# xiongzhenhai-zh/emqx

Measured on AMD Instinct MI355X. Metric: published topics matched/sec (and match evals/sec) at 10M subs; % of HBM BW, higher is better.
Workload: dtype u32; 1 GPU; B: 10M mixed exact/'+'/'#' subscriptions, 1xMI355X, batched topics of depth 4-8; n_filters=10000000, batch_topics_per_gpu=1000000, mode=routes, parallelism=replicated table, topic stream split x1, walk_order=batch order

## Files before the change

### emqx_amd/csrc/engine.cpp

```cpp
#include <hip/hip_runtime.h>

#include <algorithm>
#include <atomic>
#include <chrono>
#include <cstdlib>
#include <cstring>
#include <memory>
#include <mutex>
#include <string>
#include <thread>
#include <vector>

#include "../../include/emqx_match.h"
#include "kernels.h"
#include "streams.h"
#include "tables.h"

using namespace emqx;

namespace {

#define HIP_TRY(expr)                    \
  do {                                   \
    hipError_t _e = (expr);              \
    if (_e != hipSuccess) {              \
      set_last_error(hipGetErrorString(_e)); \
      return EMQX_EDEVICE;               \
    }                                    \
  } while (0)

thread_local std::string g_last_error;
void set_last_error(const char* s) { g_last_error = s ? s : ""; }

template <class T>
void dfree(T*& p) {
  if (p) (void)hipFree(p);
  p = nullptr;
}

template <class T>
hipError_t dalloc(T*& p, uint64_t count) {
  dfree(p);
  return hipMalloc(reinterpret_cast<void**>(&p), std::max<uint64_t>(count, 1) * sizeof(T));
}

struct DeviceTables {
  int device = 0;
  EdgeSlot* edges = nullptr;
  uint32_t* fids = nullptr;
  VocabSlot* vocab = nullptr;
  uint8_t* arena = nullptr;
  uint64_t cap_slots = 0, n_vocab = 0, cap_arena = 0;
  uint64_t bytes() const {
    return cap_slots * (sizeof(EdgeSlot) + 2 * sizeof(uint32_t)) + n_vocab * sizeof(VocabSlot) + cap_arena;
  }
  ~DeviceTables() {
    int cur = 0;
    (void)hipGetDevice(&cur);
    (void)hipSetDevice(device);
    (void)hipDeviceSynchronize();
    dfree(edges);
    dfree(fids);
    dfree(vocab);
    dfree(arena);
    (void)hipSetDevice(cur);
  }
};

struct Snapshot {
  std::shared_ptr<DeviceTables> dt;
  TableView tv{};
  uint64_t n_nodes = 0, n_slots = 0, n_words = 0, bytes = 0;
  uint32_t max_depth = 0;
};

struct LiveState {
  bool valid = false;
  std::shared_ptr<DeviceTables> dt;
  std::unique_ptr<VocabState> vocab;
  std::unique_ptr<LiveTrie> lt;
  uint64_t inserted = 0;
  uint64_t base_live = 0;
  hipStream_t stream = nullptr;
  SlotPatch* d_patch = nullptr;
  uint64_t cap_patch = 0;
  std::vector<SlotPatch> patches;
  int device = 0;
  ~LiveState() {
    (void)hipSetDevice(device);
    if (d_patch) (void)hipFree(d_patch);
    if (stream) (void)hipStreamDestroy(stream);
  }
};

struct Workspace {
  int device = 0;
  hipStream_t stream = nullptr;
  hipStream_t last_stream = nullptr;
  hipEvent_t ev0 = nullptr, ev1 = nullptr, evk = nullptr;
  uint64_t cap_n = 0, cap_tiles = 0, cap_slab = 0;
  uint32_t slab_per_tile = 256;
  uint32_t* counts = nullptr;
  uint32_t* deferred = nullptr;
  uint32_t* deep_rank = nullptr;
  uint64_t* slab = nullptr;
  uint32_t* tile_fill = nullptr;
  uint64_t* tile_defer = nullptr;
  uint2* spill = nullptr;
  uint64_t* diag = nullptr;
  uint32_t spill_cap = 2048;
  uint32_t* ctrl = nullptr;
  uint64_t* tile_sum = nullptr;
  uint2* tile_stats = nullptr;
  uint64_t* group_sum = nullptr;
  uint2* group_stats = nullptr;
  hipEvent_t done = nullptr;
  std::shared_ptr<Snapshot> inflight;
  uint32_t* deep_wids = nullptr;
  uint4* deep_stack = nullptr;
  uint32_t deep_stack_cap = 1u << 14;
  uint64_t* deep_slab = nullptr;
  uint32_t deep_slab_cap = 1u << 20;
  uint64_t* h_rb = nullptr;
  bool deep_ready = false;
  bool ordered = false;
  hipEvent_t evo = nullptr;
  uint64_t ord_cap_n = 0, ord_cap_bytes = 0, ord_temp_bytes = 0;
  uint64_t* ord_keys = nullptr;
  uint64_t* ord_keys_out = nullptr;
  uint32_t* ord_idx = nullptr;
  uint32_t* ord_perm = nullptr;
  uint32_t* ord_lens = nullptr;
  uint32_t* ord_corig = nullptr;
  uint64_t* ord_noffs = nullptr;
  uint64_t* ord_partials = nullptr;
  uint8_t* ord_bytes = nullptr;
  uint8_t* ord_temp = nullptr;

  ~Workspace() {
    (void)hipSetDevice(device);
    dfree(counts); dfree(deferred); dfree(deep_rank); dfree(slab); dfree(tile_fill);
    dfree(tile_defer); dfree(spill); dfree(diag); dfree(ctrl); dfree(tile_sum); dfree(tile_stats);
    dfree(group_sum); dfree(group_stats);
    dfree(deep_wids); dfree(deep_stack); dfree(deep_slab);
    dfree(ord_keys); dfree(ord_keys_out); dfree(ord_idx); dfree(ord_perm); dfree(ord_lens); dfree(ord_corig);
    dfree(ord_noffs); dfree(ord_partials); dfree(ord_bytes); dfree(ord_temp);
    if (h_rb) (void)hipHostFree(h_rb);
    if (ev0) (void)hipEventDestroy(ev0);
    if (ev1) (void)hipEventDestroy(ev1);
    if (evk) (void)hipEventDestroy(evk);
    if (evo) (void)hipEventDestroy(evo);
    if (done) (void)hipEventDestroy(done);
    if (stream) (void)hipStreamDestroy(stream);
  }
};

uint64_t round_pow2(uint64_t x) {
  uint64_t p = 1;
  while (p < x) p <<= 1;
  return p;
}

}

struct emqx_engine {
  int device = 0;
  std::mutex writer;
  FilterStore store;
  uint64_t epoch = 0;
  double last_build_ms = 0;
  std::mutex snap_mu;
  std::shared_ptr<Snapshot> snap;
  std::mutex ws_mu;
  std::vector<std::unique_ptr<Workspace>> all_ws;
  std::vector<Workspace*> free_ws;
  std::atomic<uint64_t> last_evals{0}, last_deferred{0}, last_max_stack{0};
  std::atomic<double> last_match_ms{0};
  std::atomic<double> last_kernel_ms{0};
  std::atomic<int> forced_variant{-1};
  std::atomic<bool> diag_on{false};
  std::atomic<uint32_t> diag_stop{0};
  uint4* timeline = nullptr;
  uint64_t timeline_cap = 0;
  std::atomic<uint32_t> slab_hint{256};
  LiveState ls;
  std::vector<uint32_t> dirty;
  bool incremental = true;
  int64_t delta_max = -1;
  uint64_t last_commit_kind = 0;
  uint64_t last_relocations = 0, last_in_place = 0, last_patches = 0, last_new_slots = 0;
  double last_host_ms = 0;
  uint64_t last_extents = 0, last_vocab_slots = 0;
  double last_upload_ms = 0;
  std::mutex hb_mu;
  std::vector<emqx_host_batch*> hb_free;
  int commit_threads = std::max(1u, std::min(8u, std::thread::hardware_concurrency()));
  std::atomic<int> order{-1};
  std::atomic<int> order_level_bits{0};
  std::atomic<int> order_sort_bits{64};
  std::atomic<int> order_deal{1};
  std::atomic<uint64_t> last_ordered{0};
  std::atomic<uint64_t> order_bpt{48};
  std::atomic<double> last_order_ms{0};
  std::atomic<bool> small_batch{true};
};

namespace {

constexpr int EMQX_NEED_FULL = 1;

void publish(emqx_engine* e, std::shared_ptr<Snapshot> s) {
  std::lock_guard<std::mutex> g(e->snap_mu);
  e->snap = std::move(s);
}

int full_commit(emqx_engine* e) {
  auto vs = std::make_unique<VocabState>();
  std::vector<uint64_t> loc;
  std::vector<uint32_t> slot_ids;
  BuildOpts o;
  o.vocab = vs.get();
  o.fid_loc = &loc;
  o.slot_ids = &slot_ids;
  o.threads = e->commit_threads;
  HostTables ht;
  std::string err;
  if (!build_tables(e->store, o, ht, &err)) {
    set_last_error(err.c_str());
    return EMQX_ENOMEM;
  }
  const uint64_t n_slots = ht.edges.size();
  const uint64_t spare = std::min<uint64_t>(std::max<uint64_t>(1u << 20, n_slots / 2), MAX_SLOTS - n_slots);
  auto dt = std::make_shared<DeviceTables>();
  dt->device = e->device;
  dt->cap_slots = n_slots + spare;
  dt->n_vocab = ht.vocab.size();
  dt->cap_arena = ht.arena.size() + std::max<uint64_t>(1u << 20, ht.arena.size() / 4) + 16;
  HIP_TRY(dalloc(dt->edges, dt->cap_slots));
  HIP_TRY(dalloc(dt->fids, 2 * dt->cap_slots));
  HIP_TRY(dalloc(dt->vocab, dt->n_vocab));
  HIP_TRY(dalloc(dt->arena, dt->cap_arena));
  HIP_TRY(hipMemcpy(dt->edges, ht.edges.data(), n_slots * sizeof(EdgeSlot), hipMemcpyHostToDevice));
  HIP_TRY(hipMemcpy(dt->fids, ht.fids.data(), ht.fids.size() * sizeof(uint32_t), hipMemcpyHostToDevice));
  HIP_TRY(hipMemcpy(dt->vocab, ht.vocab.data(), ht.vocab.size() * sizeof(VocabSlot), hipMemcpyHostToDevice));
  HIP_TRY(hipMemcpy(dt->arena, ht.arena.data(), ht.arena.size(), hipMemcpyHostToDevice));
  HIP_TRY(hipStreamSynchronize(nullptr));

  auto s = std::make_shared<Snapshot>();
  s->dt = dt;
  s->tv.edges = dt->edges;
  s->tv.fids = dt->fids;
  s->tv.vocab = dt->vocab;
  s->tv.arena = dt->arena;
  s->tv.vocab_mask = ht.vocab_mask;
  s->tv.root_base = ht.root_base;
  s->tv.root_meta = ht.root_meta;
  s->tv.root_hash_fid = ht.root_hash_fid;
  s->tv.plus_mask = ht.plus_mask;
  s->n_nodes = ht.n_nodes;
  s->n_slots = n_slots;
  s->n_words = ht.n_words;
  s->max_depth = ht.max_depth;
  s->bytes = dt->bytes();

  LiveState& d = e->ls;
  d.device = e->device;
  d.dt = dt;
  d.vocab = std::move(vs);
  if (!d.lt) d.lt = std::make_unique<LiveTrie>();
  d.lt->adopt(ht, loc, slot_ids, spare, d.vocab.get());
  d.valid = true;
  d.inserted = 0;
  d.base_live = e->store.n_live;
  e->dirty.clear();
  publish(e, std::move(s));
  e->last_commit_kind = 0;
  return EMQX_OK;
}

int live_commit(emqx_engine* e) {
  LiveState& d = e->ls;
  LiveTrie& lt = *d.lt;
  const FilterStore& fs = e->store;
  std::vector<uint32_t> ids(e->dirty);
  sort_unique_u32(ids);
  uint64_t creates = 0;
  for (uint32_t id : ids)
    if (fs.live[id] && (id >= lt.loc.size() || lt.loc[id] == FIDLOC_NONE)) ++creates;
  if (e->delta_max >= 0) {
    if (d.inserted + creates > static_cast<uint64_t>(e->delta_max)) return EMQX_NEED_FULL;
  } else if (creates && 2 * (d.inserted + creates) > d.base_live) {
    return EMQX_NEED_FULL;
  }

  const uint64_t nw0 = d.vocab->n_words(), arena0 = d.vocab->arena.size();
  auto th0 = std::chrono::steady_clock::now();
  if (!lt.commit(fs, ids, e->commit_threads)) return EMQX_NEED_FULL;
  e->last_host_ms = std::chrono::duration<double, std::milli>(std::chrono::steady_clock::now() - th0).count();
  std::vector<uint32_t> vdirty;
  if (!d.vocab->insert_table(nw0, &vdirty) || d.vocab->arena.size() + 16 > d.dt->cap_arena) return EMQX_NEED_FULL;
  lt.patches(d.patches);
  e->last_extents = lt.ranges.size();
  e->last_vocab_slots = vdirty.size();
  const auto tu0 = std::chrono::steady_clock::now();

  HIP_TRY(hipSetDevice(e->device));
  if (!d.stream) HIP_TRY(hipStreamCreateWithFlags(&d.stream, hipStreamNonBlocking));
  hipStream_t st = d.stream;
  for (const auto& r : lt.ranges) {
    const uint64_t a0 = r.first, a1 = r.second;
    HIP_TRY(hipMemcpyAsync(d.dt->edges + a0, lt.edges.data() + a0, (a1 - a0) * sizeof(EdgeSlot),
                           hipMemcpyHostToDevice, st));
    HIP_TRY(hipMemcpyAsync(d.dt->fids + 2 * a0, lt.fids.data() + 2 * a0, 2 * (a1 - a0) * sizeof(uint32_t),
                           hipMemcpyHostToDevice, st));
  }
  if (d.vocab->arena.size() > arena0)
    HIP_TRY(hipMemcpyAsync(d.dt->arena + arena0, d.vocab->arena.data() + arena0, d.vocab->arena.size() - arena0,
                           hipMemcpyHostToDevice, st));
  for (uint32_t v : vdirty)
    HIP_TRY(hipMemcpyAsync(d.dt->vocab + v, &d.vocab->table[v], sizeof(VocabSlot), hipMemcpyHostToDevice, st));
  const uint64_t np = d.patches.size();
  if (np) {
    if (np > d.cap_patch) {
      HIP_TRY(hipStreamSynchronize(st));
      d.cap_patch = round_pow2(np);
      HIP_TRY(dalloc(d.d_patch, d.cap_patch));
    }
    HIP_TRY(hipMemcpyAsync(d.d_patch, d.patches.data(), np * sizeof(SlotPatch), hipMemcpyHostToDevice, st));
    HIP_TRY(launch_slot_patches(d.dt->edges, d.dt->fids, d.d_patch, static_cast<uint32_t>(np), st));
  }
  HIP_TRY(hipStreamSynchronize(st));
  e->last_upload_ms = std::chrono::duration<double, std::milli>(std::chrono::steady_clock::now() - tu0).count();

  std::shared_ptr<Snapshot> cur;
  {
    std::lock_guard<std::mutex> g(e->snap_mu);
    cur = e->snap;
  }
  auto s = std::make_shared<Snapshot>(*cur);
  s->tv.root_base = lt.root_base;
  s->tv.root_meta = lt.root_meta;
  s->tv.root_hash_fid = lt.root_hash_fid;
  s->n_nodes = lt.n_nodes;
  s->n_slots = lt.used;
  s->n_words = d.vocab->n_words();
  s->max_depth = lt.max_depth;
  d.inserted += creates;
  e->last_relocations = lt.relocations;
  e->last_in_place = lt.in_place;
  e->last_patches = np;
  e->last_new_slots = lt.new_slots();
  e->dirty.clear();
  publish(e, std::move(s));
  e->last_commit_kind = 1;
  return EMQX_OK;
}

int commit_locked(emqx_engine* e) {
  auto t0 = std::chrono::steady_clock::now();
  int rc = EMQX_NEED_FULL;
  if (e->incremental && e->ls.valid && e->snap) rc = live_commit(e);
  if (rc == EMQX_NEED_FULL) rc = full_commit(e);
  if (rc != EMQX_OK) return rc;
  e->epoch += 1;
  e->last_build_ms = std::chrono::duration<double, std::milli>(std::chrono::steady_clock::now() - t0).count();
  return EMQX_OK;
}

Workspace* acquire_ws(emqx_engine* e, hipStream_t want = nullptr) {
  std::lock_guard<std::mutex> g(e->ws_mu);
  auto& f = e->free_ws;
  auto take = [&](size_t i) {
    Workspace* w = f[i];
    f.erase(f.begin() + static_cast<std::ptrdiff_t>(i));
    w->slab_per_tile = std::max(w->slab_per_tile, e->slab_hint.load());
    return w;
  };
  if (!f.empty() && !want) return take(f.size() - 1);
  for (size_t i = f.size(); i-- > 0;)
    if (f[i]->last_stream == want || !f[i]->last_stream) return take(i);
  if (f.size() >= 8)
    for (size_t i = f.size(); i-- > 0;)
      if (!f[i]->done || hipEventQuery(f[i]->done) == hipSuccess) return take(i);
  auto w = std::make_unique<Workspace>();
  w->device = e->device;
  w->slab_per_tile = std::max(w->slab_per_tile, e->slab_hint.load());
  Workspace* p = w.get();
  e->all_ws.push_back(std::move(w));
  return p;
}

void release_ws(emqx_engine* e, Workspace* w) {
  std::lock_guard<std::mutex> g(e->ws_mu);
  e->free_ws.push_back(w);
}

int ensure_ws(Workspace* w, uint64_t n) {
  if (!w->stream) {
    HIP_TRY(hipStreamCreateWithFlags(&w->stream, hipStreamNonBlocking));
    HIP_TRY(hipEventCreate(&w->ev0));
    HIP_TRY(hipEventCreate(&w->ev1));
    HIP_TRY(hipEventCreate(&w->evk));
    HIP_TRY(hipEventCreate(&w->evo));
    HIP_TRY(hipEventCreateWithFlags(&w->done, hipEventDisableTiming));
    HIP_TRY(hipHostMalloc(reinterpret_cast<void**>(&w->h_rb), SUM_WORDS * sizeof(uint64_t), hipHostMallocDefault));
    HIP_TRY(dalloc(w->ctrl, CTRL_WORDS));
    HIP_TRY(dalloc(w->diag, DIAG_WORDS));
    HIP_TRY(hipMemset(w->diag, 0, DIAG_WORDS * sizeof(uint64_t)));
  }
  if (!w->deep_ready) {
    HIP_TRY(dalloc(w->deep_wids, uint64_t(DEEP_WAVES) * DEEP_MAX_LEVELS));
    HIP_TRY(dalloc(w->deep_stack, uint64_t(DEEP_WAVES) * w->deep_stack_cap));
    HIP_TRY(dalloc(w->deep_slab, w->deep_slab_cap));
    w->deep_ready = true;
  }
  if (n > w->cap_n) {
    const uint64_t cap = round_pow2(std::max<uint64_t>(n, 1024));
    HIP_TRY(dalloc(w->counts, cap));
    HIP_TRY(dalloc(w->deferred, cap));
    HIP_TRY(dalloc(w->deep_rank, cap));
    w->cap_n = cap;
  }
  const uint64_t ntiles = (n + TILE_TOPICS - 1) / TILE_TOPICS;
  if (ntiles > w->cap_tiles || w->cap_tiles == 0) {
    const uint64_t cap = round_pow2(std::max<uint64_t>(ntiles, 64));
    HIP_TRY(dalloc(w->tile_fill, cap));
    HIP_TRY(dalloc(w->tile_defer, cap));
    HIP_TRY(dalloc(w->tile_sum, cap));
    HIP_TRY(dalloc(w->tile_stats, cap));
    HIP_TRY(dalloc(w->group_sum, cap / GROUP_TILES + 1));
    HIP_TRY(dalloc(w->group_stats, cap / GROUP_TILES + 1));
    HIP_TRY(dalloc(w->spill, cap * w->spill_cap));
    w->cap_tiles = cap;
  }
  const uint64_t need_slab = std::max<uint64_t>(ntiles, 1) * w->slab_per_tile;
  if (need_slab > w->cap_slab) {
    const uint64_t cap = need_slab;
    HIP_TRY(dalloc(w->slab, cap));
    w->cap_slab = cap;
  }
  return EMQX_OK;
}

constexpr uint64_t ORDER_MIN_N = 65536;

bool use_order(const emqx_engine* e, const Snapshot& snap, uint64_t n) {
  if (n > 0xFFFFFFFFull) return false;
  const int o = e->order.load();
  if (o >= 0) return o > 0 && n > 0;
  return snap.max_depth > 12 && n >= ORDER_MIN_N;
}

int ensure_order(emqx_engine* e, Workspace* w, uint64_t n, uint32_t sort_bits) {
  if (n > w->ord_cap_n) {
    const uint64_t cap = round_pow2(std::max<uint64_t>(n, 1024));
    HIP_TRY(dalloc(w->ord_keys, cap));
    HIP_TRY(dalloc(w->ord_keys_out, cap));
    HIP_TRY(dalloc(w->ord_idx, cap));
    HIP_TRY(dalloc(w->ord_perm, cap));
    HIP_TRY(dalloc(w->ord_lens, cap));
    HIP_TRY(dalloc(w->ord_corig, cap));
    HIP_TRY(dalloc(w->ord_noffs, cap + 1));
    HIP_TRY(dalloc(w->ord_partials, scan_partials(cap)));
    w->ord_cap_n = cap;
  }
  const uint64_t tb = order_sort_temp_bytes(n, sort_bits);
  if (!w->ord_temp || tb > w->ord_temp_bytes) {
    HIP_TRY(dalloc(w->ord_temp, tb));
    w->ord_temp_bytes = tb;
  }
  const uint64_t want = e->order_bpt.load() * n + 4096;
  if (!w->ord_bytes || w->ord_cap_bytes < want) {
    const uint64_t cap = std::max<uint64_t>(w->ord_cap_bytes, want);
    HIP_TRY(dalloc(w->ord_bytes, cap + 16));
    w->ord_cap_bytes = cap;
  }
  return EMQX_OK;
}

FastVariant pick_variant(const emqx_engine* e, const Snapshot& snap) {
  static const int env_forced = [] {
    const char* v = getenv("EMQX_FAST_VARIANT");
    return v ? atoi(v) : -1;
  }();
  const int fv = e->forced_variant.load();
  const int forced = fv >= 0 ? fv : env_forced;
  if (forced >= 0 && forced < FAST_NVARIANTS) return static_cast<FastVariant>(forced);
  return snap.max_depth > 12 ? FAST_K1_S512W : FAST_K1_S384B1;
}

MatchArgs match_args(emqx_engine* e, const Snapshot& snap, Workspace* w, uint32_t mode, const uint8_t* d_tbytes,
                     const uint64_t* d_toffs, uint64_t n, uint64_t* d_out_off, uint32_t* d_out_ids, uint64_t cap,
                     uint64_t* summary) {
  MatchArgs a{};
  a.tv = snap.tv;
  a.tbytes = d_tbytes;
  a.toffs = d_toffs;
  a.n = n;
  a.mode = mode;
  a.slab_cap = w->slab_per_tile;
  a.counts = w->counts;
  a.slab = w->slab;
  a.tile_fill = w->tile_fill;
  a.tile_defer = w->tile_defer;
  a.spill = w->spill;
  a.diag = e->diag_on.load() ? w->diag : nullptr;
  a.diag_stop = a.diag ? e->diag_stop.load() : 0u;
  a.timeline = a.diag && e->timeline && (n + TILE_TOPICS - 1) / TILE_TOPICS <= e->timeline_cap ? e->timeline : nullptr;
  a.spill_cap = w->spill_cap;
  a.ctrl = w->ctrl;
  a.deferred = w->deferred;
  a.deep_wids = w->deep_wids;
  a.deep_stack = w->deep_stack;
  a.deep_stack_cap = w->deep_stack_cap;
  a.deep_waves = DEEP_WAVES;
  a.deep_slab = w->deep_slab;
  a.deep_slab_cap = w->deep_slab_cap;
  a.tile_sum = w->tile_sum;
  a.tile_stats = w->tile_stats;
  a.group_sum = w->group_sum;
  a.group_stats = w->group_stats;
  a.ngroups = static_cast<uint32_t>((n + TILE_TOPICS * GROUP_TILES - 1) / (TILE_TOPICS * GROUP_TILES));
  a.deep_rank = w->deep_rank;
  a.out_off = d_out_off;
  a.out_ids = d_out_ids;
  a.out_cap = d_out_ids ? cap : 0;
  a.summary = summary;
  return a;
}

int enqueue_match(emqx_engine* e, const Snapshot& snap, Workspace* w, uint32_t mode, const uint8_t* d_tbytes,
                  const uint64_t* d_toffs, uint64_t n, uint64_t* d_out_off, uint32_t* d_out_ids, uint64_t cap,
                  uint64_t* summary, hipStream_t s) {
  int rc = ensure_ws(w, n);
  if (rc != EMQX_OK) return rc;
  MatchArgs a = match_args(e, snap, w, mode, d_tbytes, d_toffs, n, d_out_off, d_out_ids, cap, summary);
  const bool ordered = use_order(e, snap, n);
  const uint32_t sort_bits = static_cast<uint32_t>(std::min(64, std::max(1, e->order_sort_bits.load())));
  if (ordered) {
    rc = ensure_order(e, w, n, sort_bits);
    if (rc != EMQX_OK) return rc;
  }

  HIP_TRY(hipStreamWaitEvent(s, w->done, 0));
  w->last_stream = s;
  HIP_TRY(hipMemsetAsync(w->ctrl, 0, CTRL_WORDS * sizeof(uint32_t), s));
  w->ordered = ordered;
  if (ordered) {
    HIP_TRY(hipEventRecord(w->evo, s));
    OrderArgs o{};
    o.tbytes = d_tbytes;
    o.toffs = d_toffs;
    o.n = n;
    const int lb = e->order_level_bits.load();
    o.level_bits = static_cast<uint32_t>(lb > 0 ? std::min(lb, 32) : (snap.max_depth > 12 ? 4 : 8));
    o.sort_bits = sort_bits;
    o.keys = w->ord_keys;
    o.keys_out = w->ord_keys_out;
    o.idx = w->ord_idx;
    o.perm = w->ord_perm;
    o.lens = w->ord_lens;
    o.noffs = w->ord_noffs;
    o.partials = w->ord_partials;
    o.obytes = w->ord_bytes;
    o.cap_bytes = w->ord_cap_bytes;
    o.temp = w->ord_temp;
    o.temp_bytes = w->ord_temp_bytes;
    o.ctrl = w->ctrl;
    HIP_TRY(launch_order(o, s));
    a.tbytes = w->ord_bytes;
    a.toffs = w->ord_noffs;
    a.perm = w->ord_perm;
    a.deal = e->order_deal.load() ? 1u : 0u;
    a.corig = w->ord_corig;
    a.partials = w->ord_partials;
  }
  HIP_TRY(hipEventRecord(w->ev0, s));
  HIP_TRY(launch_match_fast(a, pick_variant(e, snap), s));
  HIP_TRY(hipEventRecord(w->evk, s));
  HIP_TRY(launch_match_deep(a, s));
  HIP_TRY(launch_assemble(a, s));
  HIP_TRY(hipEventRecord(w->ev1, s));
  HIP_TRY(hipEventRecord(w->done, s));
  return EMQX_OK;
}

int run_match(emqx_engine* e, const Snapshot& snap, Workspace* w, uint32_t mode, const uint8_t* d_tbytes,
              const uint64_t* d_toffs, uint64_t n, uint64_t* d_out_off, uint32_t* d_out_ids, uint64_t cap,
              uint64_t* n_out, hipStream_t s) {
  uint64_t* sum_dev = nullptr;
  HIP_TRY(hipHostGetDevicePointer(reinterpret_cast<void**>(&sum_dev), w->h_rb, 0));
  for (int attempt = 0; attempt < 8; ++attempt) {
    int rc = enqueue_match(e, snap, w, mode, d_tbytes, d_toffs, n, d_out_off, d_out_ids, cap, sum_dev, s);
    if (rc != EMQX_OK) return rc;
    HIP_TRY(hipStreamSynchronize(s));
    const uint64_t* sm = w->h_rb;
    const uint64_t flags = sm[SUM_FLAGS];
    const uint32_t err = static_cast<uint32_t>(sm[SUM_ERROR]);
    if (flags & SUM_F_ERROR) {
      set_last_error("topic longer than 65535 bytes on the deep path");
      return EMQX_EINVAL;
    }
    if (flags & SUM_F_RETRY) {
      if (sm[SUM_NEED_SLAB] > w->slab_per_tile) {
        const uint64_t need = sm[SUM_NEED_SLAB];
        w->slab_per_tile = static_cast<uint32_t>(((need + need / 8) + 511) / 512 * 512);
        uint32_t h = e->slab_hint.load();
        while (h < w->slab_per_tile && !e->slab_hint.compare_exchange_weak(h, w->slab_per_tile)) {
        }
      }
      if (err & CTRL_ERR_DEEP_SLAB) {
        w->deep_slab_cap = static_cast<uint32_t>(std::min<uint64_t>(round_pow2(sm[SUM_DEEP_FILL] + uint64_t(DEEP_WAVES) * DEEP_CHUNK + 1), 1u << 30));
        HIP_TRY(dalloc(w->deep_slab, w->deep_slab_cap));
      }
      if (err & CTRL_ERR_ORDER_CAP) {
        uint64_t nb = 0;
        HIP_TRY(hipMemcpy(&nb, d_toffs + n, sizeof(uint64_t), hipMemcpyDeviceToHost));
        uint64_t nb0 = 0;
        HIP_TRY(hipMemcpy(&nb0, d_toffs, sizeof(uint64_t), hipMemcpyDeviceToHost));
        const uint64_t need = nb - nb0;
        w->ord_cap_bytes = need + need / 8 + 4096;
        HIP_TRY(dalloc(w->ord_bytes, w->ord_cap_bytes + 16));
        const uint64_t bpt = (need + need / 8) / std::max<uint64_t>(n, 1) + 1;
        uint64_t h = e->order_bpt.load();
        while (h < bpt && !e->order_bpt.compare_exchange_weak(h, bpt)) {
        }
      }
      if (err & CTRL_ERR_TOO_DEEP) {
        if (w->deep_stack_cap >= (1u << 22)) {
          set_last_error("topic frontier exceeds the deep path's stack");
          return EMQX_ETOODEEP;
        }
        w->deep_stack_cap <<= 2;
        HIP_TRY(dalloc(w->deep_stack, uint64_t(DEEP_WAVES) * w->deep_stack_cap));
      }
      continue;
    }
    float kms = 0, ms = 0;
    if (hipEventElapsedTime(&kms, w->ev0, w->evk) == hipSuccess) e->last_kernel_ms.store(kms);
    (void)hipEventElapsedTime(&ms, w->ev0, w->ev1);
    float oms = 0;
    if (w->ordered && hipEventElapsedTime(&oms, w->evo, w->ev0) == hipSuccess) ms += oms;
    e->last_match_ms.store(ms);
    e->last_order_ms.store(w->ordered ? oms : 0.0);
    e->last_ordered.store(w->ordered ? 1 : 0);
    e->last_deferred.store(sm[SUM_DEFERRED]);
    e->last_evals.store(sm[SUM_EVALS]);
    e->last_max_stack.store(sm[SUM_MAXSTACK]);
    *n_out = sm[SUM_TOTAL];
    return (flags & SUM_F_OVERFLOW) ? EMQX_EOVERFLOW : EMQX_OK;
  }
  set_last_error("match did not converge");
  return EMQX_EDEVICE;
}

std::shared_ptr<Snapshot> current(emqx_engine* e) {
  std::lock_guard<std::mutex> g(e->snap_mu);
  return e->snap;
}

bool small_ok(const emqx_engine* e, const Snapshot& snap, uint64_t n) {
  return e->small_batch.load() && n > 0 && n <= SMALL_MAX_N && snap.max_depth <= 12 && !e->diag_on.load() &&
         !use_order(e, snap, n);
}

int enqueue_small(emqx_engine* e, const Snapshot& snap, Workspace* w, uint32_t mode, const uint8_t* h_tbytes,
                  const uint64_t* h_toffs, uint64_t n, uint64_t nbytes, uint8_t* d_tbytes, uint64_t* d_toffs,
                  uint64_t* d_out_off, uint32_t* d_out_ids, uint64_t cap, uint64_t* summary, uint64_t* h_out_off,
                  uint32_t* h_out_ids, uint64_t h_cap, const SmallFanout* f, hipStream_t s) {
  int rc = ensure_ws(w, SMALL_MAX_N);
  if (rc != EMQX_OK) return rc;
  SmallArgs sa{};
  sa.m = match_args(e, snap, w, mode, d_tbytes, d_toffs, n, d_out_off, d_out_ids, cap, summary);
  sa.m.diag = nullptr;
  sa.h_tbytes = h_tbytes;
  sa.h_toffs = h_toffs;
  sa.nbytes = nbytes;
  sa.tt = static_cast<uint32_t>((n + SMALL_WAVES - 1) / SMALL_WAVES);
  sa.slab_tiles = static_cast<uint32_t>(std::min<uint64_t>(w->cap_slab / w->slab_per_tile, w->cap_tiles));
  sa.h_out_off = h_out_off;
  sa.h_out_ids = h_out_ids;
  sa.h_cap = h_cap;
  sa.clk = e->timeline && e->timeline_cap * 2 >= SMALL_CLK_WORDS ? reinterpret_cast<uint64_t*>(e->timeline) : nullptr;
  if (f) {
    sa.has_fanout = 1;
    sa.f = *f;
  }
  HIP_TRY(hipStreamWaitEvent(s, w->done, 0));
  w->last_stream = s;
  w->ordered = false;
  HIP_TRY(launch_small_batch(sa, s));
  HIP_TRY(hipEventRecord(w->done, s));
  return EMQX_OK;
}

struct HostBatchPriv {
  emqx_engine* e = nullptr;
  hipStream_t stream = nullptr;
  hipEvent_t done = nullptr;
  uint8_t* d_tbytes = nullptr;
  uint64_t* d_toffs = nullptr;
  uint64_t* d_out_off = nullptr;
  uint32_t* d_out_ids = nullptr;
  uint64_t* summary = nullptr;
  std::shared_ptr<Snapshot> snap;
  std::shared_ptr<Snapshot> pin;
  uint32_t mode = 0;
  bool pending = false;
  uint64_t evals = 0, deferred = 0, max_stack = 0;
};

template <class T>
hipError_t halloc(T*& p, uint64_t count) {
  if (p) (void)hipHostFree(p);
  p = nullptr;
  return hipHostMalloc(reinterpret_cast<void**>(&p), std::max<uint64_t>(count, 1) * sizeof(T), hipHostMallocDefault);
}

int hb_alloc(emqx_host_batch* b, uint64_t cap_topics, uint64_t cap_bytes, uint64_t cap_ids, bool keep_inputs) {
  auto* p = static_cast<HostBatchPriv*>(b->priv);
  HIP_TRY(hipSetDevice(p->e->device));
  if (cap_topics > b->cap_topics) {
    uint64_t* t = nullptr;
    HIP_TRY(halloc(t, cap_topics + 1));
    if (keep_inputs && b->topic_offsets) std::memcpy(t, b->topic_offsets, (b->cap_topics + 1) * sizeof(uint64_t));
    if (b->topic_offsets) (void)hipHostFree(b->topic_offsets);
    b->topic_offsets = t;
    HIP_TRY(halloc(b->out_offsets, cap_topics + 1));
    HIP_TRY(dalloc(p->d_toffs, cap_topics + 1));
    HIP_TRY(dalloc(p->d_out_off, cap_topics + 1));
    b->cap_topics = cap_topics;
  }
  if (cap_bytes > b->cap_bytes) {
    uint8_t* t = nullptr;
    HIP_TRY(halloc(t, cap_bytes + 16));
    if (keep_inputs && b->topic_bytes) std::memcpy(t, b->topic_bytes, b->cap_bytes);
    if (b->topic_bytes) (void)hipHostFree(b->topic_bytes);
    b->topic_bytes = t;
    HIP_TRY(dalloc(p->d_tbytes, cap_bytes + 16));
    b->cap_bytes = cap_bytes;
  }
  if (cap_ids > b->cap_ids) {
    HIP_TRY(halloc(b->out_ids, cap_ids));
    HIP_TRY(dalloc(p->d_out_ids, cap_ids));
    b->cap_ids = cap_ids;
  }
  return EMQX_OK;
}

int hb_enqueue(emqx_host_batch* b) {
  auto* p = static_cast<HostBatchPriv*>(b->priv);
  emqx_engine* e = p->e;
  const uint64_t n = b->n, nbytes = n ? b->topic_offsets[n] : 0;
  hipStream_t s = p->stream;
  uint64_t* sum_dev = nullptr;
  HIP_TRY(hipHostGetDevicePointer(reinterpret_cast<void**>(&sum_dev), p->summary, 0));
  p->snap = p->pin ? p->pin : current(e);
  if (small_ok(e, *p->snap, n)) {
    const uint8_t* h_tb = nullptr;
    const uint64_t* h_to = nullptr;
    uint64_t* h_off = nullptr;
    uint32_t* h_ids = nullptr;
    HIP_TRY(hipHostGetDevicePointer(reinterpret_cast<void**>(const_cast<uint8_t**>(&h_tb)), b->topic_bytes, 0));
    HIP_TRY(hipHostGetDevicePointer(reinterpret_cast<void**>(const_cast<uint64_t**>(&h_to)), b->topic_offsets, 0));
    HIP_TRY(hipHostGetDevicePointer(reinterpret_cast<void**>(&h_off), b->out_offsets, 0));
    HIP_TRY(hipHostGetDevicePointer(reinterpret_cast<void**>(&h_ids), b->out_ids, 0));
    Workspace* w = acquire_ws(e, s);
    int rc = enqueue_small(e, *p->snap, w, p->mode, h_tb, h_to, n, nbytes, p->d_tbytes, p->d_toffs, p->d_out_off,
                           p->d_out_ids, b->cap_ids, sum_dev, h_off, h_ids, b->cap_ids, nullptr, s);
    if (rc == EMQX_OK) w->inflight = p->snap;
    release_ws(e, w);
    if (rc != EMQX_OK) return rc;
    HIP_TRY(hipEventRecord(p->done, s));
    p->pending = true;
    return EMQX_OK;
  }
  if (nbytes) HIP_TRY(hipMemcpyAsync(p->d_tbytes, b->topic_bytes, nbytes, hipMemcpyHostToDevice, s));
  HIP_TRY(hipMemcpyAsync(p->d_toffs, b->topic_offsets, (n + 1) * sizeof(uint64_t), hipMemcpyHostToDevice, s));
  Workspace* w = acquire_ws(e, s);
  int rc = ensure_ws(w, n);
  if (rc == EMQX_OK)
    rc = enqueue_match(e, *p->snap, w, p->mode, p->d_tbytes, p->d_toffs, n, p->d_out_off, p->d_out_ids, b->cap_ids,
                       sum_dev, s);
  if (rc == EMQX_OK) w->inflight = p->snap;
  release_ws(e, w);
  if (rc != EMQX_OK) return rc;
  uint64_t *h_off = nullptr;
  uint32_t* h_ids = nullptr;
  HIP_TRY(hipHostGetDevicePointer(reinterpret_cast<void**>(&h_off), b->out_offsets, 0));
  HIP_TRY(hipHostGetDevicePointer(reinterpret_cast<void**>(&h_ids), b->out_ids, 0));
  HIP_TRY(launch_csr_to_host(p->d_out_off, n, p->d_out_ids, b->cap_ids, h_off, h_ids, s));
  HIP_TRY(hipEventRecord(p->done, s));
  p->pending = true;
  return EMQX_OK;
}

int hb_wait(emqx_host_batch* b) {
  auto* p = static_cast<HostBatchPriv*>(b->priv);
  if (!p->pending) return EMQX_EINVAL;
  HIP_TRY(hipSetDevice(p->e->device));
  p->pending = false;
  HIP_TRY(hipEventSynchronize(p->done));
  uint64_t flags = p->summary[SUM_FLAGS];
  uint64_t total = p->summary[SUM_TOTAL];
  if (flags & SUM_F_RETRY) {
    Workspace* w = acquire_ws(p->e, p->stream);
    int rc = ensure_ws(w, b->n);
    if (rc == EMQX_OK)
      rc = run_match(p->e, *p->snap, w, p->mode, p->d_tbytes, p->d_toffs, b->n, p->d_out_off, p->d_out_ids,
                     b->cap_ids, &total, p->stream);
    release_ws(p->e, w);
    if (rc != EMQX_OK && rc != EMQX_EOVERFLOW) return rc;
    uint64_t *h_off = nullptr;
    uint32_t* h_ids = nullptr;
    HIP_TRY(hipHostGetDevicePointer(reinterpret_cast<void**>(&h_off), b->out_offsets, 0));
    HIP_TRY(hipHostGetDevicePointer(reinterpret_cast<void**>(&h_ids), b->out_ids, 0));
    HIP_TRY(launch_csr_to_host(p->d_out_off, b->n, p->d_out_ids, b->cap_ids, h_off, h_ids, p->stream));
    HIP_TRY(hipStreamSynchronize(p->stream));
    flags = total > b->cap_ids ? SUM_F_OVERFLOW : 0;
  } else if (flags & SUM_F_ERROR) {
    set_last_error("topic longer than 65535 bytes on the deep path");
    return EMQX_EINVAL;
  }
  p->snap.reset();
  b->n_out = total;
  if (!(flags & SUM_F_RETRY)) {
    p->evals = p->summary[SUM_EVALS];
    p->deferred = p->summary[SUM_DEFERRED];
    p->max_stack = p->summary[SUM_MAXSTACK];
    p->e->last_evals.store(p->evals);
    p->e->last_deferred.store(p->deferred);
    p->e->last_max_stack.store(p->max_stack);
  } else {
    p->evals = p->e->last_evals.load();
    p->deferred = p->e->last_deferred.load();
    p->max_stack = p->e->last_max_stack.load();
  }
  return (flags & SUM_F_OVERFLOW) ? EMQX_EOVERFLOW : EMQX_OK;
}

}

int emqx::engine_small_batch(emqx_engine* e, uint32_t mode, const uint8_t* h_tbytes, const uint64_t* h_toffs,
                             uint64_t n, uint64_t nbytes, uint8_t* d_tbytes, uint64_t* d_toffs, uint64_t* d_out_off,
                             uint32_t* d_out_ids, uint64_t cap, uint64_t* h_summary, const SmallFanout& f,
                             hipStream_t s) {
  auto snap = current(e);
  if (!small_ok(e, *snap, n)) return SMALL_NOT_TAKEN;
  HIP_TRY(hipSetDevice(e->device));
  Workspace* w = acquire_ws(e, s);
  int rc = enqueue_small(e, *snap, w, mode, h_tbytes, h_toffs, n, nbytes, d_tbytes, d_toffs, d_out_off, d_out_ids,
                         cap, h_summary, nullptr, nullptr, 0, &f, s);
  if (rc == EMQX_OK) w->inflight = snap;
  release_ws(e, w);
  return rc;
}

namespace {

bool offsets_ok(const uint64_t* offs, uint64_t n) {
  if (!offs) return n == 0;
  for (uint64_t i = 0; i < n; ++i)
    if (offs[i + 1] < offs[i]) return false;
  return true;
}

}

extern "C" {

int emqx_engine_create(const emqx_engine_opts* opts, emqx_engine** out) {
  if (!out) return EMQX_EINVAL;
  *out = nullptr;
  int ndev = 0;
  if (hipGetDeviceCount(&ndev) != hipSuccess || ndev <= 0) {
    set_last_error("no HIP device");
    return EMQX_EDEVICE;
  }
  int dev = 0;
  if (opts && opts->device >= 0) dev = opts->device;
  else (void)hipGetDevice(&dev);
  if (dev >= ndev) return EMQX_EINVAL;
  HIP_TRY(hipSetDevice(dev));
  auto* e = new (std::nothrow) emqx_engine();
  if (!e) return EMQX_ENOMEM;
  e->device = dev;
  int rc = commit_locked(e);
  if (rc != EMQX_OK) {
    delete e;
    return rc;
  }
  e->epoch = 0;
  *out = e;
  return EMQX_OK;
}

int emqx_engine_destroy(emqx_engine* e) {
  if (!e) return EMQX_EINVAL;
  (void)hipSetDevice(e->device);
  for (emqx_host_batch* b : e->hb_free) emqx_host_batch_destroy(b);
  e->hb_free.clear();
  dfree(e->timeline);
  delete e;
  return EMQX_OK;
}

int emqx_insert_filters(emqx_engine* e, const uint8_t* bytes, const uint64_t* offsets, uint64_t n,
                        uint32_t* ids_out) {
  if (!e || (n && (!offsets || (!bytes && offsets[n] != offsets[0])))) return EMQX_EINVAL;
  if (!offsets_ok(offsets, n)) return EMQX_EINVAL;
  std::lock_guard<std::mutex> g(e->writer);
  for (uint64_t i = 0; i < n; ++i) {
    bool created = false;
    const uint32_t id = e->store.insert(bytes + offsets[i], offsets[i + 1] - offsets[i], &created);
    e->dirty.push_back(id);
    if (ids_out) ids_out[i] = id;
  }
  return EMQX_OK;
}

int emqx_insert_filters_ext(emqx_engine* e, const uint8_t* bytes, const uint64_t* offsets, uint64_t n,
                            const uint32_t* ext_ids, uint32_t* ids_out) {
  if (!e || !ext_ids || (n && (!offsets || (!bytes && offsets[n] != offsets[0])))) return EMQX_EINVAL;
  if (!offsets_ok(offsets, n)) return EMQX_EINVAL;
  std::lock_guard<std::mutex> g(e->writer);
  for (uint64_t i = 0; i < n; ++i) {
    bool created = false;
    const uint32_t id = e->store.insert(bytes + offsets[i], offsets[i + 1] - offsets[i], &created);
    if (e->store.ext[id] != ext_ids[i]) e->ls.valid = false;
    e->store.ext[id] = ext_ids[i];
    e->dirty.push_back(id);
    if (ids_out) ids_out[i] = id;
  }
  return EMQX_OK;
}

int emqx_delete_filters(emqx_engine* e, const uint32_t* ids, uint64_t n) {
  if (!e || (n && !ids)) return EMQX_EINVAL;
  std::lock_guard<std::mutex> g(e->writer);
  for (uint64_t i = 0; i < n; ++i)
    if (ids[i] >= e->store.n_ids()) return EMQX_ENOTFOUND;
  for (uint64_t i = 0; i < n; ++i) {
    if (e->store.live[ids[i]]) {
      e->store.live[ids[i]] = 0;
      e->store.n_live -= 1;
      e->dirty.push_back(ids[i]);
    }
  }
  return EMQX_OK;
}

int emqx_lookup_filter(emqx_engine* e, const uint8_t* bytes, uint64_t len, uint32_t* id_out) {
  if (!e || !id_out || (len && !bytes)) return EMQX_EINVAL;
  std::lock_guard<std::mutex> g(e->writer);
  const uint32_t id = e->store.find(bytes, len);
  if (id == WID_NONE || !e->store.live[id]) return EMQX_ENOTFOUND;
  *id_out = id;
  return EMQX_OK;
}

int emqx_filter_name(emqx_engine* e, uint32_t id, uint8_t* buf, uint64_t cap, uint64_t* len_out) {
  if (!e || !len_out) return EMQX_EINVAL;
  std::lock_guard<std::mutex> g(e->writer);
  if (id >= e->store.n_ids()) return EMQX_ENOTFOUND;
  const uint64_t len = e->store.off[id + 1] - e->store.off[id];
  *len_out = len;
  if (buf && cap) std::memcpy(buf, e->store.bytes.data() + e->store.off[id], std::min(len, cap));
  return EMQX_OK;
}

int emqx_commit(emqx_engine* e) {
  if (!e) return EMQX_EINVAL;
  HIP_TRY(hipSetDevice(e->device));
  std::lock_guard<std::mutex> g(e->writer);
  return commit_locked(e);
}

int emqx_match_batch_device(emqx_engine* e, uint32_t mode, const uint8_t* d_topic_bytes,
                            const uint64_t* d_topic_offsets, uint64_t n, uint64_t* d_out_offsets,
                            uint32_t* d_out_ids, uint64_t cap, uint64_t* n_out, void* stream) {
  if (!e || !n_out || mode > EMQX_MODE_TRIE_WILDCARD) return EMQX_EINVAL;
  if (n && (!d_topic_bytes || !d_topic_offsets)) return EMQX_EINVAL;
  if (!d_out_offsets) return EMQX_EINVAL;
  HIP_TRY(hipSetDevice(e->device));
  auto snap = current(e);
  Workspace* w = acquire_ws(e, static_cast<hipStream_t>(stream));
  int rc = ensure_ws(w, n);
  if (rc == EMQX_OK) {
    hipStream_t s = stream ? static_cast<hipStream_t>(stream) : w->stream;
    if (!stream && after_null_stream(s) != hipSuccess) rc = EMQX_EDEVICE;
    if (rc == EMQX_OK)
      rc = run_match(e, *snap, w, mode, d_topic_bytes, d_topic_offsets, n, d_out_offsets, d_out_ids, cap, n_out, s);
  }
  release_ws(e, w);
  return rc;
}

int emqx_match_batch_device_async(emqx_engine* e, uint32_t mode, const uint8_t* d_topic_bytes,
                                  const uint64_t* d_topic_offsets, uint64_t n, uint64_t* d_out_offsets,
                                  uint32_t* d_out_ids, uint64_t cap, uint64_t* summary, void* stream) {
  if (!e || !summary || mode > EMQX_MODE_TRIE_WILDCARD) return EMQX_EINVAL;
  if (n && (!d_topic_bytes || !d_topic_offsets)) return EMQX_EINVAL;
  if (!d_out_offsets) return EMQX_EINVAL;
  HIP_TRY(hipSetDevice(e->device));
  auto snap = current(e);
  Workspace* w = acquire_ws(e, static_cast<hipStream_t>(stream));
  int rc = ensure_ws(w, n);
  if (rc == EMQX_OK) {
    hipStream_t s = stream ? static_cast<hipStream_t>(stream) : w->stream;
    if (!stream && after_null_stream(s) != hipSuccess) rc = EMQX_EDEVICE;
    if (rc == EMQX_OK)
      rc = enqueue_match(e, *snap, w, mode, d_topic_bytes, d_topic_offsets, n, d_out_offsets, d_out_ids, cap,
                       summary, s);
    w->inflight = snap;
  }
  release_ws(e, w);
  return rc;
}

int emqx_host_batch_create(emqx_engine* e, uint64_t cap_topics, uint64_t cap_bytes, uint64_t cap_ids,
                           emqx_host_batch** out) {
  if (!e || !out) return EMQX_EINVAL;
  *out = nullptr;
  auto* b = new (std::nothrow) emqx_host_batch();
  auto* p = new (std::nothrow) HostBatchPriv();
  if (!b || !p) {
    delete b;
    delete p;
    return EMQX_ENOMEM;
  }
  std::memset(b, 0, sizeof(*b));
  b->priv = p;
  p->e = e;
  int rc = EMQX_OK;
  if (hipSetDevice(e->device) != hipSuccess || hipStreamCreateWithFlags(&p->stream, hipStreamNonBlocking) != hipSuccess ||
      hipEventCreateWithFlags(&p->done, hipEventDisableTiming) != hipSuccess || halloc(p->summary, SUM_WORDS) != hipSuccess)
    rc = EMQX_EDEVICE;
  if (rc == EMQX_OK)
    rc = hb_alloc(b, std::max<uint64_t>(cap_topics, 1), std::max<uint64_t>(cap_bytes, 64), std::max<uint64_t>(cap_ids, 64),
                  false);
  if (rc != EMQX_OK) {
    emqx_host_batch_destroy(b);
    return rc;
  }
  *out = b;
  return EMQX_OK;
}

int emqx_host_batch_destroy(emqx_host_batch* b) {
  if (!b) return EMQX_EINVAL;
  auto* p = static_cast<HostBatchPriv*>(b->priv);
  (void)hipSetDevice(p->e->device);
  if (p->stream) (void)hipStreamSynchronize(p->stream);
  if (b->topic_bytes) (void)hipHostFree(b->topic_bytes);
  if (b->topic_offsets) (void)hipHostFree(b->topic_offsets);
  if (b->out_offsets) (void)hipHostFree(b->out_offsets);
  if (b->out_ids) (void)hipHostFree(b->out_ids);
  if (p->summary) (void)hipHostFree(p->summary);
  dfree(p->d_tbytes);
  dfree(p->d_toffs);
  dfree(p->d_out_off);
  dfree(p->d_out_ids);
  if (p->done) (void)hipEventDestroy(p->done);
  if (p->stream) (void)hipStreamDestroy(p->stream);
  delete p;
  delete b;
  return EMQX_OK;
}

int emqx_host_batch_reserve(emqx_host_batch* b, uint64_t cap_topics, uint64_t cap_bytes, uint64_t cap_ids) {
  if (!b || static_cast<HostBatchPriv*>(b->priv)->pending) return EMQX_EINVAL;
  return hb_alloc(b, cap_topics, cap_bytes, cap_ids, true);
}

int emqx_host_batch_submit(emqx_host_batch* b, uint32_t mode) {
  if (!b || mode > EMQX_MODE_TRIE_WILDCARD) return EMQX_EINVAL;
  auto* p = static_cast<HostBatchPriv*>(b->priv);
  if (p->pending || b->n > b->cap_topics) return EMQX_EINVAL;
  const uint64_t* o = b->topic_offsets;
  if (o[0] != 0 || o[b->n] > b->cap_bytes || !offsets_ok(o, b->n)) return EMQX_EINVAL;
  HIP_TRY(hipSetDevice(p->e->device));
  p->mode = mode;
  return hb_enqueue(b);
}

int emqx_host_batch_wait(emqx_host_batch* b) {
  if (!b) return EMQX_EINVAL;
  return hb_wait(b);
}

int emqx_host_batch_query(emqx_host_batch* b) {
  if (!b) return EMQX_EINVAL;
  auto* p = static_cast<HostBatchPriv*>(b->priv);
  return !p->pending || hipEventQuery(p->done) == hipSuccess ? 1 : 0;
}

int emqx_match_batch(emqx_engine* e, uint32_t mode, const uint8_t* topic_bytes, const uint64_t* topic_offsets,
                     uint64_t n, uint64_t* out_offsets, uint32_t* out_ids, uint64_t cap, uint64_t* n_out) {
  if (!e || !n_out || !out_offsets || mode > EMQX_MODE_TRIE_WILDCARD) return EMQX_EINVAL;
  if (n && !topic_offsets) return EMQX_EINVAL;
  if (!offsets_ok(topic_offsets, n)) return EMQX_EINVAL;
  const uint64_t b0 = n ? topic_offsets[0] : 0, b1 = n ? topic_offsets[n] : 0;
  if (b1 > b0 && !topic_bytes) return EMQX_EINVAL;
  HIP_TRY(hipSetDevice(e->device));
  constexpr uint64_t CH_TOPICS = 1u << 18, CH_BYTES = 16u << 20, CH_IDS = 8u << 20;
  emqx_host_batch* hb[2] = {nullptr, nullptr};
  {
    std::lock_guard<std::mutex> g(e->hb_mu);
    for (int k = 0; k < 2 && !e->hb_free.empty(); ++k) {
      hb[k] = e->hb_free.back();
      e->hb_free.pop_back();
    }
  }
  int rc = EMQX_OK;
  for (int k = 0; k < 2 && rc == EMQX_OK; ++k)
    if (!hb[k]) rc = emqx_host_batch_create(e, CH_TOPICS, CH_BYTES, CH_IDS, &hb[k]);
  const std::shared_ptr<Snapshot> pin = current(e);
  for (int k = 0; k < 2; ++k)
    if (hb[k]) static_cast<HostBatchPriv*>(hb[k]->priv)->pin = pin;
  uint64_t chunk_lo[2] = {0, 0}, total = 0, next = 0, evals = 0, deferred = 0, max_stack = 0;
  bool inflight[2] = {false, false}, overflow = false;
  auto pack = [&](int k) -> int {
    emqx_host_batch* b = hb[k];
    const uint64_t lo = next;
    uint64_t hi = lo;
    const uint64_t base = topic_offsets[lo];
    while (hi < n && hi - lo < b->cap_topics && topic_offsets[hi + 1] - base <= b->cap_bytes) ++hi;
    if (hi == lo) {
      int r = emqx_host_batch_reserve(b, b->cap_topics, topic_offsets[lo + 1] - base + 16, b->cap_ids);
      if (r != EMQX_OK) return r;
      hi = lo + 1;
    }
    const uint64_t nb = topic_offsets[hi] - base;
    if (nb) std::memcpy(b->topic_bytes, topic_bytes + base, nb);
    for (uint64_t i = lo; i <= hi; ++i) b->topic_offsets[i - lo] = topic_offsets[i] - base;
    b->n = hi - lo;
    chunk_lo[k] = lo;
    next = hi;
    return emqx_host_batch_submit(b, mode);
  };
  auto drain = [&](int k) -> int {
    emqx_host_batch* b = hb[k];
    int r = emqx_host_batch_wait(b);
    for (int tries = 0; r == EMQX_EOVERFLOW && tries < 4; ++tries) {
      r = emqx_host_batch_reserve(b, b->cap_topics, b->cap_bytes, b->n_out + (b->n_out >> 2) + 1024);
      if (r == EMQX_OK) r = emqx_host_batch_submit(b, mode);
      if (r == EMQX_OK) r = emqx_host_batch_wait(b);
    }
    if (r != EMQX_OK) return r;
    const auto* p = static_cast<const HostBatchPriv*>(b->priv);
    evals += p->evals;
    deferred += p->deferred;
    max_stack = std::max(max_stack, p->max_stack);
    const uint64_t lo = chunk_lo[k], m = b->n_out;
    for (uint64_t i = 0; i < b->n; ++i) out_offsets[lo + i] = total + b->out_offsets[i];
    if (!overflow && out_ids && total + m <= cap) {
      if (m) std::memcpy(out_ids + total, b->out_ids, m * sizeof(uint32_t));
    } else if (m) {
      overflow = true;
    }
    total += m;
    return EMQX_OK;
  };
  int k = 0;
  if (rc == EMQX_OK && n == 0) {
    out_offsets[0] = 0;
  } else {
    while (rc == EMQX_OK && (next < n || inflight[0] || inflight[1])) {
      if (inflight[k]) {
        rc = drain(k);
        inflight[k] = false;
      }
      if (rc == EMQX_OK && next < n) {
        rc = pack(k);
        inflight[k] = rc == EMQX_OK;
      }
      k ^= 1;
    }
  }
  for (int j = 0; j < 2; ++j)
    if (inflight[j]) (void)emqx_host_batch_wait(hb[j]);
  out_offsets[n] = total;
  *n_out = total;
  e->last_evals.store(evals);
  e->last_deferred.store(deferred);
  e->last_max_stack.store(max_stack);
  for (int j = 0; j < 2; ++j)
    if (hb[j]) static_cast<HostBatchPriv*>(hb[j]->priv)->pin.reset();
  {
    std::lock_guard<std::mutex> g(e->hb_mu);
    for (int j = 0; j < 2; ++j)
      if (hb[j]) e->hb_free.push_back(hb[j]);
  }
  if (rc == EMQX_OK && (overflow || total > cap)) rc = EMQX_EOVERFLOW;
  return rc;
}

int emqx_stats_get(emqx_engine* e, emqx_stats* dst) {
  if (!e || !dst || (dst->size && dst->size < sizeof(uint64_t))) return EMQX_EINVAL;
  const uint64_t want = dst->size ? std::min<uint64_t>(dst->size, sizeof(emqx_stats)) : sizeof(emqx_stats);
  emqx_stats full;
  emqx_stats* out = &full;
  std::memset(out, 0, sizeof(*out));
  {
    std::lock_guard<std::mutex> g(e->writer);
    out->n_filters = e->store.n_live;
    out->n_ids = e->store.n_ids();
    out->epoch = e->epoch;
    out->last_build_ms = e->last_build_ms;
    out->delta_filters = e->ls.inserted;
    out->last_commit_kind = e->last_commit_kind;
  }
  auto s = current(e);
  if (s) {
    out->n_nodes = s->n_nodes;
    out->n_slots = s->n_slots;
    out->n_words = s->n_words;
    out->table_bytes = s->bytes;
    out->max_depth = s->max_depth;
  }
  out->last_ordered = e->last_ordered.load();
  out->last_order_ms = e->last_order_ms.load();
  out->last_evals = e->last_evals.load();
  out->last_deferred = e->last_deferred.load();
  out->last_max_stack = e->last_max_stack.load();
  out->last_match_ms = e->last_match_ms.load();
  out->last_kernel_ms = e->last_kernel_ms.load();
  out->size = want;
  std::memcpy(dst, out, want);
  return EMQX_OK;
}

const char* emqx_strerror(int code) {
  switch (code) {
    case EMQX_OK: return "ok";
    case EMQX_EINVAL: return "invalid argument";
    case EMQX_ENOMEM: return "out of memory";
    case EMQX_EDEVICE: return g_last_error.empty() ? "device error" : g_last_error.c_str();
    case EMQX_EOVERFLOW: return "output capacity too small";
    case EMQX_ENOTFOUND: return "not found";
    case EMQX_ETOODEEP: return "topic frontier too deep";
    case EMQX_EBUSY: return "busy: every batch buffer is in use";
    default: return "unknown error";
  }
}

int emqx_set_tuning(emqx_engine* e, const char* key, int64_t value) {
  if (!e || !key) return EMQX_EINVAL;
  if (std::strcmp(key, "fast_variant") == 0) {
    if (value < -1 || value >= FAST_NVARIANTS) return EMQX_EINVAL;
    e->forced_variant.store(static_cast<int>(value));
    return EMQX_OK;
  }
  if (std::strcmp(key, "diag") == 0) {
    e->diag_on.store(value != 0);
    return EMQX_OK;
  }
  if (std::strcmp(key, "diag_stop") == 0) {
    e->diag_stop.store(static_cast<uint32_t>(value));
    return EMQX_OK;
  }
  if (std::strcmp(key, "timeline") == 0) {
    if (value < 0) return EMQX_EINVAL;
    HIP_TRY(hipSetDevice(e->device));
    HIP_TRY(hipDeviceSynchronize());
    dfree(e->timeline);
    e->timeline_cap = 0;
    if (value) {
      HIP_TRY(dalloc(e->timeline, static_cast<uint64_t>(value)));
      HIP_TRY(hipMemset(e->timeline, 0, static_cast<uint64_t>(value) * sizeof(uint4)));
      e->timeline_cap = static_cast<uint64_t>(value);
    }
    return EMQX_OK;
  }
  if (std::strcmp(key, "small_batch") == 0) {
    e->small_batch.store(value != 0);
    return EMQX_OK;
  }
  if (std::strcmp(key, "incremental") == 0) {
    std::lock_guard<std::mutex> g(e->writer);
    e->incremental = value != 0;
    return EMQX_OK;
  }
  if (std::strcmp(key, "commit_threads") == 0) {
    if (value < 1 || value > 256) return EMQX_EINVAL;
    std::lock_guard<std::mutex> g(e->writer);
    e->commit_threads = static_cast<int>(value);
    return EMQX_OK;
  }
  if (std::strcmp(key, "order") == 0) {
    if (value < -1 || value > 1) return EMQX_EINVAL;
    e->order.store(static_cast<int>(value));
    return EMQX_OK;
  }
  if (std::strcmp(key, "order_level_bits") == 0) {
    if (value < 0 || value > 32) return EMQX_EINVAL;
    e->order_level_bits.store(static_cast<int>(value));
    return EMQX_OK;
  }
  if (std::strcmp(key, "order_sort_bits") == 0) {
    if (value < 1 || value > 64) return EMQX_EINVAL;
    e->order_sort_bits.store(static_cast<int>(value));
    return EMQX_OK;
  }
  if (std::strcmp(key, "order_deal") == 0) {
    e->order_deal.store(value != 0);
    return EMQX_OK;
  }
  if (std::strcmp(key, "delta_max") == 0) {
    std::lock_guard<std::mutex> g(e->writer);
    e->delta_max = value;
    return EMQX_OK;
  }
  return EMQX_ENOTFOUND;
}

uint64_t emqx_permute_scratch_bytes(uint64_t n) { return permute_scratch_bytes(n); }

uint64_t emqx_owner_sort_scratch_bytes(uint64_t n, uint32_t world) { return owner_sort_scratch_bytes(n, world); }

int emqx_owner_sort_device(const uint32_t* d_owner, uint64_t n, uint32_t world, uint32_t* d_perm, void* d_scratch,
                           void* stream) {
  if (world == 0 || (n && (!d_owner || !d_perm || !d_scratch)) || n > 0xFFFFFFFFull) return EMQX_EINVAL;
  HIP_TRY(launch_owner_sort(d_owner, n, world, d_perm, d_scratch, static_cast<hipStream_t>(stream)));
  return EMQX_OK;
}

int emqx_batch_permute_device(const uint8_t* d_bytes, const uint64_t* d_offsets, uint64_t n, const uint32_t* d_perm,
                              uint8_t* d_out_bytes, uint64_t* d_out_offsets, void* d_scratch, void* stream) {
  if (!d_out_offsets || !d_scratch || (n && (!d_bytes || !d_offsets || !d_perm || !d_out_bytes))) return EMQX_EINVAL;
  HIP_TRY(launch_batch_permute(d_bytes, d_offsets, n, d_perm, d_out_bytes, d_out_offsets, d_scratch,
                               static_cast<hipStream_t>(stream)));
  return EMQX_OK;
}

int emqx_csr_unpermute_device(const uint32_t* d_counts, const uint32_t* d_ids, uint64_t n, const uint32_t* d_perm,
                              uint64_t* d_out_offsets, uint32_t* d_out_ids, void* d_scratch, void* stream) {
  if (!d_out_offsets || !d_scratch || (n && (!d_counts || !d_perm))) return EMQX_EINVAL;
  HIP_TRY(launch_csr_unpermute(d_counts, d_ids, n, d_perm, d_out_offsets, d_out_ids, d_scratch,
                               static_cast<hipStream_t>(stream)));
  return EMQX_OK;
}

int emqx_shard_owner_device(const uint8_t* d_bytes, const uint64_t* d_offsets, uint64_t n, uint32_t world,
                            uint32_t levels, uint32_t* d_owner, void* stream) {
  if ((n && (!d_bytes || !d_offsets || !d_owner)) || world == 0 || levels == 0) return EMQX_EINVAL;
  HIP_TRY(launch_shard_owner(d_bytes, d_offsets, n, world, levels, d_owner, static_cast<hipStream_t>(stream)));
  return EMQX_OK;
}

int emqx_shard_route_device(const uint8_t* d_bytes, const uint64_t* d_offsets, uint64_t n, uint32_t world,
                            const emqx_shard_split* d_splits, uint32_t n_splits, uint32_t* d_req2, void* stream) {
  if ((n && (!d_bytes || !d_offsets || !d_req2)) || world == 0 || (n_splits && !d_splits)) return EMQX_EINVAL;
  HIP_TRY(launch_shard_route(d_bytes, d_offsets, n, world, reinterpret_cast<const ShardSplitE*>(d_splits), n_splits,
                             d_req2, static_cast<hipStream_t>(stream)));
  return EMQX_OK;
}

int emqx_commit_stats(emqx_engine* e, uint64_t* out, uint32_t n) {
  if (!e || (n && !out)) return EMQX_EINVAL;
  std::lock_guard<std::mutex> g(e->writer);
  const LiveTrie* lt = e->ls.lt.get();
  uint64_t host_us = static_cast<uint64_t>(e->last_host_ms * 1e3);
  const uint64_t v[12] = {e->last_commit_kind, e->last_relocations, e->last_in_place, e->last_patches,
                          e->last_new_slots, lt ? lt->used : 0, lt ? lt->cap : 0, lt ? lt->garbage : 0, host_us,
                          e->last_extents, e->last_vocab_slots, static_cast<uint64_t>(e->last_upload_ms * 1e3)};
  for (uint32_t i = 0; i < n && i < 12; ++i) out[i] = v[i];
  return EMQX_OK;
}

int emqx_diag_read(emqx_engine* e, uint64_t* out, uint32_t n, int reset) {
  if (!e || !out) return EMQX_EINVAL;
  HIP_TRY(hipSetDevice(e->device));
  std::vector<uint64_t> acc(DIAG_WORDS, 0), tmp(DIAG_WORDS);
  std::lock_guard<std::mutex> g(e->ws_mu);
  for (auto& w : e->all_ws) {
    if (!w->diag) continue;
    HIP_TRY(hipMemcpy(tmp.data(), w->diag, DIAG_WORDS * sizeof(uint64_t), hipMemcpyDeviceToHost));
    for (uint32_t i = 0; i < DIAG_WORDS; ++i) acc[i] += tmp[i];
    if (reset) HIP_TRY(hipMemset(w->diag, 0, DIAG_WORDS * sizeof(uint64_t)));
  }
  for (uint32_t i = 0; i < n && i < DIAG_WORDS; ++i) out[i] = acc[i];
  return EMQX_OK;
}

int emqx_diag_timeline(emqx_engine* e, uint32_t* out, uint64_t cap_tiles, uint64_t* n_tiles) {
  if (!e || !n_tiles || (cap_tiles && !out)) return EMQX_EINVAL;
  *n_tiles = e->timeline_cap;
  if (!e->timeline || !cap_tiles) return EMQX_OK;
  HIP_TRY(hipSetDevice(e->device));
  HIP_TRY(hipDeviceSynchronize());
  HIP_TRY(hipMemcpy(out, e->timeline, std::min(cap_tiles, e->timeline_cap) * sizeof(uint4), hipMemcpyDeviceToHost));
  return EMQX_OK;
}

const char* emqx_version(void) { return "emqx-match-mi355x 0.1.0 (gfx950)"; }

}
```

### emqx_amd/csrc/kernels.h

```cpp
#pragma once

#include <hip/hip_runtime.h>
#include <stdint.h>

#include "layout.h"

namespace emqx {

enum Ctrl : uint32_t {
  CTRL_DEFERRED = 0,
  CTRL_NEED_SLAB = 1,
  CTRL_ERROR = 2,
  CTRL_DEEP_FILL = 3,
  CTRL_DEEP_EVALS = 4,
  CTRL_WORDS = 8
};
constexpr uint32_t GROUP_TILES = 256;
constexpr uint32_t CTRL_ERR_TOO_LONG = 1u;
constexpr uint32_t CTRL_ERR_TOO_DEEP = 2u;
constexpr uint32_t CTRL_ERR_DEEP_SLAB = 4u;
constexpr uint32_t CTRL_ERR_ORDER_CAP = 8u;

constexpr int TILE_TOPICS = 64;

enum Diag : uint32_t {
  DIAG_STEPS = 0,
  DIAG_ITEMS = 1,
  DIAG_LIT_PROBES = 2,
  DIAG_LIT_HITS = 3,
  DIAG_LIT_EXTRA = 4,
  DIAG_PLUS_PROBES = 5,
  DIAG_PLUS_HITS = 6,
  DIAG_EMITS = 7,
  DIAG_SPILLS = 8,
  DIAG_TICKS_A = 9,
  DIAG_TICKS_B = 10,
  DIAG_WAVES = 11,
  DIAG_LEVEL0 = 12,
  DIAG_SMALL = 20,
  DIAG_WIDE = 21,
  DIAG_NCOUNT = 22,
  DIAG_WORDS = 32
};
constexpr uint32_t DEEP_MAX_LEVELS = 65536;

enum Summary : uint32_t {
  SUM_FLAGS = 0,
  SUM_TOTAL = 1,
  SUM_EVALS = 2,
  SUM_MAXSTACK = 3,
  SUM_DEFERRED = 4,
  SUM_NEED_SLAB = 5,
  SUM_DEEP_FILL = 6,
  SUM_ERROR = 7,
  SUM_WORDS = 8
};
constexpr uint64_t SUM_F_RETRY = 1;
constexpr uint64_t SUM_F_OVERFLOW = 2;
constexpr uint64_t SUM_F_ERROR = 4;

struct MatchArgs {
  TableView tv;
  const uint8_t* tbytes;
  const uint64_t* toffs;
  uint64_t n;
  uint32_t mode;
  uint32_t slab_cap;
  uint32_t* counts;
  uint64_t* slab;
  uint32_t* tile_fill;
  uint64_t* tile_defer;
  uint32_t* ctrl;
  uint32_t* deferred;
  uint64_t* diag;
  uint4* timeline;
  uint32_t diag_stop;
  uint2* spill;
  uint32_t spill_cap;
  uint32_t* deep_wids;
  uint4* deep_stack;
  uint32_t deep_stack_cap;
  uint32_t deep_waves;
  uint64_t* deep_slab;
  uint32_t deep_slab_cap;
  uint64_t* tile_sum;
  uint2* tile_stats;
  uint64_t* group_sum;
  uint2* group_stats;
  uint32_t ngroups;
  uint32_t* deep_rank;
  uint64_t* out_off;
  uint32_t* out_ids;
  uint64_t out_cap;
  uint64_t* summary;
  const uint32_t* perm;
  uint32_t deal;
  uint32_t* corig;
  uint64_t* partials;
};

constexpr uint32_t SMALL_WAVES = 16;
constexpr uint64_t SMALL_MAX_N = uint64_t(SMALL_WAVES) * TILE_TOPICS;
constexpr uint32_t SMALL_FO_MAX_ENTRIES = 16384;

struct SmallFanout {
  const uint4* recs;
  uint32_t n_recs;
  const uint32_t* plain;
  const uint4* groups;
  const uint32_t* members;
  uint32_t strategy;
  uint32_t seed;
  const uint32_t* h_keys;
  uint32_t* d_keys;
  uint4* erec;
  uint32_t* etop;
  const unsigned long long* ps_count;
  uint64_t* h_off;
  uint32_t* h_subs;
  uint32_t* h_fil;
  uint64_t cap;
  uint64_t* h_sum;
};

struct SmallArgs {
  MatchArgs m;
  const uint8_t* h_tbytes;
  const uint64_t* h_toffs;
  uint64_t nbytes;
  uint32_t tt;
  uint32_t slab_tiles;
  uint32_t has_fanout;
  uint64_t* h_out_off;
  uint32_t* h_out_ids;
  uint64_t h_cap;
  uint64_t* clk;
  SmallFanout f;
};
enum : uint32_t {
  SMALL_CLK_COPY = 0, SMALL_CLK_WALK, SMALL_CLK_DEEP, SMALL_CLK_SCAN, SMALL_CLK_SCATTER, SMALL_CLK_OUT,
  SMALL_CLK_FO_PASS1, SMALL_CLK_FO_PASS2, SMALL_CLK_LAUNCHES, SMALL_CLK_WORDS = 10
};
hipError_t launch_small_batch(const SmallArgs& a, hipStream_t s);
}
struct emqx_engine;
namespace emqx {
constexpr int SMALL_NOT_TAKEN = 1;
int engine_small_batch(emqx_engine* e, uint32_t mode, const uint8_t* h_tbytes, const uint64_t* h_toffs, uint64_t n,
                       uint64_t nbytes, uint8_t* d_tbytes, uint64_t* d_toffs, uint64_t* d_out_off, uint32_t* d_out_ids,
                       uint64_t cap, uint64_t* h_summary, const SmallFanout& f, hipStream_t s);

constexpr uint32_t DEEP_WAVES = 512;
constexpr uint32_t DEEP_CHUNK = 256;
constexpr uint64_t DEEP_PAD = ~0ull;

enum FastVariant {
  FAST_K1_S1K = 0,
  FAST_K2_S1K = 1,
  FAST_K2_S2K = 2,
  FAST_K2_S768 = 3,
  FAST_K4_S2K = 4,
  FAST_K1_S256 = 5,
  FAST_K2_S512 = 6,
  FAST_K1_S384 = 7,
  FAST_K2_S512W = 8,
  FAST_K1_S768W = 9,
  FAST_K1_S512W = 10,
  FAST_K1_S384R = 11,
  FAST_K1_S384P = 12,
  FAST_K1_S384N = 13,
  FAST_K1_S384W7 = 14,
  FAST_K1_S384B2 = 15,
  FAST_K1_S384B1 = 16,
  FAST_K1_S512WB1 = 17,
  FAST_NVARIANTS = 18
};

hipError_t launch_match_fast(const MatchArgs& a, FastVariant v, hipStream_t s);
hipError_t launch_match_deep(const MatchArgs& a, hipStream_t s);
hipError_t launch_assemble(const MatchArgs& a, hipStream_t s);
hipError_t launch_csr_to_host(const uint64_t* d_off, uint64_t n, const uint32_t* d_ids, uint64_t cap,
                               uint64_t* h_off, uint32_t* h_ids, hipStream_t s);
hipError_t launch_shard_owner(const uint8_t* tbytes, const uint64_t* toffs, uint64_t n, uint32_t world,
                              uint32_t levels, uint32_t* owner, hipStream_t s);
hipError_t launch_shard_route(const uint8_t* tbytes, const uint64_t* toffs, uint64_t n, uint32_t world,
                              const ShardSplitE* splits, uint32_t n_splits, uint32_t* req2, hipStream_t s);
hipError_t launch_slot_patches(EdgeSlot* edges, uint32_t* fids, const SlotPatch* patches, uint32_t n,
                               hipStream_t s);
struct OrderArgs {
  const uint8_t* tbytes;
  const uint64_t* toffs;
  uint64_t n;
  uint32_t level_bits;
  uint32_t sort_bits;
  uint64_t* keys;
  uint64_t* keys_out;
  uint32_t* idx;
  uint32_t* perm;
  uint32_t* lens;
  uint64_t* noffs;
  uint64_t* partials;
  uint8_t* obytes;
  uint64_t cap_bytes;
  void* temp;
  uint64_t temp_bytes;
  uint32_t* ctrl;
};
uint64_t order_sort_temp_bytes(uint64_t n, uint32_t sort_bits);
hipError_t launch_order(const OrderArgs& o, hipStream_t s);
hipError_t launch_order_counts(const uint32_t* counts, const uint32_t* perm, uint64_t n, uint32_t* corig,
                               hipStream_t s);
uint64_t permute_scratch_bytes(uint64_t n);
hipError_t launch_batch_permute(const uint8_t* tbytes, const uint64_t* toffs, uint64_t n, const uint32_t* perm,
                                uint8_t* obytes, uint64_t* ooffs, void* scratch, hipStream_t s);
hipError_t launch_csr_unpermute(const uint32_t* counts, const uint32_t* ids, uint64_t n, const uint32_t* perm,
                                uint64_t* out_off, uint32_t* out_ids, void* scratch, hipStream_t s);
uint64_t owner_sort_scratch_bytes(uint64_t n, uint32_t world);
hipError_t launch_owner_sort(const uint32_t* owner, uint64_t n, uint32_t world, uint32_t* perm, void* scratch,
                             hipStream_t s);
uint64_t scan_partials(uint64_t n);
hipError_t launch_scan(const uint32_t* counts, uint64_t n, uint64_t* offsets, uint64_t* partials,
                       hipStream_t s);

}
```

### emqx_amd/csrc/layout.h

```cpp
#pragma once

#include <stdint.h>

#if defined(__HIPCC__)
#define EMQX_HD __host__ __device__ __forceinline__
#else
#define EMQX_HD inline
#endif

namespace emqx {

constexpr uint32_t WID_NONE = 0xFFFFFFFFu;
constexpr uint32_t WID_PLUS = 0xFFFFFFFEu;
constexpr uint32_t WID_HASH = 0xFFFFFFFDu;
constexpr uint32_t FID_NONE = 0xFFFFFFFFu;

constexpr uint32_t META_CAPLOG2_MASK = 0x1Fu;
constexpr uint32_t META_HAS_PLUS = 1u << 5;
constexpr uint32_t META_HAS_EDGES = 1u << 6;
constexpr uint32_t META_HAS_HASH = 1u << 7;
constexpr uint32_t META_HAS_TERM = 1u << 8;
constexpr uint32_t META_TERM_WILD = 1u << 9;
constexpr uint32_t META_PH = 1u << 10;
constexpr uint32_t META_LITF_EXACT = 1u << 11;
constexpr uint32_t META_LITF_NONE = 1u << 12;
constexpr uint32_t META_BUCKET_OVF = 1u << 13;
constexpr uint32_t META_XFID = 1u << 14;
constexpr uint32_t META_XFID_TERM = 1u << 15;
constexpr uint32_t META_F8_SHIFT = 24;
constexpr uint32_t META_SEED_SHIFT = 16;
constexpr uint32_t PH_MAX_CAPLOG = 15;

struct alignas(16) EdgeSlot {
  uint32_t wid;
  uint32_t child_base;
  uint32_t meta;
  uint32_t litf;
};
static_assert(sizeof(EdgeSlot) == 16, "EdgeSlot must be 16 bytes");
constexpr uint64_t MAX_SLOTS = (1ull << 31) - 1;

struct alignas(16) SlotPatch {
  uint32_t slot;
  uint32_t fid_h, fid_t;
  uint32_t pad;
  EdgeSlot s;
};
static_assert(sizeof(SlotPatch) == 32, "SlotPatch must be 32 bytes");

struct alignas(16) VocabSlot {
  uint32_t hash;
  uint32_t len;
  uint32_t wid;
  uint32_t off;
  uint32_t inl[4];
};
static_assert(sizeof(VocabSlot) == 32, "VocabSlot must be 32 bytes");

struct TableView {
  const EdgeSlot* edges;
  const uint32_t* fids;
  const VocabSlot* vocab;
  const uint8_t* arena;
  uint32_t vocab_mask;
  uint32_t root_base;
  uint32_t root_meta;
  uint32_t root_hash_fid;
  uint32_t plus_mask;
};

constexpr uint32_t PLUS_LINE = 4;
constexpr uint32_t PLUS_COPY_MAX_CAPLOG = 14;
EMQX_HD bool plus_copies(uint32_t plus_mask, bool has_plus, uint32_t caplog) {
  return plus_mask != 0 && has_plus && caplog > 2 && caplog <= PLUS_COPY_MAX_CAPLOG;
}
EMQX_HD bool plus_position(uint32_t i, bool copies) { return copies ? (i & (PLUS_LINE - 1u)) == 0 : i == 0; }
EMQX_HD uint32_t plus_copy(uint32_t i1, bool copies) { return copies ? (i1 & ~(PLUS_LINE - 1u)) : 0u; }

EMQX_HD uint32_t mix32(uint32_t x) {
  x ^= x >> 16;
  x *= 0x85ebca6bu;
  x ^= x >> 13;
  x *= 0xc2b2ae35u;
  x ^= x >> 16;
  return x;
}

EMQX_HD uint32_t whash_init(uint32_t len) { return len * 0x9E3779B1u + 0x7F4A7C15u; }
EMQX_HD uint32_t whash_step(uint32_t h, uint32_t d) {
  h = (h ^ d) * 0x85EBCA77u;
  return (h << 13) | (h >> 19);
}
EMQX_HD uint32_t word_hash16(uint32_t len, uint32_t w0, uint32_t w1, uint32_t w2, uint32_t w3) {
  return mix32(whash_step(whash_step(whash_step(whash_step(whash_init(len), w0), w1), w2), w3));
}
EMQX_HD uint32_t word_hash_bytes(const uint8_t* p, uint32_t n) {
  uint32_t h = whash_init(n);
  const uint32_t nd = n > 16 ? (n + 3) / 4 : 4;
  for (uint32_t i = 0; i < nd; ++i) {
    uint32_t d = 0;
    for (uint32_t b = 0; b < 4; ++b)
      if (4 * i + b < n) d |= static_cast<uint32_t>(p[4 * i + b]) << (8 * b);
    h = whash_step(h, d);
  }
  return mix32(h);
}

EMQX_HD uint32_t vocab_slot0(uint32_t hash) { return hash; }

EMQX_HD uint32_t node_hash(uint32_t wid, uint32_t seed) { return mix32(wid ^ (seed * 0x9E3779B1u + 0x7F4A7C15u)); }

EMQX_HD uint32_t ph_slot(uint32_t h, uint32_t mask, bool copies) {
  const uint32_t s = h & mask;
  return (!copies || (s & (PLUS_LINE - 1u))) ? s : s + 1u + (h >> 31);
}
EMQX_HD uint32_t lit_slot(uint32_t wid, uint32_t seed, uint32_t mask, bool copies) {
  return ph_slot(node_hash(wid, seed), mask, copies);
}


EMQX_HD uint32_t bucket1(uint32_t wid, uint32_t seed, uint32_t nbmask) { return node_hash(wid, seed) & nbmask; }
EMQX_HD uint32_t bucket2(uint32_t wid, uint32_t seed, uint32_t nbmask) {
  const uint32_t a = bucket1(wid, seed, nbmask), b = mix32(wid ^ (0xDAA66D2Bu + seed * 0x7F4A7C15u)) & nbmask;
  return b != a ? b : ((a + 1) & nbmask);
}
EMQX_HD uint32_t wide_slot1(uint32_t h, uint32_t mask, bool copies) {
  if (!copies) return 2u * (h & (mask >> 1));
  return (((h >> 1) & ((mask + 1u) / PLUS_LINE - 1u)) * PLUS_LINE) + 1u + (h & 1u);
}
EMQX_HD uint32_t wide_slot(uint32_t wid, uint32_t seed, uint32_t mask, bool copies, bool second) {
  if (!copies) return 2u * (second ? bucket2(wid, seed, mask >> 1) : bucket1(wid, seed, mask >> 1));
  const uint32_t lm = (mask + 1u) / PLUS_LINE - 1u;
  const uint32_t w1 = wide_slot1(node_hash(wid, seed), mask, true);
  if (!second) return w1;
  const uint32_t h2 = mix32(wid ^ (0xDAA66D2Bu + seed * 0x7F4A7C15u));
  const uint32_t w2 = (((h2 >> 1) & lm) * PLUS_LINE) + 1u + (h2 & 1u);
  return w2 != w1 ? w2 : (w1 ^ 3u);
}
constexpr uint32_t CUCKOO_SEEDS = 128;

EMQX_HD uint32_t litf_hash(uint32_t wid) {
  const uint32_t m = (wid ^ 0xA5A5A5A5u) * 0x9E3779B1u;
  return m ^ (m >> 15);
}

EMQX_HD bool litf_may_contain(uint32_t meta, uint32_t litf, uint32_t wid) {
  if (meta & META_LITF_NONE) return false;
  if (meta & META_XFID) {
    const uint32_t f8 = meta >> META_F8_SHIFT, h = litf_hash(wid);
    if (meta & META_LITF_EXACT) return (h >> 24) == f8;
    return ((f8 >> (h & 7u)) & 1u) != 0;
  }
  if (meta & META_LITF_EXACT) return litf == wid;
  const uint32_t h = litf_hash(wid);
  return ((litf >> (h & 31u)) & (litf >> ((h >> 5) & 31u)) & 1u) != 0;
}
constexpr uint32_t LITF_BLOOM_MAX = 16;

constexpr uint32_t SHARD_ALL = 0xFFFFFFFFu;
EMQX_HD uint32_t shard_owner(const uint8_t* p, uint64_t n, uint32_t world, uint32_t levels, bool topic) {
  uint64_t s = 0, e = 0;
  uint32_t k = 0;
  while (k < levels) {
    e = s;
    while (e < n && p[e] != '/') ++e;
    if (e - s == 1 && (p[s] == '+' || p[s] == '#')) return topic ? 0u : SHARD_ALL;
    ++k;
    if (e >= n) break;
    s = e + 1;
  }
  if (k < levels && !topic) return SHARD_ALL;
  uint32_t h = 0x811C9DC5u;
  for (uint64_t i = 0; i < e; ++i) h = (h ^ p[i]) * 0x01000193u;
  return mix32(h ^ k) % world;
}

constexpr uint32_t SHARD_NONE = 0xFFFFFFFFu;
constexpr uint32_t SHARD_SPACE_P = 0x80000000u;
constexpr uint32_t SHARD_PAIR = 0x40000000u;
constexpr uint32_t SHARD_HASH_MASK = 0x3FFFFFFFu;
constexpr uint32_t SHARD_ABSENT = 0x9E3779B9u;

struct ShardSplitE {
  uint32_t key, info;
};

constexpr uint32_t SHARD_P_REPLICATED = 0x0000FFFFu;

EMQX_HD uint32_t shard_word_step(uint32_t h, uint32_t w) { return (h ^ w) * 0x01000193u; }
EMQX_HD uint32_t shard_level_hash(const uint8_t* p, uint64_t s, uint64_t e) {
  uint32_t h = 0x811C9DC5u;
  uint64_t i = s;
  for (; i + 4 <= e; i += 4)
    h = shard_word_step(h, static_cast<uint32_t>(p[i]) | (static_cast<uint32_t>(p[i + 1]) << 8) |
                               (static_cast<uint32_t>(p[i + 2]) << 16) | (static_cast<uint32_t>(p[i + 3]) << 24));
  if (i < e) {
    uint32_t w = 0;
    for (uint32_t k = 0; i + k < e; ++k) w |= static_cast<uint32_t>(p[i + k]) << (8u * k);
    h = shard_word_step(h, w);
  }
  return mix32(h ^ static_cast<uint32_t>(e - s));
}

EMQX_HD uint32_t shard_split_find(const ShardSplitE* sp, uint32_t n, uint32_t key) {
  uint32_t lo = 0, hi = n;
  while (lo < hi) {
    const uint32_t mid = (lo + hi) >> 1;
    if (sp[mid].key < key) lo = mid + 1; else hi = mid;
  }
  return lo < n && sp[lo].key == key ? sp[lo].info : SHARD_NONE;
}

EMQX_HD bool shard_level(const uint8_t* p, uint64_t n, uint32_t k, uint64_t* s, uint64_t* e) {
  uint64_t a = 0;
  for (uint32_t j = 0; j < k; ++j) {
    while (a < n && p[a] != '/') ++a;
    if (a >= n) return false;
    ++a;
  }
  uint64_t b = a;
  while (b < n && p[b] != '/') ++b;
  *s = a;
  *e = b;
  return true;
}

EMQX_HD bool shard_is_wild(const uint8_t* p, uint64_t s, uint64_t e) {
  return e - s == 1 && (p[s] == '+' || p[s] == '#');
}

EMQX_HD void shard_place_key(uint32_t space, uint32_t hk, uint32_t next, uint32_t world, const ShardSplitE* sp,
                             uint32_t nsp, uint32_t* first, uint32_t* span) {
  const uint32_t info = shard_split_find(sp, nsp, space | (hk & SHARD_HASH_MASK));
  if (info == SHARD_NONE) {
    *first = mix32(hk ^ (space ? 0x5BD1E995u : 0x27D4EB2Fu)) % world;
    *span = 1;
    return;
  }
  const uint32_t base = info & 0xFFFFu, s = info >> 16;
  if (next == SHARD_NONE) {
    *first = base;
    *span = s;
    return;
  }
  const uint32_t pair = mix32(next ^ hk);
  const uint32_t pinfo = s > 1 && next != SHARD_ABSENT
                             ? shard_split_find(sp, nsp, SHARD_PAIR | space | (pair & SHARD_HASH_MASK))
                             : SHARD_NONE;
  *first = pinfo != SHARD_NONE ? (pinfo & 0xFFFFu) : (base + pair % s) % world;
  *span = 1;
}

EMQX_HD bool shard_p_replicated(const ShardSplitE* sp, uint32_t nsp) {
  return nsp && shard_split_find(sp, nsp, SHARD_SPACE_P) == SHARD_P_REPLICATED;
}

EMQX_HD void shard_place_filter(const uint8_t* p, uint64_t n, uint32_t world, const ShardSplitE* sp, uint32_t nsp,
                                uint32_t* first, uint32_t* span, uint32_t* engine) {
  uint64_t s1, e1, s2, e2, s3, e3;
  shard_level(p, n, 0, &s1, &e1);
  const bool has2 = shard_level(p, n, 1, &s2, &e2);
  *engine = 0;
  if (shard_is_wild(p, s1, e1)) {
    if (p[s1] == '#' || !has2 || shard_is_wild(p, s2, e2) || shard_p_replicated(sp, nsp)) {
      *first = 0;
      *span = world;
      return;
    }
    *engine = 1;
    const bool has3 = shard_level(p, n, 2, &s3, &e3);
    const uint32_t next = !has3 ? SHARD_ABSENT : shard_is_wild(p, s3, e3) ? SHARD_NONE : shard_level_hash(p, s3, e3);
    shard_place_key(SHARD_SPACE_P, shard_level_hash(p, s2, e2), next, world, sp, nsp, first, span);
    return;
  }
  const uint32_t next = !has2 ? SHARD_ABSENT : shard_is_wild(p, s2, e2) ? SHARD_NONE : shard_level_hash(p, s2, e2);
  shard_place_key(0, shard_level_hash(p, s1, e1), next, world, sp, nsp, first, span);
}

struct ShardTopicLevels {
  uint32_t n_levels;
  uint32_t h[3];
  bool wild;
};

EMQX_HD void shard_topic_levels(const uint8_t* p, uint64_t n, ShardTopicLevels* L) {
  L->n_levels = 0;
  L->wild = false;
  uint64_t s = 0;
  for (uint64_t i = 0; i <= n; ++i) {
    if (i < n && p[i] != '/') continue;
    if (L->n_levels < 3) L->h[L->n_levels] = shard_level_hash(p, s, i);
    if (i - s == 1 && (p[s] == '+' || p[s] == '#')) L->wild = true;
    ++L->n_levels;
    s = i + 1;
  }
}

EMQX_HD void shard_route_levels(const uint8_t* p, uint64_t n, const ShardTopicLevels& L, uint32_t world,
                                const ShardSplitE* sp, uint32_t nsp, uint32_t* req) {
  req[0] = req[1] = SHARD_NONE;
  uint32_t first, span, engine;
  if (L.wild) {
    shard_place_filter(p, n, world, sp, nsp, &first, &span, &engine);
    req[engine] = 2 * first + engine;
    return;
  }
  const bool has2 = L.n_levels >= 2, has3 = L.n_levels >= 3;
  shard_place_key(0, L.h[0], has2 ? L.h[1] : SHARD_ABSENT, world, sp, nsp, &first, &span);
  req[0] = 2 * first;
  if (!has2 || (n > 0 && p[0] == '$')) return;
  if (shard_p_replicated(sp, nsp)) return;
  shard_place_key(SHARD_SPACE_P, L.h[1], has3 ? L.h[2] : SHARD_ABSENT, world, sp, nsp, &first, &span);
  req[1] = 2 * first + 1;
}

EMQX_HD void shard_route_topic(const uint8_t* p, uint64_t n, uint32_t world, const ShardSplitE* sp, uint32_t nsp,
                               uint32_t* req) {
  ShardTopicLevels L;
  shard_topic_levels(p, n, &L);
  shard_route_levels(p, n, L, world, sp, nsp, req);
}

}
```

### emqx_amd/csrc/match_kernels.hip

```cpp
#include <hip/hip_runtime.h>

#include <algorithm>

#include "fanout.h"
#include "kernels.h"

namespace emqx {

namespace {

constexpr uint32_t MODE_ROUTES = 0, MODE_TRIE = 1;

__device__ __forceinline__ uint32_t lane_id() {
  return __builtin_amdgcn_mbcnt_hi(~0u, __builtin_amdgcn_mbcnt_lo(~0u, 0u));
}

__device__ __forceinline__ void wave_sync() {
  __builtin_amdgcn_fence(__ATOMIC_SEQ_CST, "wavefront");
  __builtin_amdgcn_wave_barrier();
}

__device__ __forceinline__ uint64_t lanemask_lt(uint32_t lane) { return (1ull << lane) - 1ull; }

template <int BITS>
__device__ __forceinline__ uint32_t wave_prefix(uint32_t v, uint32_t lane, uint32_t* total) {
  (void)lane;
  uint32_t pre = 0, tot = 0;
#pragma unroll
  for (int b = 0; b < BITS; ++b) {
    const uint64_t m = __ballot((v >> b) & 1u);
    pre += __builtin_amdgcn_mbcnt_hi(static_cast<uint32_t>(m >> 32), __builtin_amdgcn_mbcnt_lo(static_cast<uint32_t>(m), 0u))
           << b;
    tot += static_cast<uint32_t>(__popcll(m)) << b;
  }
  *total = tot;
  return pre;
}

__device__ __forceinline__ uint32_t wave_incl_scan(uint32_t v, uint32_t lane) {
#pragma unroll
  for (uint32_t d = 1; d < 64; d <<= 1) {
    const uint32_t o = __shfl_up(v, d, 64);
    if (lane >= d) v += o;
  }
  return v;
}

__device__ __forceinline__ uint64_t wave_incl_scan64(uint64_t v, uint32_t lane) {
#pragma unroll
  for (uint32_t d = 1; d < 64; d <<= 1) {
    const uint32_t lo = __shfl_up(static_cast<uint32_t>(v), d, 64);
    const uint32_t hi = __shfl_up(static_cast<uint32_t>(v >> 32), d, 64);
    if (lane >= d) v += (static_cast<uint64_t>(hi) << 32) | lo;
  }
  return v;
}

__device__ __forceinline__ uint32_t wave_sum(uint32_t v) {
#pragma unroll
  for (uint32_t d = 32; d >= 1; d >>= 1) v += __shfl_xor(v, d, 64);
  return v;
}


__device__ __forceinline__ uint64_t wave_or64(uint64_t v) {
#pragma unroll
  for (uint32_t d = 32; d >= 1; d >>= 1) {
    const uint32_t lo = __shfl_xor(static_cast<uint32_t>(v), d, 64);
    const uint32_t hi = __shfl_xor(static_cast<uint32_t>(v >> 32), d, 64);
    v |= (static_cast<uint64_t>(hi) << 32) | lo;
  }
  return v;
}

struct Slot {
  uint4 a;
  uint32_t idx;
};

__device__ __forceinline__ Slot load_slot(const EdgeSlot* edges, uint32_t i) {
  Slot s;
  s.a = *reinterpret_cast<const uint4*>(edges + i);
  s.idx = i;
  return s;
}

constexpr uint64_t ENTRY_REF = 1ull << 63;

__device__ __forceinline__ uint64_t emit_value(const Slot& s, uint32_t kind) {
  if (!(s.a.z & META_HAS_EDGES)) return kind ? s.a.w : s.a.y;
  if (s.a.z & META_XFID) return s.a.w;
  return ENTRY_REF | (2u * s.idx + kind);
}

__device__ __forceinline__ uint32_t resolve_entry(const TableView& tv, uint64_t e) {
  return (e & ENTRY_REF) ? tv.fids[static_cast<uint32_t>(e)] : static_cast<uint32_t>(e);
}

__device__ __forceinline__ Slot empty_slot() {
  Slot s;
  s.a = make_uint4(WID_NONE, 0, 0, 0);
  s.idx = 0;
  return s;
}


__device__ __forceinline__ bool term_ok(uint32_t meta, uint32_t mode, bool dollar_root_literal) {
  if (!(meta & META_HAS_TERM)) return false;
  if (mode == MODE_ROUTES) return true;
  if (meta & META_TERM_WILD) return true;
  return mode == MODE_TRIE && dollar_root_literal;
}

__device__ __forceinline__ uint32_t intern_word(const TableView& tv, uint32_t h, uint32_t len, uint32_t w0,
                                uint32_t w1, uint32_t w2, uint32_t w3, const uint8_t* tbytes,
                                uint64_t wstart) {
  uint32_t i = vocab_slot0(h) & tv.vocab_mask;
  for (uint32_t k = 0; k <= tv.vocab_mask; ++k) {
    const uint4* vp = reinterpret_cast<const uint4*>(tv.vocab + i);
    const uint4 hd = vp[0];
    if (hd.z == WID_NONE) return WID_NONE;
    if (hd.x == h && hd.y == len) {
      const uint4 in = vp[1];
      bool eq = in.x == w0 && in.y == w1 && in.z == w2 && in.w == w3;
      if (eq && len > 16) {
        for (uint32_t b = 16; b < len && eq; ++b) eq = tv.arena[hd.w + b] == tbytes[wstart + b];
      }
      if (eq) return hd.z;
    }
    i = (i + 1) & tv.vocab_mask;
  }
  return WID_NONE;
}

__device__ __forceinline__ bool probe_one(const EdgeSlot* edges, uint32_t plus_mask, uint32_t base,
                                          uint32_t meta, uint32_t wid, Slot* out) {
  if (wid == WID_PLUS) {
    *out = load_slot(edges, base);
    return out->a.x == WID_PLUS;
  }
  const uint32_t mask = (1u << (meta & META_CAPLOG2_MASK)) - 1u;
  const uint32_t sd = (meta >> META_SEED_SHIFT) & 255u;
  if (meta & META_PH) {
    const bool cp = plus_copies(plus_mask, (meta & META_HAS_PLUS) != 0, meta & META_CAPLOG2_MASK);
    *out = load_slot(edges, base + lit_slot(wid, sd, mask, cp));
    return out->a.x == wid;
  }
  const bool cp = plus_copies(plus_mask, (meta & META_HAS_PLUS) != 0, meta & META_CAPLOG2_MASK);
  const uint32_t b1 = wide_slot(wid, sd, mask, cp, false);
  const Slot x = load_slot(edges, base + b1), y = load_slot(edges, base + b1 + 1);
  if (x.a.x == wid) { *out = x; return true; }
  if (y.a.x == wid) { *out = y; return true; }
  if (!(x.a.z & META_BUCKET_OVF)) return false;
  const uint32_t b2 = wide_slot(wid, sd, mask, cp, true);
  const Slot u = load_slot(edges, base + b2), v = load_slot(edges, base + b2 + 1);
  if (u.a.x == wid) { *out = u; return true; }
  if (v.a.x == wid) { *out = v; return true; }
  return false;
}

template <class WidAt>
__device__ uint32_t exact_walk1(const TableView& tv, uint32_t root_base, uint32_t root_meta, uint32_t root_hash_fid,
                                uint32_t nlev, WidAt wid_at) {
  uint32_t base = root_base, meta = root_meta, at = 0, term_inline = FID_NONE;
  bool root = true;
  for (uint32_t k = 0; k < nlev; ++k) {
    const uint32_t w = wid_at(k);
    if (w == WID_HASH && k + 1 == nlev) {
      if (!(meta & META_HAS_HASH)) return FID_NONE;
      if (root) return root_hash_fid;
      return (meta & META_HAS_EDGES) ? tv.fids[2u * at] : base;
    }
    if (w == WID_NONE || !(meta & META_HAS_EDGES)) return FID_NONE;
    Slot s;
    if (!probe_one(tv.edges, tv.plus_mask, base, meta, w, &s)) return FID_NONE;
    base = s.a.y;
    meta = s.a.z;
    term_inline = s.a.w;
    at = s.idx;
    root = false;
  }
  if (root || !(meta & META_HAS_TERM)) return FID_NONE;
  return (meta & META_HAS_EDGES) ? tv.fids[2u * at + 1u] : term_inline;
}

template <class WidAt>
__device__ uint32_t exact_walk(const TableView& tv, uint32_t nlev, WidAt wid_at) {
  return exact_walk1(tv, tv.root_base, tv.root_meta, tv.root_hash_fid, nlev, wid_at);
}

constexpr uint32_t IT_TOPIC_SHIFT = 10;
constexpr uint32_t IT_DROOT = 1u << 16;
constexpr uint32_t IT_PLUS = 1u << 17;
constexpr uint32_t IT_NOLIT = 1u << 18;
constexpr uint32_t IT_PH = 1u << 19;
constexpr uint32_t IT_HASH_SHIFT = 20;

__device__ __forceinline__ uint2 make_item(uint32_t base, uint32_t meta, bool droot, bool nolit, uint32_t tl,
                                           uint32_t widx) {
  const bool ph = (meta & META_PH) != 0;
  const uint32_t caplog = meta & META_CAPLOG2_MASK;
  const uint32_t sd = (meta >> META_SEED_SHIFT) & 255u;
  const uint32_t hp = ph ? (caplog | (sd << 4)) : (caplog | (sd << 5));
  return make_uint2(base, widx | (tl << IT_TOPIC_SHIFT) | (droot ? IT_DROOT : 0u) |
                              ((meta & META_HAS_PLUS) ? IT_PLUS : 0u) | (nolit ? IT_NOLIT : 0u) |
                              (ph ? IT_PH : 0u) | (hp << IT_HASH_SHIFT));
}

__device__ __forceinline__ uint32_t item_topic(uint2 it) { return (it.y >> IT_TOPIC_SHIFT) & 63u; }

typedef uint32_t u32x4 __attribute__((ext_vector_type(4)));
__device__ __forceinline__ void load3_masked(const EdgeSlot* edges, uint32_t ip, uint32_t il, uint32_t ia, bool np,
                                             bool nl, bool na, Slot& p, Slot& l, Slot& a) {
  const uint64_t mp = __ballot(np), ml = __ballot(nl), ma = __ballot(na);
  const EdgeSlot* pp = edges + ip;
  const EdgeSlot* pl = edges + il;
  const EdgeSlot* pa = edges + ia;
  u32x4 vp = {WID_NONE, 0u, 0u, 0u}, vl = vp, va = vp;
  uint64_t save;
  asm volatile(
      "s_mov_b64 %[sv], exec\n\t"
      "s_and_b64 exec, %[sv], %[mp]\n\t"
      "global_load_dwordx4 %[p], %[ap], off\n\t"
      "s_and_b64 exec, %[sv], %[ml]\n\t"
      "global_load_dwordx4 %[l], %[al], off\n\t"
      "s_and_b64 exec, %[sv], %[ma]\n\t"
      "global_load_dwordx4 %[a], %[aa], off\n\t"
      "s_mov_b64 exec, %[sv]\n\t"
      "s_waitcnt vmcnt(0)"
      : [p] "+v"(vp), [l] "+v"(vl), [a] "+v"(va), [sv] "=&s"(save)
      : [ap] "v"(pp), [al] "v"(pl), [aa] "v"(pa), [mp] "s"(mp), [ml] "s"(ml), [ma] "s"(ma)
      : "memory");
  p.a = make_uint4(vp.x, vp.y, vp.z, vp.w);
  p.idx = ip;
  l.a = make_uint4(vl.x, vl.y, vl.z, vl.w);
  l.idx = il;
  a.a = make_uint4(va.x, va.y, va.z, va.w);
  a.idx = ia;
}

__device__ __forceinline__ void load6_masked(const EdgeSlot* edges, const uint32_t (&ip)[2], const uint32_t (&il)[2],
                                             const bool (&np)[2], const bool (&nl)[2], const bool (&na)[2],
                                             Slot (&p)[2], Slot (&l)[2], Slot (&a)[2]) {
  const uint64_t mp0 = __ballot(np[0]), ml0 = __ballot(nl[0]), ma0 = __ballot(na[0]);
  const uint64_t mp1 = __ballot(np[1]), ml1 = __ballot(nl[1]), ma1 = __ballot(na[1]);
  const EdgeSlot *pp0 = edges + ip[0], *pl0 = edges + il[0], *pa0 = edges + il[0] + 1;
  const EdgeSlot *pp1 = edges + ip[1], *pl1 = edges + il[1], *pa1 = edges + il[1] + 1;
  u32x4 vp0 = {WID_NONE, 0u, 0u, 0u}, vl0 = vp0, va0 = vp0, vp1 = vp0, vl1 = vp0, va1 = vp0;
  uint64_t save;
  asm volatile(
      "s_mov_b64 %[sv], exec\n\t"
      "s_and_b64 exec, %[sv], %[mp0]\n\t"
      "global_load_dwordx4 %[p0], %[ap0], off\n\t"
      "s_and_b64 exec, %[sv], %[ml0]\n\t"
      "global_load_dwordx4 %[l0], %[al0], off\n\t"
      "s_and_b64 exec, %[sv], %[ma0]\n\t"
      "global_load_dwordx4 %[a0], %[aa0], off\n\t"
      "s_and_b64 exec, %[sv], %[mp1]\n\t"
      "global_load_dwordx4 %[p1], %[ap1], off\n\t"
      "s_and_b64 exec, %[sv], %[ml1]\n\t"
      "global_load_dwordx4 %[l1], %[al1], off\n\t"
      "s_and_b64 exec, %[sv], %[ma1]\n\t"
      "global_load_dwordx4 %[a1], %[aa1], off\n\t"
      "s_mov_b64 exec, %[sv]\n\t"
      "s_waitcnt vmcnt(0)"
      : [p0] "+v"(vp0), [l0] "+v"(vl0), [a0] "+v"(va0), [p1] "+v"(vp1), [l1] "+v"(vl1), [a1] "+v"(va1),
        [sv] "=&s"(save)
      : [ap0] "v"(pp0), [al0] "v"(pl0), [aa0] "v"(pa0), [ap1] "v"(pp1), [al1] "v"(pl1), [aa1] "v"(pa1),
        [mp0] "s"(mp0), [ml0] "s"(ml0), [ma0] "s"(ma0), [mp1] "s"(mp1), [ml1] "s"(ml1), [ma1] "s"(ma1)
      : "memory");
  p[0].a = make_uint4(vp0.x, vp0.y, vp0.z, vp0.w);
  p[0].idx = ip[0];
  l[0].a = make_uint4(vl0.x, vl0.y, vl0.z, vl0.w);
  l[0].idx = il[0];
  a[0].a = make_uint4(va0.x, va0.y, va0.z, va0.w);
  a[0].idx = il[0] + 1;
  p[1].a = make_uint4(vp1.x, vp1.y, vp1.z, vp1.w);
  p[1].idx = ip[1];
  l[1].a = make_uint4(vl1.x, vl1.y, vl1.z, vl1.w);
  l[1].idx = il[1];
  a[1].a = make_uint4(va1.x, va1.y, va1.z, va1.w);
  a[1].idx = il[1] + 1;
}

template <int K, bool RL = false>
__device__ __forceinline__ void probe_items(const EdgeSlot* __restrict__ edges, uint32_t plus_mask,
                                            const uint32_t (&base)[K],
                                            const uint32_t (&hparams)[K], const bool (&isph)[K],
                                            const bool (&cpy)[K], const bool (&needL)[K], const uint32_t (&wid)[K],
                                            const bool (&needP)[K], Slot (&lit)[K], bool (&fL)[K],
                                            Slot (&pls)[K], bool (&fP)[K], uint32_t& extra,
                                            const uint4* rl = nullptr, uint32_t rsz = 0, uint32_t root_base = 0) {
  Slot alt[K];
  bool wide[K], again[K];
  uint32_t sdk[K], msk[K], atp[K], atl[K];
#pragma unroll
  for (int k = 0; k < K; ++k) {
    const uint32_t caplog = isph[k] ? (hparams[k] & 15u) : (hparams[k] & 31u);
    sdk[k] = isph[k] ? (hparams[k] >> 4) : (hparams[k] >> 5);
    const uint32_t mask = (1u << caplog) - 1u;
    msk[k] = mask;
    wide[k] = needL[k] && !isph[k];
    const uint32_t h = node_hash(wid[k], sdk[k]);
    const uint32_t i1 = isph[k] ? ph_slot(h, mask, cpy[k]) : wide_slot1(h, mask, cpy[k]);
    atp[k] = base[k] + (needL[k] ? plus_copy(i1, cpy[k]) : 0u);
    atl[k] = base[k] + i1;
  }
  if constexpr (K == 1 && RL) {
    const bool r = rsz != 0 && base[0] == root_base;
    load3_masked(edges, atp[0], atl[0], atl[0] + 1, needP[0] && !r, needL[0] && !r, wide[0] && !r, pls[0], lit[0],
                 alt[0]);
    if (r) {
      if (needP[0]) pls[0].a = rl[atp[0] - root_base];
      if (needL[0]) lit[0].a = rl[atl[0] - root_base];
      if (wide[0]) alt[0].a = rl[atl[0] + 1 - root_base];
    }
  } else if constexpr (K == 1) {
    load3_masked(edges, atp[0], atl[0], atl[0] + 1, needP[0], needL[0], wide[0], pls[0], lit[0], alt[0]);
  } else if constexpr (K == 2) {
    load6_masked(edges, atp, atl, needP, needL, wide, pls, lit, alt);
  } else {
#pragma unroll
    for (int k = 0; k < K; ++k) {
      pls[k] = empty_slot();
      lit[k] = pls[k];
      alt[k] = pls[k];
      if (needP[k]) pls[k] = load_slot(edges, atp[k]);
      if (needL[k]) lit[k] = load_slot(edges, atl[k]);
      if (wide[k]) alt[k] = load_slot(edges, atl[k] + 1);
    }
  }
  bool any_again = false;
#pragma unroll
  for (int k = 0; k < K; ++k) {
    fP[k] = needP[k] && pls[k].a.x == WID_PLUS;
    fL[k] = needL[k] && lit[k].a.x == wid[k];
    if (wide[k] && !fL[k] && alt[k].a.x == wid[k]) {
      lit[k] = alt[k];
      fL[k] = true;
    }
    again[k] = wide[k] && !fL[k] && (lit[k].a.z & META_BUCKET_OVF);
    any_again |= again[k];
  }
  if (__any(any_again)) {
#pragma unroll
    for (int k = 0; k < K; ++k) {
      if (!again[k]) continue;
      const uint32_t i2 = wide_slot(wid[k], sdk[k], msk[k], cpy[k], true);
      const Slot u = load_slot(edges, base[k] + i2), v = load_slot(edges, base[k] + i2 + 1);
      ++extra;
      if (u.a.x == wid[k]) { lit[k] = u; fL[k] = true; }
      else if (v.a.x == wid[k]) { lit[k] = v; fL[k] = true; }
    }
  }
}

}


struct ByteWin {
  const uint8_t* p;
  uint64_t lim;
  bool vec_ok;
  uint64_t wbase;
  uint4 w;
  __device__ __forceinline__ ByteWin(const uint8_t* p_, uint64_t lim_)
      : p(p_), lim(lim_), vec_ok((reinterpret_cast<uintptr_t>(p_) & 15u) == 0), wbase(~0ull),
        w(make_uint4(0, 0, 0, 0)) {}
  __device__ __forceinline__ uint32_t operator()(uint64_t i) {
    const uint64_t b = i & ~15ull;
    if (b != wbase) {
      wbase = b;
      if (vec_ok && b + 16 <= lim) {
        w = *reinterpret_cast<const uint4*>(p + b);
      } else {
        uint64_t lo = 0, hi = 0;
#pragma unroll
        for (int k = 0; k < 8; ++k) {
          if (b + k < lim) lo |= static_cast<uint64_t>(p[b + k]) << (8 * k);
          if (b + 8 + k < lim) hi |= static_cast<uint64_t>(p[b + 8 + k]) << (8 * k);
        }
        w = make_uint4(static_cast<uint32_t>(lo), static_cast<uint32_t>(lo >> 32), static_cast<uint32_t>(hi),
                       static_cast<uint32_t>(hi >> 32));
      }
    }
    const uint32_t j = static_cast<uint32_t>(i & 15u);
    const uint64_t lo = (static_cast<uint64_t>(w.y) << 32) | w.x;
    const uint64_t hi = (static_cast<uint64_t>(w.w) << 32) | w.z;
    const uint64_t q = (j & 8u) ? hi : lo;
    return static_cast<uint32_t>(q >> (8u * (j & 7u))) & 0xFFu;
  }
};

struct Chunk64 {
  const uint8_t* p;
  uint64_t lim;
  bool vec_ok;
  uint64_t cb;
  uint4 w0, w1, w2, w3;
  __device__ __forceinline__ Chunk64(const uint8_t* p_, uint64_t lim_)
      : p(p_), lim(lim_), vec_ok((reinterpret_cast<uintptr_t>(p_) & 15u) == 0), cb(~0ull) {}
  __device__ __forceinline__ static uint4 win(const uint8_t* p, uint64_t lim, bool vec_ok, uint64_t b) {
    if (vec_ok && b + 16 <= lim) return *reinterpret_cast<const uint4*>(p + b);
    uint32_t v[4] = {0, 0, 0, 0};
#pragma unroll
    for (uint32_t k = 0; k < 16; ++k)
      if (b + k < lim) v[k >> 2] |= static_cast<uint32_t>(p[b + k]) << (8u * (k & 3u));
    return make_uint4(v[0], v[1], v[2], v[3]);
  }
  __device__ __forceinline__ uint32_t dword(uint64_t i) {
    if (i < cb || i >= cb + 64) {
      cb = i & ~15ull;
      w0 = win(p, lim, vec_ok, cb);
      w1 = win(p, lim, vec_ok, cb + 16);
      w2 = win(p, lim, vec_ok, cb + 32);
      w3 = win(p, lim, vec_ok, cb + 48);
    }
    const uint32_t r = static_cast<uint32_t>(i - cb);
    const uint32_t q = r >> 4, d = (r >> 2) & 3u;
    return pick4(d, pick4(q, w0.x, w1.x, w2.x, w3.x), pick4(q, w0.y, w1.y, w2.y, w3.y),
                 pick4(q, w0.z, w1.z, w2.z, w3.z), pick4(q, w0.w, w1.w, w2.w, w3.w));
  }
  __device__ __forceinline__ static uint32_t pick4(uint32_t q, uint32_t a, uint32_t b, uint32_t c, uint32_t d) {
    return (q & 2u) ? ((q & 1u) ? d : c) : ((q & 1u) ? b : a);
  }
};

__device__ __forceinline__ uint32_t sel8(uint4 a, uint4 b, uint32_t i) {
  const uint32_t lo = Chunk64::pick4(i & 3u, a.x, a.y, a.z, a.w), hi = Chunk64::pick4(i & 3u, b.x, b.y, b.z, b.w);
  return (i & 4u) ? hi : lo;
}

__device__ __forceinline__ void word_head(uint4 wa, uint4 wb, uint32_t sh, uint32_t len, uint32_t (&w)[4]) {
#pragma unroll
  for (uint32_t o = 0; o < 4; ++o) {
    const uint32_t i = (sh >> 2) + o;
    const uint32_t v = __builtin_amdgcn_alignbyte(sel8(wa, wb, i + 1), sel8(wa, wb, i), sh & 3u);
    const uint32_t nb = len > 4 * o ? min(len - 4 * o, 4u) : 0u;
    w[o] = nb >= 4 ? v : (v & ((1u << (8 * nb)) - 1u));
  }
}

constexpr uint32_t AUX_LEN_SHIFT = 20;
constexpr uint64_t AUX_OFF_LIM = 1ull << AUX_LEN_SHIFT;
constexpr uint32_t AUX_LEN_MAX = 4095;
constexpr uint32_t WID_RESOLVED = 0xFFFFFFF0u;

__device__ __forceinline__ uint32_t byte_eq_mask(uint32_t x, uint32_t pat) {
  const uint32_t y = x ^ pat;
  const uint32_t z = ~(((y & 0x7F7F7F7Fu) + 0x7F7F7F7Fu) | y) & 0x80808080u;
  return (((z >> 7) * 0x204081u) >> 21) & 0xFu;
}

__device__ __forceinline__ uint32_t chunk_levelmap(uint4 v) {
  const uint32_t d[4] = {v.x, v.y, v.z, v.w};
  uint32_t m = 0;
#pragma unroll
  for (uint32_t i = 0; i < 4; ++i) {
    m |= byte_eq_mask(d[i], 0x2F2F2F2Fu) << (4 * i);
    m |= (byte_eq_mask(d[i], 0x2B2B2B2Bu) | byte_eq_mask(d[i], 0x23232323u)) << (16 + 4 * i);
  }
  return m;
}

__device__ __forceinline__ uint32_t span_mask(uint32_t k, uint32_t lo, uint32_t hi) {
  const uint32_t c = 16u * k;
  const uint32_t b0 = lo > c ? lo - c : 0u, b1 = min(hi - c, 16u);
  return ((1u << b1) - 1u) & ~((1u << b0) - 1u);
}

constexpr int ceil_log2(int v) { return v <= 1 ? 0 : 1 + ceil_log2((v + 1) / 2); }

template <int STACK_CAP, int WID_CAP>
struct FastLds {
  uint2 stack[STACK_CAP];
  uint32_t wids[WID_CAP];
  uint32_t wend[64];
  uint32_t cnt[64];
};

constexpr uint32_t PA_WIDS = 192;
template <int STACK_CAP, int WID_CAP, int K, bool DIAG, bool RL = false, int PA = 0, bool NH = true>
__device__ __forceinline__ void fast_tile(const MatchArgs& a, FastLds<STACK_CAP, WID_CAP>& L, uint64_t tile,
                                          uint32_t tt, const uint4* rl = nullptr, uint32_t rsz = 0) {
  static_assert(STACK_CAP >= 4 * 64 * K && STACK_CAP % 128 == 0, "stack must hold 4 pops");
  static_assert(WID_CAP <= 1024, "item word index is 10 bits");
  static_assert(PA == 0 || (!DIAG && PA_WIDS + WID_CAP <= 2 * 2048), "split tiles: no diagnostics; record fits the spill");
  const uint32_t lane = lane_id();
  const uint64_t t0 = tile * tt;
  if (t0 >= a.n) return;
  if (a.perm && (a.ctrl[CTRL_ERROR] & CTRL_ERR_ORDER_CAP)) return;
  const uint64_t clk0 = DIAG ? wall_clock64() : 0;

  const TableView& tv = a.tv;
  const uint32_t tcount = static_cast<uint32_t>(min<uint64_t>(tt, a.n - t0));
  const bool valid = lane < tcount;
  const uint64_t t = t0 + lane;
  uint64_t start = 0, end = 0;
  if (valid) {
    start = a.toffs[t];
    end = a.toffs[t + 1];
  }

  uint32_t nlev = 0, wbase = 0;
  bool wild = false, dollar = false, defer = false;
  uint64_t defer_mask = 0;
  if constexpr (PA == 2) {
    const uint32_t* pa = reinterpret_cast<const uint32_t*>(a.spill + tile * a.spill_cap);
    const uint32_t fl = pa[64 + lane];
    L.wend[lane] = pa[lane];
    const uint32_t nw = pa[128];
    for (uint32_t j = lane; j < nw; j += 64) L.wids[j] = pa[PA_WIDS + j];
    nlev = fl & 0xFFFFu;
    defer = valid && ((fl >> 16) & 1u);
    wild = (fl >> 17) & 1u;
    dollar = (fl >> 18) & 1u;
    wbase = fl >> 20;
    defer_mask = __ballot(defer);
    L.cnt[lane] = 0;
    wave_sync();
  } else {
  const uint64_t lim = a.toffs[a.n];
  const uint64_t A0 = a.toffs[t0] & ~15ull;
  const uint64_t tend = a.toffs[t0 + tcount];
  const bool vec_ok = (reinterpret_cast<uintptr_t>(a.tbytes) & 15u) == 0;
  constexpr uint32_t MAP_CHUNKS = 2 * STACK_CAP;
  const bool use_map = tend - A0 <= 16ull * MAP_CHUNKS;
  uint32_t* lmap = reinterpret_cast<uint32_t*>(L.stack);
  const uint32_t lo = static_cast<uint32_t>(start - A0), hi = static_cast<uint32_t>(end - A0);
  Chunk64 C(a.tbytes, lim);
  bool longw = false;
  if (use_map) {
    const uint32_t first = (valid && end > start) ? a.tbytes[start] : 0u;
    const uint32_t nch = static_cast<uint32_t>((tend - A0 + 15) >> 4);
    for (uint32_t c0 = 0; c0 < nch; c0 += 256) {
      uint4 v[4];
#pragma unroll
      for (uint32_t u = 0; u < 4; ++u) {
        const uint32_t c = c0 + lane + 64u * u;
        v[u] = c < nch ? Chunk64::win(a.tbytes, lim, vec_ok, A0 + 16ull * c) : make_uint4(0, 0, 0, 0);
      }
#pragma unroll
      for (uint32_t u = 0; u < 4; ++u) {
        const uint32_t c = c0 + lane + 64u * u;
        if (c < nch) lmap[c] = chunk_levelmap(v[u]);
      }
    }
    dollar = first == '$';
    wave_sync();
    if (valid) {
      uint32_t cnt = 0;
      for (uint32_t k = lo >> 4; 16u * k < hi; ++k) cnt += __popc(lmap[k] & span_mask(k, lo, hi));
      nlev = cnt + 1;
    }
  } else if (valid) {
    nlev = 1;
    uint32_t llen = 0, first = 0;
    for (uint64_t i = start & ~3ull; i < end; i += 4) {
      const uint32_t d = C.dword(i);
#pragma unroll
      for (uint32_t b = 0; b < 4; ++b) {
        const uint64_t pos = i + b;
        if (pos < start || pos >= end) continue;
        const uint32_t c = (d >> (8u * b)) & 0xFFu;
        if (pos == start) dollar = c == '$';
        if (c == '/') {
          longw |= llen >= AUX_LEN_MAX;
          ++nlev;
          llen = 0;
        } else {
          if (llen == 0) first = c;
          ++llen;
        }
      }
    }
    longw |= llen >= AUX_LEN_MAX;
  }
  defer = valid && (nlev > static_cast<uint32_t>(WID_CAP / 8) || longw || end - A0 >= AUX_OFF_LIM);
  const uint32_t need = (valid && !defer) ? nlev : 0u;
  const uint32_t incl = wave_incl_scan(need, lane);
  wbase = incl - need;
  if (valid && !defer && incl > static_cast<uint32_t>(WID_CAP)) defer = true;
  L.wend[lane] = incl;

  if (valid && !defer) {
    uint32_t j = wbase;
    uint64_t ws = start;
    auto put = [&](uint64_t wend_) {
      const uint32_t len = static_cast<uint32_t>(wend_ - ws);
      uint32_t v = static_cast<uint32_t>(ws - A0) | (len << AUX_LEN_SHIFT);
      if (len == 1) {
        const bool maybe = !use_map || ((lmap[(ws - A0) >> 4] >> (16u + ((ws - A0) & 15u))) & 1u);
        const uint32_t c = maybe ? static_cast<uint32_t>(a.tbytes[ws]) : 0u;
        v = c == '+' ? WID_PLUS : c == '#' ? WID_HASH : v;
      }
      v = len >= AUX_LEN_MAX ? WID_NONE : v;
      L.wids[j++] = v;
      return v;
    };
    uint32_t seen = 0;
    auto note = [](uint32_t v) -> uint32_t {
      return (v == WID_PLUS || v == WID_HASH ? 1u : 0u) | (v == WID_NONE ? 2u : 0u);
    };
    if (use_map) {
      for (uint32_t k = lo >> 4; 16u * k < hi; ++k) {
        uint32_t m = lmap[k] & span_mask(k, lo, hi);
        while (m) {
          const uint64_t pos = A0 + 16u * k + static_cast<uint32_t>(__builtin_ctz(m));
          m &= m - 1u;
          seen |= note(put(pos));
          ws = pos + 1;
        }
      }
    } else {
      for (uint64_t i = start & ~3ull; i < end; i += 4) {
        const uint32_t d = C.dword(i);
#pragma unroll
        for (uint32_t b = 0; b < 4; ++b) {
          const uint64_t pos = i + b;
          if (pos < start || pos >= end) continue;
          if (((d >> (8u * b)) & 0xFFu) == '/') {
            seen |= note(put(pos));
            ws = pos + 1;
          }
        }
      }
    }
    seen |= note(put(end));
    wild = (seen & 1u) != 0;
    longw = (seen & 2u) != 0;
  }
  uint32_t nwords = (valid && !defer) ? incl : 0u;
#pragma unroll
  for (uint32_t dd = 32; dd >= 1; dd >>= 1) nwords = max(nwords, static_cast<uint32_t>(__shfl_xor(nwords, dd, 64)));
  defer |= longw;
  defer_mask = __ballot(defer);
  wave_sync();

  constexpr uint32_t IW = 2;
  for (uint32_t j0 = 0; j0 < nwords; j0 += 64u * IW) {
    uint32_t jj[IW], ln[IW], sh[IW], hh[IW], w[IW][4];
    uint64_t wsa[IW];
    bool act[IW];
    uint4 wa[IW], wb[IW], hd[IW], in[IW];
#pragma unroll
    for (uint32_t u = 0; u < IW; ++u) {
      jj[u] = j0 + lane + 64u * u;
      const uint32_t v = jj[u] < nwords ? L.wids[jj[u]] : WID_NONE;
      act[u] = v < WID_RESOLVED;
      ln[u] = v >> AUX_LEN_SHIFT;
      wsa[u] = A0 + (v & (AUX_OFF_LIM - 1));
      sh[u] = static_cast<uint32_t>(wsa[u] & 15u);
      const uint64_t w0 = wsa[u] & ~15ull;
      wa[u] = (act[u] && ln[u]) ? Chunk64::win(a.tbytes, lim, vec_ok, w0) : make_uint4(0, 0, 0, 0);
      wb[u] = (act[u] && sh[u] + min(ln[u], 16u) > 16u) ? Chunk64::win(a.tbytes, lim, vec_ok, w0 + 16)
                                                         : make_uint4(0, 0, 0, 0);
    }
#pragma unroll
    for (uint32_t u = 0; u < IW; ++u) {
      word_head(wa[u], wb[u], sh[u], ln[u], w[u]);
      hh[u] = !act[u] ? 0u : ln[u] <= 16 ? word_hash16(ln[u], w[u][0], w[u][1], w[u][2], w[u][3])
                          : word_hash_bytes(a.tbytes + wsa[u], ln[u]);
      const uint4* vp = reinterpret_cast<const uint4*>(tv.vocab + (vocab_slot0(hh[u]) & tv.vocab_mask));
      hd[u] = act[u] ? vp[0] : make_uint4(0, 0, WID_NONE, 0);
      in[u] = act[u] ? vp[1] : make_uint4(0, 0, 0, 0);
    }
#pragma unroll
    for (uint32_t u = 0; u < IW; ++u) {
      if (!act[u]) continue;
      uint32_t wid;
      if (hd[u].z == WID_NONE) {
        wid = WID_NONE;
      } else if (hd[u].x == hh[u] && hd[u].y == ln[u] && ln[u] <= 16 && in[u].x == w[u][0] &&
                 in[u].y == w[u][1] && in[u].z == w[u][2] && in[u].w == w[u][3]) {
        wid = hd[u].z;
      } else {
        wid = intern_word(tv, hh[u], ln[u], w[u][0], w[u][1], w[u][2], w[u][3], a.tbytes, wsa[u]);
      }
      L.wids[jj[u]] = wid;
    }
  }
  L.cnt[lane] = 0;
  wave_sync();
  if constexpr (PA == 1) {
    uint32_t* pa = reinterpret_cast<uint32_t*>(a.spill + tile * a.spill_cap);
    pa[lane] = L.wend[lane];
    pa[64 + lane] = (nlev & 0xFFFFu) | (defer ? 1u << 16 : 0u) | (wild ? 1u << 17 : 0u) | (dollar ? 1u << 18 : 0u) |
                    ((wbase & 0xFFFu) << 20);
    if (lane == 0) pa[128] = nwords;
    for (uint32_t j = lane; j < nwords; j += 64) pa[PA_WIDS + j] = L.wids[j];
    return;
  }
  }
  const uint64_t clk1 = DIAG ? wall_clock64() : 0;

  uint64_t* slab = a.slab + tile * a.slab_cap;
  uint2* spill = a.spill + tile * a.spill_cap;
  const uint32_t cap = a.slab_cap;
  const uint32_t mode = a.mode;
  uint32_t cursor = 0;
  uint32_t top = 0;
  uint32_t stop = 0;
  uint32_t maxtop = 0;
  uint32_t evals = 0;
  uint32_t dg[DIAG_NCOUNT] = {};

  {
    bool e0 = false, e1 = false, push = false;
    uint32_t g1 = 0;
    uint2 it = make_uint2(0, 0);
    if (valid && !defer) {
      if (wild) {
        if (mode == MODE_ROUTES) {
          g1 = exact_walk(tv, nlev, [&](uint32_t k) { return L.wids[wbase + k]; });
          e1 = g1 != FID_NONE;
        }
      } else {
        evals = 1;
        e0 = !dollar && (tv.root_meta & META_HAS_HASH);
        if (tv.root_meta & META_HAS_EDGES) {
          push = true;
          const uint32_t rmeta = dollar ? (tv.root_meta & ~META_HAS_PLUS) : tv.root_meta;
          it = make_item(tv.root_base, rmeta, dollar, false, lane, wbase);
        }
      }
    }
    const uint32_t c = (e0 ? 1u : 0u) + (e1 ? 1u : 0u);
    uint32_t tot;
    uint32_t pos = wave_prefix<2>(c, lane, &tot);
    const uint64_t tag = static_cast<uint64_t>(lane) << 32;
    if (e0) { if (pos < cap) slab[pos] = tag | tv.root_hash_fid; ++pos; }
    if (e1) { if (pos < cap) slab[pos] = tag | g1; ++pos; }
    if (c) L.cnt[lane] = c;
    cursor = tot;
    uint32_t ptot;
    const uint32_t ppos = wave_prefix<2>(push ? 1u : 0u, lane, &ptot);
    if (push) L.stack[ppos] = it;
    top = ptot;
    maxtop = top;
    wave_sync();
  }

  if (DIAG && a.diag_stop) top = 0;
  constexpr uint32_t POP = 64u * K;
  constexpr uint32_t HALF = STACK_CAP / 2;
  while (true) {
    top = __builtin_amdgcn_readfirstlane(top);
    stop = __builtin_amdgcn_readfirstlane(stop);
    if (top < POP && stop > 0) {
      const uint32_t r = min(stop, HALF - (top < HALF ? top : HALF));
      for (uint32_t i = lane; i < r; i += 64) L.stack[top + i] = spill[stop - r + i];
      top += r;
      stop -= r;
      wave_sync();
    }
    if (top == 0) break;
    if (top + POP > static_cast<uint32_t>(STACK_CAP)) {
      if (stop + HALF <= a.spill_cap) {
        for (uint32_t i = lane; i < HALF; i += 64) spill[stop + i] = L.stack[i];
        for (uint32_t i0 = 0; i0 < top - HALF; i0 += 64) {
          const uint32_t i = i0 + lane;
          uint2 v = make_uint2(0, 0);
          if (i < top - HALF) v = L.stack[HALF + i];
          wave_sync();
          if (i < top - HALF) L.stack[i] = v;
          wave_sync();
        }
        stop += HALF;
        top -= HALF;
        if (DIAG) dg[8] += lane == 0 ? 1u : 0u;
      } else {
        uint64_t m = 0;
        for (uint32_t i = lane; i < top; i += 64) m |= 1ull << item_topic(L.stack[i]);
        for (uint32_t i = lane; i < stop; i += 64) m |= 1ull << item_topic(spill[i]);
        defer_mask |= wave_or64(m);
        top = 0;
        stop = 0;
        break;
      }
    }
    const uint32_t nb = min(POP, top);
    uint2 it[K];
    bool act[K], needL[K], needP[K], leaf[K], droot[K], isph[K];
    uint32_t wid[K], tl[K], widx[K], ibase[K], hpar[K];
#pragma unroll
    for (int k = 0; k < K; ++k) {
      const uint32_t idx = lane + 64u * k;
      act[k] = idx < nb;
      it[k] = act[k] ? L.stack[top - nb + idx] : make_uint2(0, 0);
    }
    top -= nb;
#pragma unroll
    for (int k = 0; k < K; ++k) {
      tl[k] = item_topic(it[k]);
      widx[k] = it[k].y & 1023u;
      droot[k] = (it[k].y & IT_DROOT) != 0;
      isph[k] = (it[k].y & IT_PH) != 0;
      hpar[k] = it[k].y >> IT_HASH_SHIFT;
      ibase[k] = it[k].x;
      wid[k] = act[k] ? L.wids[widx[k]] : WID_NONE;
      leaf[k] = act[k] && (widx[k] + 1 == L.wend[tl[k]]);
      needL[k] = act[k] && wid[k] != WID_NONE && !(it[k].y & IT_NOLIT);
      needP[k] = act[k] && (it[k].y & IT_PLUS);
    }
    wave_sync();
    Slot lit[K], pls[K];
    bool fL[K], fP[K];
    bool cpy[K];
#pragma unroll
    for (int k = 0; k < K; ++k)
      cpy[k] = plus_copies(tv.plus_mask, (it[k].y & IT_PLUS) || (droot[k] && (tv.root_meta & META_HAS_PLUS)),
                           isph[k] ? (hpar[k] & 15u) : (hpar[k] & 31u));
    uint32_t nw0[K];
    if constexpr (NH) {
#pragma unroll
      for (int k = 0; k < K; ++k) nw0[k] = act[k] ? L.wids[widx[k] + 1] : WID_NONE;
    }
    probe_items<K, RL>(tv.edges, tv.plus_mask, ibase, hpar, isph, cpy, needL, wid, needP, lit, fL, pls, fP, dg[4], rl,
                       rsz, tv.root_base);
    if (DIAG) {
#pragma unroll
      for (int k = 0; k < K; ++k) {
        dg[1] += act[k] ? 1u : 0u;
        dg[2] += needL[k] ? 1u : 0u;
        dg[3] += fL[k] ? 1u : 0u;
        dg[5] += needP[k] ? 1u : 0u;
        dg[6] += fP[k] ? 1u : 0u;
        if (act[k]) {
          const uint32_t lvl = widx[k] - (tl[k] ? L.wend[tl[k] - 1] : 0u);
#pragma unroll
          for (uint32_t q = 0; q < 8; ++q) dg[DIAG_LEVEL0 + q] += (lvl == q || (q == 7 && lvl > 7)) ? 1u : 0u;
          const uint32_t cl = isph[k] ? (hpar[k] & 15u) : (hpar[k] & 31u);
          dg[DIAG_SMALL] += cl <= 3 ? 1u : 0u;
          dg[DIAG_WIDE] += cl > 3 ? 1u : 0u;
        }
      }
      dg[0] += 1;
    }

    bool eLh[K], eLt[K], ePh[K], ePt[K], pL[K], pP[K], nlL[K], nlP[K];
    uint32_t ce[K], nwid[K], ecount = 0, pcount = 0;
#pragma unroll
    for (int k = 0; k < K; ++k) {
      evals += (fL[k] ? 1u : 0u) + (fP[k] ? 1u : 0u);
      eLh[k] = fL[k] && (lit[k].a.z & META_HAS_HASH);
      eLt[k] = fL[k] && leaf[k] && term_ok(lit[k].a.z, mode, droot[k]);
      ePh[k] = fP[k] && (pls[k].a.z & META_HAS_HASH);
      ePt[k] = fP[k] && leaf[k] && term_ok(pls[k].a.z, mode, false);
      pL[k] = fL[k] && !leaf[k] && (lit[k].a.z & META_HAS_EDGES);
      pP[k] = fP[k] && !leaf[k] && (pls[k].a.z & META_HAS_EDGES);
      nwid[k] = (pL[k] || pP[k]) ? (NH ? nw0[k] : L.wids[widx[k] + 1]) : WID_NONE;
      nlL[k] = nwid[k] == WID_NONE || !litf_may_contain(lit[k].a.z, lit[k].a.w, nwid[k]);
      nlP[k] = nwid[k] == WID_NONE || !litf_may_contain(pls[k].a.z, pls[k].a.w, nwid[k]);
      pL[k] = pL[k] && !(nlL[k] && !(lit[k].a.z & META_HAS_PLUS));
      pP[k] = pP[k] && !(nlP[k] && !(pls[k].a.z & META_HAS_PLUS));
      ce[k] = (eLh[k] ? 1u : 0u) + (eLt[k] ? 1u : 0u) + (ePh[k] ? 1u : 0u) + (ePt[k] ? 1u : 0u);
      ecount += ce[k];
      pcount += (pL[k] ? 1u : 0u) + (pP[k] ? 1u : 0u);
    }
    {
      uint32_t ptot;
      uint32_t pos = top + wave_prefix<ceil_log2(2 * K + 1)>(pcount, lane, &ptot);
#pragma unroll
      for (int k = 0; k < K; ++k) {
        if (pL[k]) L.stack[pos++] = make_item(lit[k].a.y, lit[k].a.z, false, nlL[k], tl[k], widx[k] + 1);
        if (pP[k]) L.stack[pos++] = make_item(pls[k].a.y, pls[k].a.z, false, nlP[k], tl[k], widx[k] + 1);
      }
      top += ptot;
      maxtop = max(maxtop, top + stop);
    }
    {
      uint32_t tot;
      uint32_t pos = cursor + wave_prefix<ceil_log2(4 * K + 1)>(ecount, lane, &tot);
#pragma unroll
      for (int k = 0; k < K; ++k) {
        const uint64_t tag = static_cast<uint64_t>(tl[k]) << 32;
        if (eLh[k]) { if (pos < cap) slab[pos] = tag | emit_value(lit[k], 0); ++pos; }
        if (eLt[k]) { if (pos < cap) slab[pos] = tag | emit_value(lit[k], 1); ++pos; }
        if (ePh[k]) { if (pos < cap) slab[pos] = tag | emit_value(pls[k], 0); ++pos; }
        if (ePt[k]) { if (pos < cap) slab[pos] = tag | emit_value(pls[k], 1); ++pos; }
        if (ce[k]) atomicAdd(&L.cnt[tl[k]], ce[k]);
      }
      cursor += tot;
      if (DIAG) dg[7] += ecount;
    }
    wave_sync();
  }

  wave_sync();
  if (DIAG && a.diag) {
    dg[0] = lane == 0 ? dg[0] : 0u;
    dg[8] = lane == 0 ? dg[8] : 0u;
    const uint64_t clk2 = wall_clock64();
    dg[9] = lane == 0 ? static_cast<uint32_t>(clk1 - clk0) : 0u;
    dg[10] = lane == 0 ? static_cast<uint32_t>(clk2 - clk1) : 0u;
    dg[11] = lane == 0 ? 1u : 0u;
    if (a.timeline && lane == 0)
      a.timeline[tile] = make_uint4(static_cast<uint32_t>(clk0), static_cast<uint32_t>(clk0 >> 32),
                                    static_cast<uint32_t>(clk1 - clk0) | (static_cast<uint32_t>(__smid()) << 20),
                                    static_cast<uint32_t>(clk2 - clk0));
#pragma unroll
    for (int i = 0; i < DIAG_NCOUNT; ++i) {
      const uint32_t v = wave_sum(dg[i]);
      if (lane == 0 && v) atomicAdd(reinterpret_cast<unsigned long long*>(a.diag + i), static_cast<unsigned long long>(v));
    }
  }
  const uint32_t mine = (valid && !((defer_mask >> lane) & 1ull)) ? L.cnt[lane] : 0u;
  if (valid) a.counts[t] = mine;
  const uint32_t ev = wave_sum(evals);
  const uint32_t tsum = wave_sum(mine);
  if (lane == 0) {
    a.tile_sum[tile] = tsum;
    a.tile_stats[tile] = make_uint2(ev, maxtop);
    a.tile_fill[tile] = cursor;
    a.tile_defer[tile] = defer_mask;
    if (cursor > cap) atomicMax(&a.ctrl[CTRL_NEED_SLAB], cursor);
  }
  if (defer_mask) {
    uint32_t pos0 = 0;
    if (lane == 0) pos0 = atomicAdd(&a.ctrl[CTRL_DEFERRED], static_cast<uint32_t>(__popcll(defer_mask)));
    pos0 = __shfl(pos0, 0, 64);
    if ((defer_mask >> lane) & 1ull)
      a.deferred[pos0 + __popcll(defer_mask & lanemask_lt(lane))] = static_cast<uint32_t>(t);
  }
}

constexpr uint32_t ROOT_LDS_SLOTS = 256;

constexpr int fast_waves_hint(int K, int WC) { return K == 1 ? (WC == 448 ? 7 : 8) : 5; }
template <int WAVES, int STACK_CAP, int WID_CAP, int K, bool DIAG, bool RL = false, int PA = 0, bool NH = true>
__global__ __launch_bounds__(WAVES * 64, fast_waves_hint(K, WID_CAP)) void match_fast_kernel(MatchArgs a) {
  __shared__ FastLds<STACK_CAP, WID_CAP> lds_all[WAVES];
  __shared__ uint4 rl[RL ? ROOT_LDS_SLOTS : 1];
  const uint32_t wv = threadIdx.x >> 6;
  uint32_t rsz = 0;
  if constexpr (RL) {
    const TableView& tv = a.tv;
    const uint32_t cl = (tv.root_meta & META_PH) ? (tv.root_meta & 15u) : (tv.root_meta & META_CAPLOG2_MASK);
    const uint32_t n = (tv.root_meta & META_HAS_EDGES) ? (1u << cl) : 0u;
    rsz = n <= ROOT_LDS_SLOTS ? n : 0u;
    const uint4* src = reinterpret_cast<const uint4*>(tv.edges + tv.root_base);
    for (uint32_t i = threadIdx.x; i < rsz; i += blockDim.x) rl[i] = src[i];
    __syncthreads();
  }
  uint64_t blk = blockIdx.x;
  if (a.deal) {
    const uint32_t nb = gridDim.x, x = blockIdx.x & 7u, j = blockIdx.x >> 3, q = nb >> 3, r = nb & 7u;
    blk = static_cast<uint64_t>(x) * q + min(x, r) + j;
  }
  fast_tile<STACK_CAP, WID_CAP, K, DIAG, RL, PA, NH>(a, lds_all[wv], blk * WAVES + wv, TILE_TOPICS, rl, rsz);
}

__device__ __forceinline__ void deep_walk(const MatchArgs& a, uint32_t gw, uint32_t nwaves, uint32_t tt) {
  const uint32_t lane = lane_id();
  const TableView& tv = a.tv;
  const uint32_t ndef = __hip_atomic_load(&a.ctrl[CTRL_DEFERRED], __ATOMIC_RELAXED, __HIP_MEMORY_SCOPE_AGENT);
  uint32_t* wids = a.deep_wids + static_cast<uint64_t>(gw) * DEEP_MAX_LEVELS;
  uint4* stack = a.deep_stack + static_cast<uint64_t>(gw) * a.deep_stack_cap;
  const uint32_t scap = a.deep_stack_cap;
  const uint32_t mode = a.mode;

  uint32_t ccur = 0, cend = 0;
  auto pad_chunk = [&]() {
    for (uint32_t p = ccur + lane; p < cend; p += 64)
      if (p < a.deep_slab_cap) a.deep_slab[p] = DEEP_PAD;
    ccur = cend;
  };
  for (uint32_t j = gw; j < ndef; j += nwaves) {
    const uint32_t t = a.deferred[j];
    if (lane == 0) a.deep_rank[j] = 0;
    const uint64_t start = a.toffs[t], end = a.toffs[t + 1];
    if (end - start > 65535u) {
      if (lane == 0) {
        atomicOr(&a.ctrl[CTRL_ERROR], CTRL_ERR_TOO_LONG);
        a.counts[t] = 0;
      }
      continue;
    }
    auto byte_at = [&](uint64_t i) -> uint32_t { return a.tbytes[i]; };
    uint32_t nlev = 0, wild = 0, dollar = 0;
    if (lane == 0) {
      uint32_t k = 0, len = 0, w0 = 0, w1 = 0, w2 = 0, w3 = 0;
      uint64_t ws = start;
      for (uint64_t i = start; i <= end; ++i) {
        const uint32_t c = (i < end) ? byte_at(i) : static_cast<uint32_t>('/');
        if (c != '/') {
          if (len < 16) {
            const uint32_t v = c << (8u * (len & 3u));
            const uint32_t q = len >> 2;
            w0 |= q == 0 ? v : 0u;
            w1 |= q == 1 ? v : 0u;
            w2 |= q == 2 ? v : 0u;
            w3 |= q == 3 ? v : 0u;
          }
          ++len;
        } else {
          uint32_t wid;
          if (len == 1 && w0 == '+') { wid = WID_PLUS; wild = 1; }
          else if (len == 1 && w0 == '#') { wid = WID_HASH; wild = 1; }
          else {
            const uint32_t h = len <= 16 ? word_hash16(len, w0, w1, w2, w3) : word_hash_bytes(a.tbytes + ws, len);
            wid = intern_word(tv, h, len, w0, w1, w2, w3, a.tbytes, ws);
          }
          wids[k++] = wid;
          len = 0;
          w0 = w1 = w2 = w3 = 0;
          ws = i + 1;
        }
      }
      nlev = k;
      dollar = (end > start && byte_at(start) == '$') ? 1u : 0u;
    }
    __threadfence_block();
    nlev = __shfl(nlev, 0, 64);
    wild = __shfl(wild, 0, 64);
    dollar = __shfl(dollar, 0, 64);
    uint32_t count = 0, evals = 0;

    auto emit = [&](bool e0, uint64_t g0, bool e1, uint64_t g1, bool e2, uint64_t g2, bool e3, uint64_t g3) {
      const uint32_t c = (e0 ? 1u : 0u) + (e1 ? 1u : 0u) + (e2 ? 1u : 0u) + (e3 ? 1u : 0u);
      uint32_t tot;
      const uint32_t rel = wave_prefix<3>(c, lane, &tot);
      if (tot == 0) return;
      if (ccur + tot > cend) {
        pad_chunk();
        const uint32_t want = max(tot, DEEP_CHUNK);
        uint32_t base = 0;
        if (lane == 0) base = atomicAdd(&a.ctrl[CTRL_DEEP_FILL], want);
        ccur = __shfl(base, 0, 64);
        cend = ccur + want;
      }
      uint32_t pos = ccur + rel;
      ccur += tot;
      const uint64_t tag = static_cast<uint64_t>(j) << 32;
      bool over = false;
      if (e0) { if (pos < a.deep_slab_cap) a.deep_slab[pos] = tag | g0; else over = true; ++pos; }
      if (e1) { if (pos < a.deep_slab_cap) a.deep_slab[pos] = tag | g1; else over = true; ++pos; }
      if (e2) { if (pos < a.deep_slab_cap) a.deep_slab[pos] = tag | g2; else over = true; ++pos; }
      if (e3) { if (pos < a.deep_slab_cap) a.deep_slab[pos] = tag | g3; else over = true; ++pos; }
      if (over) atomicOr(&a.ctrl[CTRL_ERROR], CTRL_ERR_DEEP_SLAB);
      count += tot;
    };

    uint32_t top = 0;
    if (wild) {
      if (mode == MODE_ROUTES) {
        uint32_t f = FID_NONE;
        if (lane == 0) f = exact_walk(tv, nlev, [&](uint32_t k) { return wids[k]; });
        f = __shfl(f, 0, 64);
        emit(lane == 0 && f != FID_NONE, f, false, 0, false, 0, false, 0);
      }
    } else {
      if (lane == 0) evals = 1;
      const bool eh = lane == 0 && !dollar && (tv.root_meta & META_HAS_HASH);
      emit(eh, tv.root_hash_fid, false, 0, false, 0, false, 0);
      if (tv.root_meta & META_HAS_EDGES) {
        const uint32_t rmeta = dollar ? (tv.root_meta & ~META_HAS_PLUS) : tv.root_meta;
        if (lane == 0)
          stack[top] = make_uint4(tv.root_base, rmeta, 0u, dollar ? 1u : 0u);
        top += 1;
      }
    }
    __threadfence_block();

    while (top > 0) {
      const uint32_t nb = min(64u, min(top, scap - top));
      if (nb == 0) {
        if (lane == 0) atomicOr(&a.ctrl[CTRL_ERROR], CTRL_ERR_TOO_DEEP);
        break;
      }
      const bool act = lane < nb;
      uint4 q = make_uint4(0, 0, 0, 0);
      if (act) q = stack[top - nb + lane];
      top -= nb;
      __threadfence_block();
      const bool droot = (q.w & 1u) != 0;
      const uint32_t widx = q.z;
      const uint32_t qbase[1] = {q.x};
      const bool qph[1] = {(q.y & META_PH) != 0};
      const uint32_t qsd = (q.y >> META_SEED_SHIFT) & 255u;
      const uint32_t qhp[1] = {qph[0] ? ((q.y & 15u) | (qsd << 4)) : ((q.y & META_CAPLOG2_MASK) | (qsd << 5))};
      const uint32_t w[1] = {act ? wids[widx] : WID_NONE};
      const bool leaf = act && widx + 1 == nlev;
      const bool nL[1] = {act && w[0] != WID_NONE};
      const bool nP[1] = {act && (q.y & META_HAS_PLUS) != 0};
      Slot lit[1], pls[1];
      bool fL[1], fP[1];
      uint32_t extra = 0;
      const bool qcp[1] = {plus_copies(tv.plus_mask, (q.y & META_HAS_PLUS) || (droot && (tv.root_meta & META_HAS_PLUS)),
                                       q.y & META_CAPLOG2_MASK)};
      probe_items<1>(tv.edges, tv.plus_mask, qbase, qhp, qph, qcp, nL, w, nP, lit, fL, pls, fP, extra);
      evals += (fL[0] ? 1u : 0u) + (fP[0] ? 1u : 0u);
      const uint32_t m0 = lit[0].a.z, m1 = pls[0].a.z;
      const bool e0 = fL[0] && (m0 & META_HAS_HASH), e1 = fL[0] && leaf && term_ok(m0, mode, droot);
      const bool e2 = fP[0] && (m1 & META_HAS_HASH), e3 = fP[0] && leaf && term_ok(m1, mode, false);
      emit(e0, emit_value(lit[0], 0), e1, emit_value(lit[0], 1), e2, emit_value(pls[0], 0), e3,
           emit_value(pls[0], 1));
      const bool p0 = fL[0] && !leaf && (m0 & META_HAS_EDGES);
      const bool p1 = fP[0] && !leaf && (m1 & META_HAS_EDGES);
      uint32_t ptot;
      const uint32_t ppos = wave_prefix<2>((p0 ? 1u : 0u) + (p1 ? 1u : 0u), lane, &ptot);
      if (p0) stack[top + ppos] = make_uint4(lit[0].a.y, m0, widx + 1, 0u);
      if (p1) stack[top + ppos + (p0 ? 1u : 0u)] = make_uint4(pls[0].a.y, m1, widx + 1, 0u);
      top += ptot;
      __threadfence_block();
    }
    const uint32_t ev = wave_sum(evals);
    if (lane == 0) {
      a.counts[t] = count;
      if (count) atomicAdd(reinterpret_cast<unsigned long long*>(a.tile_sum + t / tt),
                           static_cast<unsigned long long>(count));
      atomicAdd(a.ctrl + CTRL_DEEP_EVALS, ev);
    }
  }
  pad_chunk();
}

__global__ __launch_bounds__(256) void match_deep_kernel(MatchArgs a) {
  const uint32_t gw = (blockIdx.x * blockDim.x + threadIdx.x) >> 6;
  if (gw >= a.deep_waves) return;
  deep_walk(a, gw, a.deep_waves, TILE_TOPICS);
}

namespace {
constexpr int SCAN_THREADS = 256;
constexpr int SCAN_ITEMS = 8;
constexpr int SCAN_TILE = SCAN_THREADS * SCAN_ITEMS;

__device__ __forceinline__ uint64_t block_excl_scan(uint64_t v, uint64_t* total) {
  __shared__ uint64_t wsum[SCAN_THREADS / 64];
  const uint32_t lane = threadIdx.x & 63, w = threadIdx.x >> 6;
  const uint64_t incl = wave_incl_scan64(v, lane);
  if (lane == 63) wsum[w] = incl;
  __syncthreads();
  uint64_t before = 0, all = 0;
  for (uint32_t k = 0; k < SCAN_THREADS / 64; ++k) {
    if (k < w) before += wsum[k];
    all += wsum[k];
  }
  __syncthreads();
  *total = all;
  return before + incl - v;
}
}

__global__ __launch_bounds__(SCAN_THREADS) void scan_reduce_kernel(const uint32_t* counts, uint64_t n,
                                                                   uint64_t* partials) {
  const uint64_t base = static_cast<uint64_t>(blockIdx.x) * SCAN_TILE;
  uint64_t s = 0;
  for (int k = 0; k < SCAN_ITEMS; ++k) {
    const uint64_t i = base + static_cast<uint64_t>(k) * SCAN_THREADS + threadIdx.x;
    if (i < n) s += counts[i];
  }
  uint64_t tot;
  block_excl_scan(s, &tot);
  if (threadIdx.x == 0) partials[blockIdx.x] = tot;
}

__global__ __launch_bounds__(SCAN_THREADS) void scan_partials_kernel(uint64_t* partials, uint64_t nb,
                                                                     uint64_t* offsets, uint64_t n) {
  uint64_t carry = 0;
  for (uint64_t b0 = 0; b0 < nb; b0 += SCAN_THREADS) {
    const uint64_t i = b0 + threadIdx.x;
    const uint64_t v = i < nb ? partials[i] : 0;
    uint64_t tot;
    const uint64_t ex = block_excl_scan(v, &tot);
    if (i < nb) partials[i] = carry + ex;
    carry += tot;
  }
  if (threadIdx.x == 0) offsets[n] = carry;
}

__global__ __launch_bounds__(SCAN_THREADS) void scan_final_kernel(const uint32_t* counts, uint64_t n,
                                                                  const uint64_t* partials,
                                                                  uint64_t* offsets) {
  const uint64_t base = static_cast<uint64_t>(blockIdx.x) * SCAN_TILE + static_cast<uint64_t>(threadIdx.x) * SCAN_ITEMS;
  uint32_t v[SCAN_ITEMS];
  uint64_t s = 0;
#pragma unroll
  for (int k = 0; k < SCAN_ITEMS; ++k) {
    const uint64_t i = base + k;
    v[k] = i < n ? counts[i] : 0u;
    s += v[k];
  }
  uint64_t tot;
  uint64_t run = partials[blockIdx.x] + block_excl_scan(s, &tot);
#pragma unroll
  for (int k = 0; k < SCAN_ITEMS; ++k) {
    const uint64_t i = base + k;
    if (i < n) offsets[i] = run;
    run += v[k];
  }
}

__global__ __launch_bounds__(SCAN_THREADS) void scan_single_kernel(const uint32_t* counts, uint64_t n,
                                                                   uint64_t* offsets) {
  const uint64_t base = static_cast<uint64_t>(threadIdx.x) * SCAN_ITEMS;
  uint32_t v[SCAN_ITEMS];
  uint64_t s = 0;
#pragma unroll
  for (int k = 0; k < SCAN_ITEMS; ++k) {
    const uint64_t i = base + k;
    v[k] = i < n ? counts[i] : 0u;
    s += v[k];
  }
  uint64_t tot;
  uint64_t run = block_excl_scan(s, &tot);
#pragma unroll
  for (int k = 0; k < SCAN_ITEMS; ++k) {
    const uint64_t i = base + k;
    if (i < n) offsets[i] = run;
    run += v[k];
  }
  if (threadIdx.x == 0) offsets[n] = tot;
}

__device__ __forceinline__ uint64_t wave_sum64(uint64_t v) {
#pragma unroll
  for (uint32_t d = 32; d >= 1; d >>= 1)
    v += (static_cast<uint64_t>(__shfl_xor(static_cast<uint32_t>(v >> 32), d, 64)) << 32) |
         __shfl_xor(static_cast<uint32_t>(v), d, 64);
  return v;
}

__global__ __launch_bounds__(GROUP_TILES) void group_reduce_kernel(MatchArgs a, uint64_t ntiles) {
  __shared__ uint64_t ws[GROUP_TILES / 64], we[GROUP_TILES / 64];
  __shared__ uint32_t wm[GROUP_TILES / 64];
  const uint32_t lane = threadIdx.x & 63, w = threadIdx.x >> 6;
  const uint64_t i = static_cast<uint64_t>(blockIdx.x) * GROUP_TILES + threadIdx.x;
  uint64_t v = 0, ev = 0;
  uint32_t mx = 0;
  if (i < ntiles) {
    v = a.tile_sum[i];
    const uint2 st = a.tile_stats[i];
    ev = st.x;
    mx = st.y;
  }
  v = wave_sum64(v);
  ev = wave_sum64(ev);
  for (uint32_t d = 32; d >= 1; d >>= 1) mx = max(mx, static_cast<uint32_t>(__shfl_xor(mx, d, 64)));
  if (lane == 0) {
    ws[w] = v;
    we[w] = ev;
    wm[w] = mx;
  }
  __syncthreads();
  if (threadIdx.x == 0) {
    uint64_t sv = 0, se = 0;
    uint32_t sm = 0;
    for (uint32_t k = 0; k < GROUP_TILES / 64; ++k) {
      sv += ws[k];
      se += we[k];
      sm = max(sm, wm[k]);
    }
    a.group_sum[blockIdx.x] = sv;
    a.group_stats[blockIdx.x] = make_uint2(static_cast<uint32_t>(min<uint64_t>(se, 0xFFFFFFFFull)), sm);
  }
}

__device__ __forceinline__ void scatter_tile(const MatchArgs& a, uint64_t tile, uint64_t off);

__global__ __launch_bounds__(256) void scatter_fast_kernel(MatchArgs a) {
  const uint32_t lane = lane_id();
  const uint32_t wv = threadIdx.x >> 6;
  const uint64_t tile = static_cast<uint64_t>(blockIdx.x) * 4 + wv;
  const uint64_t t0 = tile * TILE_TOPICS;
  if (t0 >= a.n) return;
  const uint64_t t = t0 + lane;
  uint64_t off = 0;
  if (a.perm) {
    if (a.ctrl[CTRL_ERROR] & CTRL_ERR_ORDER_CAP) return;
    off = t < a.n ? a.out_off[a.perm[t]] : 0;
  } else {
    const uint64_t g = tile / GROUP_TILES, g0 = g * GROUP_TILES;
    uint64_t before = 0;
    for (uint64_t k = lane; k < g; k += 64) before += a.group_sum[k];
    for (uint64_t j = g0 + lane; j < tile; j += 64) before += a.tile_sum[j];
    before = wave_sum64(before);
    const uint64_t c = t < a.n ? a.counts[t] : 0;
    off = before + wave_incl_scan64(c, lane) - c;
    if (t < a.n) a.out_off[t] = off;
  }
  scatter_tile(a, tile, off);
}

__device__ __forceinline__ void scatter_tile(const MatchArgs& a, uint64_t tile, uint64_t off) {
  const uint32_t lane = lane_id();
  uint64_t next = off;
  const uint32_t fill = min(a.tile_fill[tile], a.slab_cap);
  const uint64_t dmask = a.tile_defer[tile];
  const uint64_t* slab = a.slab + tile * a.slab_cap;
  const uint64_t lt = lanemask_lt(lane);
  constexpr uint32_t U = 4;
  for (uint32_t i0 = 0; i0 < fill; i0 += 64 * U) {
    uint64_t e[U];
    uint32_t id[U];
#pragma unroll
    for (uint32_t u = 0; u < U; ++u) {
      const uint32_t i = i0 + 64 * u + lane;
      e[u] = i < fill ? slab[i] : ~0ull;
    }
#pragma unroll
    for (uint32_t u = 0; u < U; ++u) id[u] = e[u] != ~0ull ? resolve_entry(a.tv, e[u]) : 0u;
#pragma unroll
    for (uint32_t u = 0; u < U; ++u) {
      const uint32_t tl = static_cast<uint32_t>(e[u] >> 32) & 63u;
      const bool keep = e[u] != ~0ull && !((dmask >> tl) & 1ull);
      const uint64_t km = __ballot(keep);
      uint64_t peers = km, mine = km;
#pragma unroll
      for (uint32_t bit = 0; bit < 6; ++bit) {
        const uint64_t m = __ballot(keep && ((tl >> bit) & 1u));
        peers &= ((tl >> bit) & 1u) ? m : ~m;
        mine &= ((lane >> bit) & 1u) ? m : ~m;
      }
      const uint32_t rk = static_cast<uint32_t>(__popcll(peers & lt));
      const uint32_t lo = __shfl(static_cast<uint32_t>(next), static_cast<int>(tl), 64);
      const uint32_t hi = __shfl(static_cast<uint32_t>(next >> 32), static_cast<int>(tl), 64);
      if (keep) {
        const uint64_t p = ((static_cast<uint64_t>(hi) << 32) | lo) + rk;
        if (p < a.out_cap) a.out_ids[p] = id[u];
      }
      next += static_cast<uint64_t>(__popcll(mine));
    }
  }
}

__global__ __launch_bounds__(64) void summary_kernel(MatchArgs a) {
  const uint32_t lane = lane_id();
  uint64_t tot = 0, ev = 0;
  uint32_t mx = 0;
  for (uint32_t k = lane; k < a.ngroups; k += 64) {
    tot += a.group_sum[k];
    const uint2 st = a.group_stats[k];
    ev += st.x;
    mx = max(mx, st.y);
  }
  tot = wave_sum64(tot);
  ev = wave_sum64(ev);
  for (uint32_t d = 32; d >= 1; d >>= 1) mx = max(mx, static_cast<uint32_t>(__shfl_xor(mx, d, 64)));
  if (lane == 0) {
    const uint32_t* c = a.ctrl;
    const uint32_t need = c[CTRL_NEED_SLAB], err = c[CTRL_ERROR];
    uint64_t flags = 0;
    if (need > a.slab_cap || (err & (CTRL_ERR_DEEP_SLAB | CTRL_ERR_TOO_DEEP | CTRL_ERR_ORDER_CAP))) flags |= SUM_F_RETRY;
    if (tot > a.out_cap) flags |= SUM_F_OVERFLOW;
    if (err & CTRL_ERR_TOO_LONG) flags |= SUM_F_ERROR;
    a.out_off[a.n] = tot;
    uint64_t* sm = a.summary;
    sm[SUM_TOTAL] = tot;
    sm[SUM_EVALS] = ev + c[CTRL_DEEP_EVALS];
    sm[SUM_MAXSTACK] = mx;
    sm[SUM_DEFERRED] = c[CTRL_DEFERRED];
    sm[SUM_NEED_SLAB] = need;
    sm[SUM_DEEP_FILL] = c[CTRL_DEEP_FILL];
    sm[SUM_ERROR] = err;
    sm[SUM_FLAGS] = flags;
    __threadfence_system();
  }
}

__global__ __launch_bounds__(256) void scatter_deep_kernel(MatchArgs a) {
  const uint32_t fill = min(a.ctrl[CTRL_DEEP_FILL], a.deep_slab_cap);
  for (uint64_t i = static_cast<uint64_t>(blockIdx.x) * blockDim.x + threadIdx.x; i < fill;
       i += static_cast<uint64_t>(gridDim.x) * blockDim.x) {
    const uint64_t e = a.deep_slab[i];
    if (e == DEEP_PAD) continue;
    const uint32_t j = static_cast<uint32_t>(e >> 32) & 0x7FFFFFFFu;
    const uint32_t t = a.deferred[j];
    const uint64_t p = a.out_off[a.perm ? a.perm[t] : t] + atomicAdd(&a.deep_rank[j], 1u);
    if (p < a.out_cap) a.out_ids[p] = resolve_entry(a.tv, e);
  }
}

__global__ __launch_bounds__(256) void csr_to_host_kernel(const uint64_t* __restrict__ d_off, uint64_t n,
                                                          const uint32_t* __restrict__ d_ids, uint64_t cap,
                                                          uint64_t* h_off, uint32_t* h_ids) {
  const uint64_t tid = static_cast<uint64_t>(blockIdx.x) * blockDim.x + threadIdx.x;
  const uint64_t nt = static_cast<uint64_t>(gridDim.x) * blockDim.x;
  const uint64_t total = min(d_off[n], cap);
  const uint64_t no2 = (n + 1) / 2;
  for (uint64_t i = tid; i < no2; i += nt)
    reinterpret_cast<uint4*>(h_off)[i] = reinterpret_cast<const uint4*>(d_off)[i];
  if (tid == 0 && ((n + 1) & 1)) h_off[n] = d_off[n];
  const uint64_t nv = total / 4;
  for (uint64_t i = tid; i < nv; i += nt)
    reinterpret_cast<uint4*>(h_ids)[i] = reinterpret_cast<const uint4*>(d_ids)[i];
  if (tid < total - 4 * nv) h_ids[4 * nv + tid] = d_ids[4 * nv + tid];
}

__global__ __launch_bounds__(256) void shard_owner_kernel(const uint8_t* __restrict__ tbytes,
                                                          const uint64_t* __restrict__ toffs, uint64_t n,
                                                          uint32_t world, uint32_t levels,
                                                          uint32_t* __restrict__ owner) {
  for (uint64_t i = static_cast<uint64_t>(blockIdx.x) * blockDim.x + threadIdx.x; i < n;
       i += static_cast<uint64_t>(gridDim.x) * blockDim.x) {
    const uint64_t a = toffs[i], b = toffs[i + 1];
    owner[i] = shard_owner(tbytes + a, b - a, world, levels, true);
  }
}

__global__ void slot_patch_kernel(EdgeSlot* edges, uint32_t* fids, const SlotPatch* patches, uint32_t n,
                                  int phase) {
  for (uint32_t i = blockIdx.x * blockDim.x + threadIdx.x; i < n; i += gridDim.x * blockDim.x) {
    const SlotPatch& p = patches[i];
    if (phase == 0) {
      *reinterpret_cast<uint2*>(fids + 2ull * p.slot) = make_uint2(p.fid_h, p.fid_t);
    } else {
      *reinterpret_cast<uint4*>(edges + p.slot) = make_uint4(p.s.wid, p.s.child_base, p.s.meta, p.s.litf);
    }
  }
}

namespace {

__device__ __forceinline__ uint64_t small_block_scan(uint64_t v, uint64_t* total, uint64_t* wsum) {
  const uint32_t lane = lane_id(), w = threadIdx.x >> 6;
  const uint64_t incl = wave_incl_scan64(v, lane);
  if (lane == 63) wsum[w] = incl;
  __syncthreads();
  uint64_t before = 0, all = 0;
  for (uint32_t k = 0; k < SMALL_WAVES; ++k) {
    before += k < w ? wsum[k] : 0;
    all += wsum[k];
  }
  __syncthreads();
  *total = all;
  return before + incl - v;
}

__device__ __forceinline__ void small_phase_barrier() {
  __syncthreads();
}

__device__ __forceinline__ uint32_t small_floor(const uint32_t* v, uint32_t n, uint32_t x) {
  uint32_t lo = 0, hi = n;
  while (hi - lo > 1) {
    const uint32_t mid = (lo + hi) >> 1;
    if (v[mid] <= x) lo = mid; else hi = mid;
  }
  return lo;
}

}

__global__ __launch_bounds__(SMALL_WAVES * 64) void small_batch_kernel(SmallArgs sa) {
  constexpr int SC = 384, WC = 640;
  struct FoLds {
    uint32_t D[SMALL_FO_MAX_ENTRIES + 1];
    uint32_t off[SMALL_MAX_N + 1];
  };
  union Lds {
    FastLds<SC, WC> w[SMALL_WAVES];
    FoLds f;
  };
  __shared__ Lds lds;
  __shared__ uint64_t wsum[SMALL_WAVES];
  const MatchArgs& a = sa.m;
  const uint32_t tid = threadIdx.x, lane = lane_id(), wv = tid >> 6;
  constexpr uint32_t NT = SMALL_WAVES * 64;
  const uint64_t n = a.n;
  uint64_t* const clk = sa.clk;
  uint64_t tprev = clk ? wall_clock64() : 0;
  auto mark = [&](uint32_t k) {
    if (clk && tid == 0) {
      const uint64_t now = wall_clock64();
      atomicAdd(reinterpret_cast<unsigned long long*>(clk + k), static_cast<unsigned long long>(now - tprev));
      tprev = now;
    }
  };
  auto finish = [&](uint32_t k) {
    if (!clk) return;
    __syncthreads();
    mark(k);
    if (tid == 0) atomicAdd(reinterpret_cast<unsigned long long*>(clk + SMALL_CLK_LAUNCHES), 1ull);
  };

  if (tid < CTRL_WORDS) a.ctrl[tid] = 0;
  {
    uint64_t* toffs = const_cast<uint64_t*>(a.toffs);
    uint4* tb = reinterpret_cast<uint4*>(const_cast<uint8_t*>(a.tbytes));
    const uint4* hb = reinterpret_cast<const uint4*>(sa.h_tbytes);
    const uint64_t nch = (sa.nbytes + 15) / 16;
    for (uint64_t i = tid; i <= n; i += NT) toffs[i] = sa.h_toffs[i];
    for (uint64_t i = tid; i < nch; i += NT) tb[i] = hb[i];
    if (sa.has_fanout && sa.f.h_keys)
      for (uint64_t i = tid; i < n; i += NT) sa.f.d_keys[i] = sa.f.h_keys[i];
  }
  small_phase_barrier();
  mark(SMALL_CLK_COPY);

  const uint32_t tt = sa.tt;
  const uint64_t ntiles = (n + tt - 1) / tt;
  if (wv < ntiles) fast_tile<SC, WC, 1, false>(a, lds.w[wv], wv, tt);
  small_phase_barrier();
  mark(SMALL_CLK_WALK);
  auto ctrl = [&](uint32_t k) { return __hip_atomic_load(&a.ctrl[k], __ATOMIC_RELAXED, __HIP_MEMORY_SCOPE_AGENT); };
  if (ctrl(CTRL_DEFERRED)) deep_walk(a, wv, SMALL_WAVES, tt);
  small_phase_barrier();
  mark(SMALL_CLK_DEEP);

  uint64_t* sm = a.summary;
  const uint32_t need = ctrl(CTRL_NEED_SLAB), err = ctrl(CTRL_ERROR);
  uint64_t flags = 0;
  if (need > a.slab_cap || (err & (CTRL_ERR_DEEP_SLAB | CTRL_ERR_TOO_DEEP))) flags |= SUM_F_RETRY;
  if (err & CTRL_ERR_TOO_LONG) flags |= SUM_F_ERROR;

  uint64_t total = 0;
  {
    const uint64_t c = (tid < n && !flags) ? a.counts[tid] : 0;
    const uint64_t ex = small_block_scan(c, &total, wsum);
    if (tid < n) a.out_off[tid] = ex;
    if (tid == 0) a.out_off[n] = total;
  }
  if (total > a.out_cap) flags |= SUM_F_OVERFLOW;
  small_phase_barrier();
  mark(SMALL_CLK_SCAN);
  if (!(flags & (SUM_F_RETRY | SUM_F_ERROR))) {
    if (wv < ntiles) {
      const uint64_t t = uint64_t(wv) * tt + lane;
      scatter_tile(a, wv, (lane < tt && t < n) ? a.out_off[t] : 0);
    }
    const uint32_t fill = min(ctrl(CTRL_DEEP_FILL), a.deep_slab_cap);
    for (uint32_t i = tid; i < fill; i += NT) {
      const uint64_t e = a.deep_slab[i];
      if (e == DEEP_PAD) continue;
      const uint32_t j = static_cast<uint32_t>(e >> 32) & 0x7FFFFFFFu;
      const uint64_t p = a.out_off[a.deferred[j]] + atomicAdd(&a.deep_rank[j], 1u);
      if (p < a.out_cap) a.out_ids[p] = resolve_entry(a.tv, e);
    }
  }
  small_phase_barrier();
  mark(SMALL_CLK_SCATTER);
  if (tid == 0) {
    uint64_t ev = ctrl(CTRL_DEEP_EVALS);
    uint32_t mx = 0;
    for (uint64_t k = 0; k < ntiles; ++k) {
      const uint2 st = a.tile_stats[k];
      ev += st.x;
      mx = max(mx, st.y);
    }
    sm[SUM_TOTAL] = total;
    sm[SUM_EVALS] = ev;
    sm[SUM_MAXSTACK] = mx;
    sm[SUM_DEFERRED] = ctrl(CTRL_DEFERRED);
    sm[SUM_NEED_SLAB] = need;
    sm[SUM_DEEP_FILL] = ctrl(CTRL_DEEP_FILL);
    sm[SUM_ERROR] = err;
    sm[SUM_FLAGS] = flags;
  }

  if (sa.h_out_off) {
    if (!(flags & (SUM_F_RETRY | SUM_F_ERROR))) {
      const uint64_t no2 = (n + 1) / 2;
      for (uint64_t i = tid; i < no2; i += NT)
        reinterpret_cast<uint4*>(sa.h_out_off)[i] = reinterpret_cast<const uint4*>(a.out_off)[i];
      if (tid == 0 && ((n + 1) & 1)) sa.h_out_off[n] = a.out_off[n];
      const uint64_t ids = min(total, sa.h_cap), nv = ids / 4;
      for (uint64_t i = tid; i < nv; i += NT)
        reinterpret_cast<uint4*>(sa.h_out_ids)[i] = reinterpret_cast<const uint4*>(a.out_ids)[i];
      if (tid < ids - 4 * nv) sa.h_out_ids[4 * nv + tid] = a.out_ids[4 * nv + tid];
    }
    finish(SMALL_CLK_OUT);
    return;
  }
  if (!sa.has_fanout) {
    finish(SMALL_CLK_OUT);
    return;
  }

  const SmallFanout& f = sa.f;
  const uint64_t m = total;
  if (flags || m > SMALL_FO_MAX_ENTRIES) {
    if (tid == 0) {
      f.h_sum[FO_SUM_FLAGS] = flags ? FO_SUM_F_MATCH : FO_SUM_F_SMALL;
      f.h_sum[FO_SUM_TOTAL] = 0;
      f.h_sum[FO_SUM_ENTRIES] = m;
      f.h_sum[FO_SUM_STATE] = f.ps_count ? *f.ps_count : 0;
    }
    finish(SMALL_CLK_OUT);
    return;
  }
  uint32_t* D = lds.f.D;
  uint32_t* off = lds.f.off;
  for (uint64_t t = tid; t <= n; t += NT) off[t] = static_cast<uint32_t>(a.out_off[t]);
  small_phase_barrier();
  constexpr uint32_t FU = 4;
  uint64_t T = 0;
  for (uint32_t r0 = 0; r0 < m; r0 += FU * NT) {
    uint32_t fid[FU], c[FU];
    uint4 rec[FU];
#pragma unroll
    for (uint32_t u = 0; u < FU; ++u) {
      const uint32_t e = r0 + u * NT + tid;
      fid[u] = e < m ? a.out_ids[e] : 0xFFFFFFFFu;
    }
#pragma unroll
    for (uint32_t u = 0; u < FU; ++u) rec[u] = fid[u] < f.n_recs ? f.recs[2u * fid[u]] : make_uint4(0, 0, 0, 0);
#pragma unroll
    for (uint32_t u = 0; u < FU; ++u) {
      const uint32_t e = r0 + u * NT + tid;
      c[u] = e < m ? fo_rec_plain(rec[u]) + fo_rec_groups(rec[u]) : 0u;
      if (e < m) {
        f.erec[e] = rec[u];
        f.etop[e] = small_floor(off, static_cast<uint32_t>(n), e);
      }
    }
#pragma unroll
    for (uint32_t u = 0; u < FU; ++u) {
      const uint32_t e = r0 + u * NT + tid;
      if (r0 + u * NT >= m) break;
      uint64_t tc;
      const uint64_t ex = small_block_scan(c[u], &tc, wsum);
      if (e < m) D[e] = static_cast<uint32_t>(T + ex);
      T += tc;
    }
  }
  if (tid == 0) D[m] = static_cast<uint32_t>(min<uint64_t>(T, 0xFFFFFFFFull));
  small_phase_barrier();
  mark(SMALL_CLK_FO_PASS1);
  for (uint64_t t = tid; t <= n; t += NT) f.h_off[t] = t < n ? D[off[t]] : T;
  const bool fits = T <= f.cap;
  if (fits) {
    const bool hash = f.strategy == 3u || f.strategy == 4u;
    for (uint64_t j0 = 0; j0 < T; j0 += FU * NT) {
      uint32_t e[FU], r[FU], fid[FU], sub[FU], key[FU];
      bool ok[FU], grp[FU];
      uint4 rec[FU], g[FU];
#pragma unroll
      for (uint32_t u = 0; u < FU; ++u) {
        const uint64_t j = j0 + u * NT + tid;
        ok[u] = j < T;
        e[u] = ok[u] ? small_floor(D, static_cast<uint32_t>(m), static_cast<uint32_t>(j)) : 0u;
        r[u] = ok[u] ? static_cast<uint32_t>(j) - D[e[u]] : 0u;
      }
#pragma unroll
      for (uint32_t u = 0; u < FU; ++u) {
        rec[u] = ok[u] ? f.erec[e[u]] : make_uint4(0, 0, 0, 0);
        fid[u] = ok[u] ? a.out_ids[e[u]] : 0u;
        key[u] = ok[u] && hash ? f.d_keys[f.etop[e[u]]] : 0u;
      }
#pragma unroll
      for (uint32_t u = 0; u < FU; ++u) {
        const uint32_t np = rec[u].y & ~FO_INLINE_BIT;
        grp[u] = ok[u] && r[u] >= np;
        sub[u] = 0;
        g[u] = make_uint4(0, 0, 0, 0);
        if (ok[u] && !grp[u]) {
          const bool inl = (rec[u].y & FO_INLINE_BIT) != 0;
          sub[u] = (inl && r[u] < FO_INLINE_HEAD)
                       ? fo_inline_head(rec[u], r[u])
                       : *(inl ? reinterpret_cast<const uint32_t*>(f.recs + 2u * fid[u] + 1u) + (r[u] - FO_INLINE_HEAD)
                               : f.plain + rec[u].x + r[u]);
        }
        if (grp[u]) g[u] = f.groups[rec[u].z + (r[u] - np)];
      }
#pragma unroll
      for (uint32_t u = 0; u < FU; ++u) {
        if (!grp[u]) continue;
        const uint32_t np = rec[u].y & ~FO_INLINE_BIT;
        const uint32_t gidx = rec[u].z + (r[u] - np);
        const uint32_t idx = g[u].y <= 1 ? 0u : fo_stateless_index(f.strategy, key[u], f.seed, e[u], gidx, g[u].y);
        sub[u] = f.members[g[u].x + idx];
      }
#pragma unroll
      for (uint32_t u = 0; u < FU; ++u) {
        if (!ok[u]) continue;
        const uint64_t j = j0 + u * NT + tid;
        f.h_subs[j] = sub[u];
        f.h_fil[j] = grp[u] ? (fid[u] | FANOUT_SHARED_BIT) : fid[u];
      }
    }
  }
  if (tid == 0) {
    f.h_sum[FO_SUM_FLAGS] = fits ? 0 : FO_SUM_F_OVERFLOW;
    f.h_sum[FO_SUM_TOTAL] = T;
    f.h_sum[FO_SUM_ENTRIES] = m;
    f.h_sum[FO_SUM_STATE] = f.ps_count ? *f.ps_count : 0;
  }
  finish(SMALL_CLK_FO_PASS2);
}

template <int W, int S, int WC, int K, bool RL = false, bool NH = true>
static void launch_fast_t(const MatchArgs& a, uint64_t ntiles, hipStream_t s) {
  const uint64_t grid = (ntiles + W - 1) / W;
  if (a.diag)
    hipLaunchKernelGGL((match_fast_kernel<W, S, WC, K, true, RL, 0, NH>), dim3(static_cast<uint32_t>(grid)),
                       dim3(W * 64), 0, s, a);
  else
    hipLaunchKernelGGL((match_fast_kernel<W, S, WC, K, false, RL, 0, NH>), dim3(static_cast<uint32_t>(grid)),
                       dim3(W * 64), 0, s, a);
}

hipError_t launch_match_fast(const MatchArgs& a, FastVariant v, hipStream_t s) {
  const uint64_t ntiles = (a.n + TILE_TOPICS - 1) / TILE_TOPICS;
  if (ntiles == 0) return hipSuccess;
  switch (v) {
    case FAST_K1_S1K: launch_fast_t<4, 1024, 1024, 1>(a, ntiles, s); break;
    case FAST_K2_S1K: launch_fast_t<4, 1024, 1024, 2>(a, ntiles, s); break;
    case FAST_K2_S2K: launch_fast_t<2, 2048, 1024, 2>(a, ntiles, s); break;
    case FAST_K2_S768: launch_fast_t<4, 768, 768, 2>(a, ntiles, s); break;
    case FAST_K4_S2K: launch_fast_t<2, 2048, 1024, 4>(a, ntiles, s); break;
    case FAST_K1_S256: launch_fast_t<4, 256, 512, 1>(a, ntiles, s); break;
    case FAST_K2_S512: launch_fast_t<4, 512, 640, 2>(a, ntiles, s); break;
    case FAST_K1_S384: launch_fast_t<4, 384, 640, 1>(a, ntiles, s); break;
    case FAST_K2_S512W: launch_fast_t<4, 512, 512, 2>(a, ntiles, s); break;
    case FAST_K1_S768W: launch_fast_t<4, 768, 1024, 1>(a, ntiles, s); break;
    case FAST_K1_S512W: launch_fast_t<4, 512, 1024, 1>(a, ntiles, s); break;
    case FAST_K1_S384R: launch_fast_t<4, 384, 640, 1, true>(a, ntiles, s); break;
    case FAST_K1_S384N: launch_fast_t<4, 384, 640, 1, false, false>(a, ntiles, s); break;
    case FAST_K1_S384W7: launch_fast_t<4, 384, 448, 1>(a, ntiles, s); break;
    case FAST_K1_S384B2: launch_fast_t<2, 384, 640, 1>(a, ntiles, s); break;
    case FAST_K1_S384B1: launch_fast_t<1, 384, 640, 1>(a, ntiles, s); break;
    case FAST_K1_S512WB1: launch_fast_t<1, 512, 1024, 1>(a, ntiles, s); break;
    case FAST_K1_S384P: {
      if (a.diag) {
        launch_fast_t<4, 384, 640, 1>(a, ntiles, s);
        break;
      }
      const dim3 grid(static_cast<uint32_t>((ntiles + 3) / 4));
      hipLaunchKernelGGL((match_fast_kernel<4, 384, 640, 1, false, false, 1>), grid, dim3(256), 0, s, a);
      hipLaunchKernelGGL((match_fast_kernel<4, 384, 640, 1, false, false, 2>), grid, dim3(256), 0, s, a);
      break;
    }
    default: return hipErrorInvalidValue;
  }
  return hipGetLastError();
}

hipError_t launch_small_batch(const SmallArgs& a, hipStream_t s) {
  const uint64_t tiles = a.tt ? (a.m.n + a.tt - 1) / a.tt : 0;
  if (a.m.n == 0 || a.m.n > SMALL_MAX_N || a.tt == 0 || a.tt > TILE_TOPICS || tiles > SMALL_WAVES ||
      tiles > a.slab_tiles)
    return hipErrorInvalidValue;
  hipLaunchKernelGGL(small_batch_kernel, dim3(1), dim3(SMALL_WAVES * 64), 0, s, a);
  return hipGetLastError();
}

hipError_t launch_match_deep(const MatchArgs& a, hipStream_t s) {
  const uint32_t blocks = (a.deep_waves * 64 + 255) / 256;
  hipLaunchKernelGGL(match_deep_kernel, dim3(blocks), dim3(256), 0, s, a);
  return hipGetLastError();
}

uint64_t scan_partials(uint64_t n) { return (n + SCAN_TILE - 1) / SCAN_TILE + 1; }

hipError_t launch_scan(const uint32_t* counts, uint64_t n, uint64_t* offsets, uint64_t* partials,
                       hipStream_t s) {
  const uint64_t nb = (n + SCAN_TILE - 1) / SCAN_TILE;
  if (nb <= 1) {
    hipLaunchKernelGGL(scan_single_kernel, dim3(1), dim3(SCAN_THREADS), 0, s, counts, n, offsets);
    return hipGetLastError();
  }
  hipLaunchKernelGGL(scan_reduce_kernel, dim3(static_cast<uint32_t>(nb)), dim3(SCAN_THREADS), 0, s, counts, n, partials);
  hipLaunchKernelGGL(scan_partials_kernel, dim3(1), dim3(SCAN_THREADS), 0, s, partials, nb, offsets, n);
  hipLaunchKernelGGL(scan_final_kernel, dim3(static_cast<uint32_t>(nb)), dim3(SCAN_THREADS), 0, s, counts, n, partials, offsets);
  return hipGetLastError();
}

hipError_t launch_assemble(const MatchArgs& a, hipStream_t s) {
  const uint64_t ntiles = (a.n + TILE_TOPICS - 1) / TILE_TOPICS;
  if (ntiles) {
    hipLaunchKernelGGL(group_reduce_kernel, dim3(a.ngroups), dim3(GROUP_TILES), 0, s, a, ntiles);
    if (a.perm) {
      hipError_t err = launch_order_counts(a.counts, a.perm, a.n, a.corig, s);
      if (err == hipSuccess) err = launch_scan(a.corig, a.n, a.out_off, a.partials, s);
      if (err != hipSuccess) return err;
    }
    hipLaunchKernelGGL(scatter_fast_kernel, dim3(static_cast<uint32_t>((ntiles + 3) / 4)), dim3(256), 0, s, a);
  }
  hipLaunchKernelGGL(scatter_deep_kernel, dim3(64), dim3(256), 0, s, a);
  hipLaunchKernelGGL(summary_kernel, dim3(1), dim3(64), 0, s, a);
  return hipGetLastError();
}

hipError_t launch_csr_to_host(const uint64_t* d_off, uint64_t n, const uint32_t* d_ids, uint64_t cap,
                               uint64_t* h_off, uint32_t* h_ids, hipStream_t s) {
  const uint64_t work = std::max<uint64_t>((n + 1) / 2, cap / 4);
  const uint32_t blocks = static_cast<uint32_t>(std::min<uint64_t>((work + 255) / 256 + 1, 2048));
  hipLaunchKernelGGL(csr_to_host_kernel, dim3(blocks), dim3(256), 0, s, d_off, n, d_ids, cap, h_off, h_ids);
  return hipGetLastError();
}

hipError_t launch_shard_owner(const uint8_t* tbytes, const uint64_t* toffs, uint64_t n, uint32_t world,
                              uint32_t levels, uint32_t* owner, hipStream_t s) {
  if (!n) return hipSuccess;
  const uint32_t blocks = static_cast<uint32_t>(std::min<uint64_t>((n + 255) / 256, 4096));
  hipLaunchKernelGGL(shard_owner_kernel, dim3(blocks), dim3(256), 0, s, tbytes, toffs, n, world, levels, owner);
  return hipGetLastError();
}

hipError_t launch_slot_patches(EdgeSlot* edges, uint32_t* fids, const SlotPatch* patches, uint32_t n,
                               hipStream_t s) {
  if (!n) return hipSuccess;
  const dim3 grid(std::min<uint32_t>((n + 255) / 256, 1024));
  hipLaunchKernelGGL(slot_patch_kernel, grid, dim3(256), 0, s, edges, fids, patches, n, 0);
  hipLaunchKernelGGL(slot_patch_kernel, grid, dim3(256), 0, s, edges, fids, patches, n, 1);
  return hipGetLastError();
}

}
```

Before: 1.822 billion topics/s.

## Narrow slab entries to 32-bit and resolve filter ids at emit time

```diff
diff --git a/emqx_amd/csrc/engine.cpp b/emqx_amd/csrc/engine.cpp
--- a/emqx_amd/csrc/engine.cpp
+++ b/emqx_amd/csrc/engine.cpp
@@ -72,6 +72,7 @@
   TableView tv{};
   uint64_t n_nodes = 0, n_slots = 0, n_words = 0, bytes = 0;
   uint32_t max_depth = 0;
+  bool narrow = false;
 };
 
 struct LiveState {
@@ -98,12 +99,13 @@
   hipStream_t stream = nullptr;
   hipStream_t last_stream = nullptr;
   hipEvent_t ev0 = nullptr, ev1 = nullptr, evk = nullptr;
-  uint64_t cap_n = 0, cap_tiles = 0, cap_slab = 0;
+  uint64_t cap_n = 0, cap_tiles = 0;
+  uint64_t cap_slab = 0;
   uint32_t slab_per_tile = 256;
   uint32_t* counts = nullptr;
   uint32_t* deferred = nullptr;
   uint32_t* deep_rank = nullptr;
-  uint64_t* slab = nullptr;
+  uint8_t* slab = nullptr;
   uint32_t* tile_fill = nullptr;
   uint64_t* tile_defer = nullptr;
   uint2* spill = nullptr;
@@ -262,6 +264,9 @@
   s->n_words = ht.n_words;
   s->max_depth = ht.max_depth;
   s->bytes = dt->bytes();
+  uint32_t max_id = 0;
+  for (uint32_t x : e->store.ext) max_id = std::max(max_id, x);
+  s->narrow = slab_narrow_ok(max_id);
 
   LiveState& d = e->ls;
   d.device = e->device;
@@ -292,6 +297,10 @@
   } else if (creates && 2 * (d.inserted + creates) > d.base_live) {
     return EMQX_NEED_FULL;
   }
+
+  if (e->snap->narrow)
+    for (uint32_t id : ids)
+      if (!slab_narrow_ok(fs.ext[id])) return EMQX_NEED_FULL;
 
   const uint64_t nw0 = d.vocab->n_words(), arena0 = d.vocab->arena.size();
   auto th0 = std::chrono::steady_clock::now();
@@ -395,7 +404,7 @@
   e->free_ws.push_back(w);
 }
 
-int ensure_ws(Workspace* w, uint64_t n) {
+int ensure_ws(Workspace* w, uint64_t n, uint64_t entry_bytes) {
   if (!w->stream) {
     HIP_TRY(hipStreamCreateWithFlags(&w->stream, hipStreamNonBlocking));
     HIP_TRY(hipEventCreate(&w->ev0));
@@ -433,7 +442,7 @@
     HIP_TRY(dalloc(w->spill, cap * w->spill_cap));
     w->cap_tiles = cap;
   }
-  const uint64_t need_slab = std::max<uint64_t>(ntiles, 1) * w->slab_per_tile;
+  const uint64_t need_slab = std::max<uint64_t>(ntiles, 1) * w->slab_per_tile * entry_bytes;
   if (need_slab > w->cap_slab) {
     const uint64_t cap = need_slab;
     HIP_TRY(dalloc(w->slab, cap));
@@ -501,6 +510,7 @@
   a.slab_cap = w->slab_per_tile;
   a.counts = w->counts;
   a.slab = w->slab;
+  a.narrow = snap.narrow ? 1u : 0u;
   a.tile_fill = w->tile_fill;
   a.tile_defer = w->tile_defer;
   a.spill = w->spill;
@@ -529,10 +539,14 @@
   return a;
 }
 
+uint64_t slab_entry_bytes(const Snapshot& snap) {
+  return snap.narrow ? sizeof(SlabNarrow::T) : sizeof(SlabWide::T);
+}
+
 int enqueue_match(emqx_engine* e, const Snapshot& snap, Workspace* w, uint32_t mode, const uint8_t* d_tbytes,
                   const uint64_t* d_toffs, uint64_t n, uint64_t* d_out_off, uint32_t* d_out_ids, uint64_t cap,
                   uint64_t* summary, hipStream_t s) {
-  int rc = ensure_ws(w, n);
+  int rc = ensure_ws(w, n, slab_entry_bytes(snap));
   if (rc != EMQX_OK) return rc;
   MatchArgs a = match_args(e, snap, w, mode, d_tbytes, d_toffs, n, d_out_off, d_out_ids, cap, summary);
   const bool ordered = use_order(e, snap, n);
@@ -668,16 +682,17 @@
                   const uint64_t* h_toffs, uint64_t n, uint64_t nbytes, uint8_t* d_tbytes, uint64_t* d_toffs,
                   uint64_t* d_out_off, uint32_t* d_out_ids, uint64_t cap, uint64_t* summary, uint64_t* h_out_off,
                   uint32_t* h_out_ids, uint64_t h_cap, const SmallFanout* f, hipStream_t s) {
-  int rc = ensure_ws(w, SMALL_MAX_N);
+  int rc = ensure_ws(w, SMALL_MAX_N, sizeof(SlabWide::T));
   if (rc != EMQX_OK) return rc;
   SmallArgs sa{};
   sa.m = match_args(e, snap, w, mode, d_tbytes, d_toffs, n, d_out_off, d_out_ids, cap, summary);
   sa.m.diag = nullptr;
+  sa.m.narrow = 0;
   sa.h_tbytes = h_tbytes;
   sa.h_toffs = h_toffs;
   sa.nbytes = nbytes;
   sa.tt = static_cast<uint32_t>((n + SMALL_WAVES - 1) / SMALL_WAVES);
-  sa.slab_tiles = static_cast<uint32_t>(std::min<uint64_t>(w->cap_slab / w->slab_per_tile, w->cap_tiles));
+  sa.slab_tiles = static_cast<uint32_t>(std::min<uint64_t>(w->cap_slab / (sizeof(SlabWide::T) * w->slab_per_tile), w->cap_tiles));
   sa.h_out_off = h_out_off;
   sa.h_out_ids = h_out_ids;
   sa.h_cap = h_cap;
@@ -778,7 +793,7 @@
   if (nbytes) HIP_TRY(hipMemcpyAsync(p->d_tbytes, b->topic_bytes, nbytes, hipMemcpyHostToDevice, s));
   HIP_TRY(hipMemcpyAsync(p->d_toffs, b->topic_offsets, (n + 1) * sizeof(uint64_t), hipMemcpyHostToDevice, s));
   Workspace* w = acquire_ws(e, s);
-  int rc = ensure_ws(w, n);
+  int rc = ensure_ws(w, n, slab_entry_bytes(*p->snap));
   if (rc == EMQX_OK)
     rc = enqueue_match(e, *p->snap, w, p->mode, p->d_tbytes, p->d_toffs, n, p->d_out_off, p->d_out_ids, b->cap_ids,
                        sum_dev, s);
@@ -805,7 +820,7 @@
   uint64_t total = p->summary[SUM_TOTAL];
   if (flags & SUM_F_RETRY) {
     Workspace* w = acquire_ws(p->e, p->stream);
-    int rc = ensure_ws(w, b->n);
+    int rc = ensure_ws(w, b->n, slab_entry_bytes(*p->snap));
     if (rc == EMQX_OK)
       rc = run_match(p->e, *p->snap, w, p->mode, p->d_tbytes, p->d_toffs, b->n, p->d_out_off, p->d_out_ids,
                      b->cap_ids, &total, p->stream);
@@ -985,7 +1000,7 @@
   HIP_TRY(hipSetDevice(e->device));
   auto snap = current(e);
   Workspace* w = acquire_ws(e, static_cast<hipStream_t>(stream));
-  int rc = ensure_ws(w, n);
+  int rc = ensure_ws(w, n, slab_entry_bytes(*snap));
   if (rc == EMQX_OK) {
     hipStream_t s = stream ? static_cast<hipStream_t>(stream) : w->stream;
     if (!stream && after_null_stream(s) != hipSuccess) rc = EMQX_EDEVICE;
@@ -1005,7 +1020,7 @@
   HIP_TRY(hipSetDevice(e->device));
   auto snap = current(e);
   Workspace* w = acquire_ws(e, static_cast<hipStream_t>(stream));
-  int rc = ensure_ws(w, n);
+  int rc = ensure_ws(w, n, slab_entry_bytes(*snap));
   if (rc == EMQX_OK) {
     hipStream_t s = stream ? static_cast<hipStream_t>(stream) : w->stream;
     if (!stream && after_null_stream(s) != hipSuccess) rc = EMQX_EDEVICE;
diff --git a/emqx_amd/csrc/kernels.h b/emqx_amd/csrc/kernels.h
--- a/emqx_amd/csrc/kernels.h
+++ b/emqx_amd/csrc/kernels.h
@@ -67,7 +67,8 @@
   uint32_t mode;
   uint32_t slab_cap;
   uint32_t* counts;
-  uint64_t* slab;
+  void* slab;
+  uint32_t narrow;
   uint32_t* tile_fill;
   uint64_t* tile_defer;
   uint32_t* ctrl;
diff --git a/emqx_amd/csrc/layout.h b/emqx_amd/csrc/layout.h
--- a/emqx_amd/csrc/layout.h
+++ b/emqx_amd/csrc/layout.h
@@ -39,6 +39,24 @@
 };
 static_assert(sizeof(EdgeSlot) == 16, "EdgeSlot must be 16 bytes");
 constexpr uint64_t MAX_SLOTS = (1ull << 31) - 1;
+
+constexpr uint32_t SLAB_NARROW_ID_BITS = 26;
+constexpr uint32_t SLAB_NARROW_IDS = (1u << SLAB_NARROW_ID_BITS) - 1u;
+EMQX_HD bool slab_narrow_ok(uint32_t max_id) { return max_id < SLAB_NARROW_IDS; }
+struct SlabWide {
+  typedef uint64_t T;
+  static constexpr T PAD = ~0ull;
+  static EMQX_HD T make(uint32_t owner, uint32_t id) { return (static_cast<uint64_t>(owner) << 32) | id; }
+  static EMQX_HD uint32_t owner(T e) { return static_cast<uint32_t>(e >> 32) & 63u; }
+  static EMQX_HD uint32_t id(T e) { return static_cast<uint32_t>(e); }
+};
+struct SlabNarrow {
+  typedef uint32_t T;
+  static constexpr T PAD = ~0u;
+  static EMQX_HD T make(uint32_t owner, uint32_t id) { return (owner << SLAB_NARROW_ID_BITS) | id; }
+  static EMQX_HD uint32_t owner(T e) { return e >> SLAB_NARROW_ID_BITS; }
+  static EMQX_HD uint32_t id(T e) { return e & ((1u << SLAB_NARROW_ID_BITS) - 1u); }
+};
 
 struct alignas(16) SlotPatch {
   uint32_t slot;
diff --git a/emqx_amd/csrc/match_kernels.hip b/emqx_amd/csrc/match_kernels.hip
--- a/emqx_amd/csrc/match_kernels.hip
+++ b/emqx_amd/csrc/match_kernels.hip
@@ -95,6 +95,13 @@
 
 __device__ __forceinline__ uint32_t resolve_entry(const TableView& tv, uint64_t e) {
   return (e & ENTRY_REF) ? tv.fids[static_cast<uint32_t>(e)] : static_cast<uint32_t>(e);
+}
+
+__device__ __forceinline__ bool ids_in_fids(const Slot& s) {
+  return (s.a.z & (META_HAS_EDGES | META_XFID)) == META_HAS_EDGES;
+}
+__device__ __forceinline__ uint32_t slot_id(const Slot& s, uint32_t kind) {
+  return ((s.a.z & META_HAS_EDGES) || kind) ? s.a.w : s.a.y;
 }
 
 __device__ __forceinline__ Slot empty_slot() {
@@ -480,7 +487,7 @@
 };
 
 constexpr uint32_t PA_WIDS = 192;
-template <int STACK_CAP, int WID_CAP, int K, bool DIAG, bool RL = false, int PA = 0, bool NH = true>
+template <int STACK_CAP, int WID_CAP, int K, bool DIAG, bool RL = false, int PA = 0, bool NH = true, class E = SlabWide>
 __device__ __forceinline__ void fast_tile(const MatchArgs& a, FastLds<STACK_CAP, WID_CAP>& L, uint64_t tile,
                                           uint32_t tt, const uint4* rl = nullptr, uint32_t rsz = 0) {
   static_assert(STACK_CAP >= 4 * 64 * K && STACK_CAP % 128 == 0, "stack must hold 4 pops");
@@ -694,7 +701,7 @@
   }
   const uint64_t clk1 = DIAG ? wall_clock64() : 0;
 
-  uint64_t* slab = a.slab + tile * a.slab_cap;
+  typename E::T* slab = static_cast<typename E::T*>(a.slab) + tile * a.slab_cap;
   uint2* spill = a.spill + tile * a.spill_cap;
   const uint32_t cap = a.slab_cap;
   const uint32_t mode = a.mode;
@@ -728,9 +735,8 @@
     const uint32_t c = (e0 ? 1u : 0u) + (e1 ? 1u : 0u);
     uint32_t tot;
     uint32_t pos = wave_prefix<2>(c, lane, &tot);
-    const uint64_t tag = static_cast<uint64_t>(lane) << 32;
-    if (e0) { if (pos < cap) slab[pos] = tag | tv.root_hash_fid; ++pos; }
-    if (e1) { if (pos < cap) slab[pos] = tag | g1; ++pos; }
+    if (e0) { if (pos < cap) slab[pos] = E::make(lane, tv.root_hash_fid); ++pos; }
+    if (e1) { if (pos < cap) slab[pos] = E::make(lane, g1); ++pos; }
     if (c) L.cnt[lane] = c;
     cursor = tot;
     uint32_t ptot;
@@ -740,6 +746,31 @@
     maxtop = top;
     wave_sync();
   }
+
+  uint2 pv[2 * K];
+  uint32_t ppos[K], pend[K];
+#pragma unroll
+  for (int k = 0; k < K; ++k) {
+    pv[2 * k] = pv[2 * k + 1] = make_uint2(0, 0);
+    ppos[k] = 0;
+    pend[k] = 0;
+  }
+  auto flush_pending = [&]() {
+    bool any = false;
+#pragma unroll
+    for (int k = 0; k < K; ++k) any = any || (pend[k] & 0x30u);
+    if (!__ballot(any)) return;
+#pragma unroll
+    for (int k = 0; k < K; ++k) {
+      const uint32_t f = pend[k], ptl = f >> 8;
+      uint32_t q = ppos[k];
+      if (f & 1u) { if ((f & 0x10u) && q < cap) slab[q] = E::make(ptl, pv[2 * k].x); ++q; }
+      if (f & 2u) { if ((f & 0x10u) && q < cap) slab[q] = E::make(ptl, pv[2 * k].y); ++q; }
+      if (f & 4u) { if ((f & 0x20u) && q < cap) slab[q] = E::make(ptl, pv[2 * k + 1].x); ++q; }
+      if (f & 8u) { if ((f & 0x20u) && q < cap) slab[q] = E::make(ptl, pv[2 * k + 1].y); ++q; }
+      pend[k] = 0;
+    }
+  };
 
   if (DIAG && a.diag_stop) top = 0;
   constexpr uint32_t POP = 64u * K;
@@ -818,6 +849,9 @@
     }
     probe_items<K, RL>(tv.edges, tv.plus_mask, ibase, hpar, isph, cpy, needL, wid, needP, lit, fL, pls, fP, dg[4], rl,
                        rsz, tv.root_base);
+#pragma unroll
+    for (int k = 0; k < 2 * K; ++k) asm volatile("" : "+v"(pv[k].x), "+v"(pv[k].y));
+    flush_pending();
     if (DIAG) {
 #pragma unroll
       for (int k = 0; k < K; ++k) {
@@ -874,11 +908,19 @@
       uint32_t pos = cursor + wave_prefix<ceil_log2(4 * K + 1)>(ecount, lane, &tot);
 #pragma unroll
       for (int k = 0; k < K; ++k) {
-        const uint64_t tag = static_cast<uint64_t>(tl[k]) << 32;
-        if (eLh[k]) { if (pos < cap) slab[pos] = tag | emit_value(lit[k], 0); ++pos; }
-        if (eLt[k]) { if (pos < cap) slab[pos] = tag | emit_value(lit[k], 1); ++pos; }
-        if (ePh[k]) { if (pos < cap) slab[pos] = tag | emit_value(pls[k], 0); ++pos; }
-        if (ePt[k]) { if (pos < cap) slab[pos] = tag | emit_value(pls[k], 1); ++pos; }
+        const bool rL = (eLh[k] || eLt[k]) && ids_in_fids(lit[k]);
+        const bool rP = (ePh[k] || ePt[k]) && ids_in_fids(pls[k]);
+        if (rL) pv[2 * k] = *reinterpret_cast<const uint2*>(tv.fids + 2ull * lit[k].idx);
+        if (rP) pv[2 * k + 1] = *reinterpret_cast<const uint2*>(tv.fids + 2ull * pls[k].idx);
+        if (rL || rP) {
+          ppos[k] = pos;
+          pend[k] = (eLh[k] ? 1u : 0u) | (eLt[k] ? 2u : 0u) | (ePh[k] ? 4u : 0u) | (ePt[k] ? 8u : 0u) |
+                    (rL ? 0x10u : 0u) | (rP ? 0x20u : 0u) | (tl[k] << 8);
+        }
+        if (eLh[k]) { if (!rL && pos < cap) slab[pos] = E::make(tl[k], slot_id(lit[k], 0)); ++pos; }
+        if (eLt[k]) { if (!rL && pos < cap) slab[pos] = E::make(tl[k], slot_id(lit[k], 1)); ++pos; }
+        if (ePh[k]) { if (!rP && pos < cap) slab[pos] = E::make(tl[k], slot_id(pls[k], 0)); ++pos; }
+        if (ePt[k]) { if (!rP && pos < cap) slab[pos] = E::make(tl[k], slot_id(pls[k], 1)); ++pos; }
         if (ce[k]) atomicAdd(&L.cnt[tl[k]], ce[k]);
       }
       cursor += tot;
@@ -887,6 +929,7 @@
     wave_sync();
   }
 
+  flush_pending();
   wave_sync();
   if (DIAG && a.diag) {
     dg[0] = lane == 0 ? dg[0] : 0u;
@@ -928,7 +971,8 @@
 constexpr uint32_t ROOT_LDS_SLOTS = 256;
 
 constexpr int fast_waves_hint(int K, int WC) { return K == 1 ? (WC == 448 ? 7 : 8) : 5; }
-template <int WAVES, int STACK_CAP, int WID_CAP, int K, bool DIAG, bool RL = false, int PA = 0, bool NH = true>
+template <int WAVES, int STACK_CAP, int WID_CAP, int K, bool DIAG, bool RL = false, int PA = 0, bool NH = true,
+          class E = SlabWide>
 __global__ __launch_bounds__(WAVES * 64, fast_waves_hint(K, WID_CAP)) void match_fast_kernel(MatchArgs a) {
   __shared__ FastLds<STACK_CAP, WID_CAP> lds_all[WAVES];
   __shared__ uint4 rl[RL ? ROOT_LDS_SLOTS : 1];
@@ -948,7 +992,7 @@
     const uint32_t nb = gridDim.x, x = blockIdx.x & 7u, j = blockIdx.x >> 3, q = nb >> 3, r = nb & 7u;
     blk = static_cast<uint64_t>(x) * q + min(x, r) + j;
   }
-  fast_tile<STACK_CAP, WID_CAP, K, DIAG, RL, PA, NH>(a, lds_all[wv], blk * WAVES + wv, TILE_TOPICS, rl, rsz);
+  fast_tile<STACK_CAP, WID_CAP, K, DIAG, RL, PA, NH, E>(a, lds_all[wv], blk * WAVES + wv, TILE_TOPICS, rl, rsz);
 }
 
 __device__ __forceinline__ void deep_walk(const MatchArgs& a, uint32_t gw, uint32_t nwaves, uint32_t tt) {
@@ -1258,8 +1302,10 @@
   }
 }
 
+template <class E>
 __device__ __forceinline__ void scatter_tile(const MatchArgs& a, uint64_t tile, uint64_t off);
 
+template <class E>
 __global__ __launch_bounds__(256) void scatter_fast_kernel(MatchArgs a) {
   const uint32_t lane = lane_id();
   const uint32_t wv = threadIdx.x >> 6;
@@ -1281,31 +1327,31 @@
     off = before + wave_incl_scan64(c, lane) - c;
     if (t < a.n) a.out_off[t] = off;
   }
-  scatter_tile(a, tile, off);
-}
-
+  scatter_tile<E>(a, tile, off);
+}
+
+template <class E>
 __device__ __forceinline__ void scatter_tile(const MatchArgs& a, uint64_t tile, uint64_t off) {
+  typedef typename E::T T;
   const uint32_t lane = lane_id();
   uint64_t next = off;
   const uint32_t fill = min(a.tile_fill[tile], a.slab_cap);
   const uint64_t dmask = a.tile_defer[tile];
-  const uint64_t* slab = a.slab + tile * a.slab_cap;
+  const T* slab = static_cast<const T*>(a.slab) + tile * a.slab_cap;
   const uint64_t lt = lanemask_lt(lane);
-  constexpr uint32_t U = 4;
+  constexpr uint32_t U = 32 / sizeof(T);
   for (uint32_t i0 = 0; i0 < fill; i0 += 64 * U) {
-    uint64_t e[U];
-    uint32_t id[U];
+    T e[U];
 #pragma unroll
     for (uint32_t u = 0; u < U; ++u) {
       const uint32_t i = i0 + 64 * u + lane;
-      e[u] = i < fill ? slab[i] : ~0ull;
-    }
-#pragma unroll
-    for (uint32_t u = 0; u < U; ++u) id[u] = e[u] != ~0ull ? resolve_entry(a.tv, e[u]) : 0u;
+      e[u] = i < fill ? slab[i] : E::PAD;
+    }
 #pragma unroll
     for (uint32_t u = 0; u < U; ++u) {
-      const uint32_t tl = static_cast<uint32_t>(e[u] >> 32) & 63u;
-      const bool keep = e[u] != ~0ull && !((dmask >> tl) & 1ull);
+      if (i0 + 64 * u >= fill) break;
+      const uint32_t tl = E::owner(e[u]);
+      const bool keep = e[u] != E::PAD && !((dmask >> tl) & 1ull);
       const uint64_t km = __ballot(keep);
       uint64_t peers = km, mine = km;
 #pragma unroll
@@ -1319,7 +1365,7 @@
       const uint32_t hi = __shfl(static_cast<uint32_t>(next >> 32), static_cast<int>(tl), 64);
       if (keep) {
         const uint64_t p = ((static_cast<uint64_t>(hi) << 32) | lo) + rk;
-        if (p < a.out_cap) a.out_ids[p] = id[u];
+        if (p < a.out_cap) a.out_ids[p] = E::id(e[u]);
       }
       next += static_cast<uint64_t>(__popcll(mine));
     }
@@ -1519,7 +1565,7 @@
   if (!(flags & (SUM_F_RETRY | SUM_F_ERROR))) {
     if (wv < ntiles) {
       const uint64_t t = uint64_t(wv) * tt + lane;
-      scatter_tile(a, wv, (lane < tt && t < n) ? a.out_off[t] : 0);
+      scatter_tile<SlabWide>(a, wv, (lane < tt && t < n) ? a.out_off[t] : 0);
     }
     const uint32_t fill = min(ctrl(CTRL_DEEP_FILL), a.deep_slab_cap);
     for (uint32_t i = tid; i < fill; i += NT) {
@@ -1683,13 +1729,18 @@
 
 template <int W, int S, int WC, int K, bool RL = false, bool NH = true>
 static void launch_fast_t(const MatchArgs& a, uint64_t ntiles, hipStream_t s) {
-  const uint64_t grid = (ntiles + W - 1) / W;
-  if (a.diag)
-    hipLaunchKernelGGL((match_fast_kernel<W, S, WC, K, true, RL, 0, NH>), dim3(static_cast<uint32_t>(grid)),
-                       dim3(W * 64), 0, s, a);
-  else
-    hipLaunchKernelGGL((match_fast_kernel<W, S, WC, K, false, RL, 0, NH>), dim3(static_cast<uint32_t>(grid)),
-                       dim3(W * 64), 0, s, a);
+  const dim3 grid(static_cast<uint32_t>((ntiles + W - 1) / W)), block(W * 64);
+  if (a.narrow) {
+    if (a.diag)
+      hipLaunchKernelGGL((match_fast_kernel<W, S, WC, K, true, RL, 0, NH, SlabNarrow>), grid, block, 0, s, a);
+    else
+      hipLaunchKernelGGL((match_fast_kernel<W, S, WC, K, false, RL, 0, NH, SlabNarrow>), grid, block, 0, s, a);
+  } else {
+    if (a.diag)
+      hipLaunchKernelGGL((match_fast_kernel<W, S, WC, K, true, RL, 0, NH, SlabWide>), grid, block, 0, s, a);
+    else
+      hipLaunchKernelGGL((match_fast_kernel<W, S, WC, K, false, RL, 0, NH, SlabWide>), grid, block, 0, s, a);
+  }
 }
 
 hipError_t launch_match_fast(const MatchArgs& a, FastVariant v, hipStream_t s) {
@@ -1720,7 +1771,10 @@
       }
       const dim3 grid(static_cast<uint32_t>((ntiles + 3) / 4));
       hipLaunchKernelGGL((match_fast_kernel<4, 384, 640, 1, false, false, 1>), grid, dim3(256), 0, s, a);
-      hipLaunchKernelGGL((match_fast_kernel<4, 384, 640, 1, false, false, 2>), grid, dim3(256), 0, s, a);
+      if (a.narrow)
+        hipLaunchKernelGGL((match_fast_kernel<4, 384, 640, 1, false, false, 2, true, SlabNarrow>), grid, dim3(256), 0, s, a);
+      else
+        hipLaunchKernelGGL((match_fast_kernel<4, 384, 640, 1, false, false, 2>), grid, dim3(256), 0, s, a);
       break;
     }
     default: return hipErrorInvalidValue;
@@ -1731,7 +1785,7 @@
 hipError_t launch_small_batch(const SmallArgs& a, hipStream_t s) {
   const uint64_t tiles = a.tt ? (a.m.n + a.tt - 1) / a.tt : 0;
   if (a.m.n == 0 || a.m.n > SMALL_MAX_N || a.tt == 0 || a.tt > TILE_TOPICS || tiles > SMALL_WAVES ||
-      tiles > a.slab_tiles)
+      tiles > a.slab_tiles || a.m.narrow)
     return hipErrorInvalidValue;
   hipLaunchKernelGGL(small_batch_kernel, dim3(1), dim3(SMALL_WAVES * 64), 0, s, a);
   return hipGetLastError();
@@ -1767,7 +1821,11 @@
       if (err == hipSuccess) err = launch_scan(a.corig, a.n, a.out_off, a.partials, s);
       if (err != hipSuccess) return err;
     }
-    hipLaunchKernelGGL(scatter_fast_kernel, dim3(static_cast<uint32_t>((ntiles + 3) / 4)), dim3(256), 0, s, a);
+    const dim3 grid(static_cast<uint32_t>((ntiles + 3) / 4));
+    if (a.narrow)
+      hipLaunchKernelGGL(scatter_fast_kernel<SlabNarrow>, grid, dim3(256), 0, s, a);
+    else
+      hipLaunchKernelGGL(scatter_fast_kernel<SlabWide>, grid, dim3(256), 0, s, a);
   }
   hipLaunchKernelGGL(scatter_deep_kernel, dim3(64), dim3(256), 0, s, a);
   hipLaunchKernelGGL(summary_kernel, dim3(1), dim3(64), 0, s, a);
```

After: 1.894 billion topics/s, median of 6. 3.9% higher.
